# ratschlab/secedo

Measured on AMD Instinct MI355X. Metric: cell-pair x locus updates/sec (similarity matrix), higher is better.
Workload: dtype int64; 1 GPU; C3: 8000 cells x 100000 loci; entries=24345058, kept_entries=24223307, reads=23997029, block_cells=128, tiles=2016, normalization=ADD_MIN, max_fragment_length=1000, num_threads=8, parallelism=single GPU, backend=none, world_size=1, rccl_world_size=1

## Files before the change

include/secedo_simmat.h:

```cpp
#ifndef SECEDO_SIMMAT_H
#define SECEDO_SIMMAT_H

#include <stdint.h>

#ifdef __cplusplus
extern "C" {
#endif

#define SECEDO_OK 0
#define SECEDO_E_INVALID_ARG (-1)
#define SECEDO_E_INVALID_NORMALIZATION (-2)
#define SECEDO_E_NO_DEVICE (-3)
#define SECEDO_E_HIP (-4)
#define SECEDO_E_STATE (-5)
#define SECEDO_E_LIMIT (-6)

#define SECEDO_NORM_ADD_MIN 0
#define SECEDO_NORM_EXPONENTIATE 1
#define SECEDO_NORM_SCALE_MAX_1 2

int secedo_simmat_normalization_from_string(const char *name);

const char *secedo_simmat_last_error(void);
const char *secedo_simmat_version(void);
int secedo_simmat_device_count(void);

int secedo_simmat_compute(const uint32_t *chr_locus_off, uint32_t n_chr, const uint32_t *locus_pos,
                          const uint64_t *locus_entry_off, const uint32_t *read_ids,
                          const uint16_t *id_base16, const uint32_t *id_base32,
                          const uint32_t *group_id_to_pos, uint32_t n_groups, uint32_t num_cells,
                          uint32_t max_fragment_length, double mutation_rate,
                          double homozygous_rate, double seq_error_rate, uint32_t num_threads,
                          int normalization, double *out);
int secedo_simmat_set_devices(const int *device_ids, uint32_t n_devices);
int secedo_simmat_get_devices(int *device_ids, uint32_t capacity);

int secedo_simmat_staging_acquire(const uint64_t bytes[5], void *ptrs[5]);
void secedo_simmat_staging_release(void);

void secedo_simmat_release_cache(void);

typedef struct secedo_simmat secedo_simmat_t;

int secedo_simmat_create(secedo_simmat_t **handle, int device_id);
void secedo_simmat_destroy(secedo_simmat_t *handle);

int secedo_simmat_set_pileup(secedo_simmat_t *handle, const uint32_t *chr_locus_off, uint32_t n_chr,
                             const uint32_t *locus_pos, const uint64_t *locus_entry_off,
                             const uint32_t *read_ids, const uint16_t *id_base16,
                             const uint32_t *id_base32, const uint32_t *group_id_to_pos,
                             uint32_t n_groups);

int secedo_simmat_set_pileup_device(secedo_simmat_t *handle, const uint32_t *d_chr_locus_off,
                                    uint32_t n_chr, const uint32_t *d_locus_pos,
                                    const uint64_t *d_locus_entry_off, const uint32_t *d_read_ids,
                                    const uint16_t *d_id_base16, const uint32_t *d_id_base32,
                                    const uint32_t *d_group_id_to_pos, uint32_t n_groups,
                                    uint32_t n_loci, uint64_t n_entries);

int secedo_simmat_set_packing(secedo_simmat_t *handle, int mode);
int secedo_simmat_used_device_packing(const secedo_simmat_t *handle);
int secedo_simmat_used_single_entry_path(const secedo_simmat_t *handle);
#define SECEDO_ROUTE_ATTEMPTS 3
#define SECEDO_ROUTE_RADIX 4
#define SECEDO_ROUTE_RETRIED_PLAIN 8
#define SECEDO_ROUTE_ASKED_HOST 16
int secedo_simmat_packing_route(const secedo_simmat_t *handle);

int secedo_simmat_prepare(secedo_simmat_t *handle, uint32_t num_cells, uint32_t max_fragment_length,
                          uint32_t num_threads, uint32_t block_cells, void *stream);

uint32_t secedo_simmat_num_tiles(const secedo_simmat_t *handle);
uint32_t secedo_simmat_block_cells(const secedo_simmat_t *handle);
uint64_t secedo_simmat_acc_elems(const secedo_simmat_t *handle);
uint64_t secedo_simmat_num_entries(const secedo_simmat_t *handle);
uint64_t secedo_simmat_num_reads(const secedo_simmat_t *handle);
uint64_t secedo_simmat_num_loci(const secedo_simmat_t *handle);

uint64_t secedo_simmat_pair_bound(const secedo_simmat_t *handle);
uint32_t secedo_simmat_max_read_entries(const secedo_simmat_t *handle);
int secedo_simmat_cell_squares(secedo_simmat_t *handle, uint64_t *d_out , void *stream);
int secedo_simmat_set_scale_bounds(secedo_simmat_t *handle, uint64_t pair_bound, uint32_t max_read_entries);
int secedo_simmat_set_pair_bound(secedo_simmat_t *handle, uint64_t pair_bound);
int secedo_simmat_scale_bounds_state(const secedo_simmat_t *handle);
int secedo_simmat_scale_log2(const secedo_simmat_t *handle);

int secedo_simmat_zero_acc(secedo_simmat_t *handle, int64_t *d_acc, void *stream);
int secedo_simmat_accumulate(secedo_simmat_t *handle, double mutation_rate, double homozygous_rate,
                             double seq_error_rate, uint32_t tile_begin, uint32_t tile_end,
                             int64_t *d_acc, void *stream);
int secedo_simmat_assign(secedo_simmat_t *handle, double mutation_rate, double homozygous_rate,
                         double seq_error_rate, uint32_t tile_begin, uint32_t tile_end, int64_t *d_acc,
                         void *stream);
int secedo_simmat_finalize(secedo_simmat_t *handle, int normalization, const int64_t *d_acc,
                           double *d_out, void *stream);
int secedo_simmat_assign_finalize(secedo_simmat_t *handle, double mutation_rate, double homozygous_rate,
                                  double seq_error_rate, int normalization, int64_t *d_acc, double *d_out,
                                  void *stream);
int secedo_simmat_tiles_of_rows(const secedo_simmat_t *handle, uint32_t row_begin, uint32_t row_end,
                                uint32_t *tile_ids, uint32_t *n_tile_ids);
int secedo_simmat_accumulate_list(secedo_simmat_t *handle, double mutation_rate, double homozygous_rate,
                                  double seq_error_rate, const uint32_t *tile_ids, uint32_t n_tile_ids,
                                  int64_t *d_acc, void *stream);
int secedo_simmat_assign_list(secedo_simmat_t *handle, double mutation_rate, double homozygous_rate,
                              double seq_error_rate, const uint32_t *tile_ids, uint32_t n_tile_ids,
                              int64_t *d_acc, void *stream);
int secedo_simmat_max_of_tiles(secedo_simmat_t *handle, const int64_t *d_acc, const uint32_t *tile_ids,
                               uint32_t n_tile_ids, double *max_value, void *stream);
int secedo_simmat_finalize_rows_max(secedo_simmat_t *handle, int normalization, const int64_t *d_acc,
                                    uint32_t row_begin, uint32_t row_end, double max_value, double *d_out_rows,
                                    void *stream);
int secedo_simmat_finalize_rows(secedo_simmat_t *handle, int normalization, const int64_t *d_acc,
                                uint32_t row_begin, uint32_t row_end, double *d_out_rows, void *stream);
int secedo_simmat_finalize_raw(secedo_simmat_t *handle, const int64_t *d_acc, double *d_out,
                               void *stream);

int secedo_simmat_last_counts(secedo_simmat_t *handle, uint64_t *updates, uint64_t *read_pairs);
int secedo_simmat_last_accumulate_ms(secedo_simmat_t *handle, float *ms);
int secedo_simmat_last_pair_kernel_ms(secedo_simmat_t *handle, float *ms);
const char *secedo_simmat_pair_kernel(const secedo_simmat_t *handle);
int secedo_simmat_last_correction_fused(const secedo_simmat_t *handle);
int secedo_simmat_last_locus_words(const secedo_simmat_t *handle);
uint32_t secedo_simmat_last_workgroups(const secedo_simmat_t *handle);
int secedo_simmat_debug_flag_lists(secedo_simmat_t *handle, uint64_t *n_flagged, uint32_t *grp, uint32_t *rec,
                                   uint32_t *idx);

double secedo_simmat_llr(uint32_t x_s, uint32_t x_d, double mutation_rate, double homozygous_rate,
                         double seq_error_rate);
double secedo_simmat_llr_closed_form(uint32_t x_s, uint32_t x_d, double mutation_rate, double homozygous_rate,
                                     double seq_error_rate);

int secedo_is_significant(const uint16_t *base_count , double seq_error_rate,
                          uint32_t cell_proportion);

int secedo_filter(const uint32_t *chr_locus_off, uint32_t n_chr, const uint32_t *locus_pos,
                  const uint64_t *locus_entry_off, const uint32_t *read_ids, const uint16_t *id_base16,
                  const uint32_t *id_base32, const uint32_t *id_to_pos, uint32_t n_groups,
                  double seq_error_rate, uint32_t cell_proportion, uint32_t *out_chr_locus_off,
                  uint32_t *out_locus_pos, uint64_t *out_locus_entry_off, uint32_t *out_read_ids,
                  void *out_id_base, uint64_t *out_n_loci, uint64_t *out_n_entries, double *avg_coverage);

int secedo_filter_device(const uint32_t *d_chr_locus_off, uint32_t n_chr, const uint32_t *d_locus_pos,
                         const uint64_t *d_locus_entry_off, const uint32_t *d_read_ids,
                         const uint16_t *d_id_base16, const uint32_t *d_id_base32, const uint32_t *d_id_to_pos,
                         uint32_t n_groups, uint32_t n_loci, uint64_t n_entries, double seq_error_rate,
                         uint32_t cell_proportion, uint32_t *d_out_chr_locus_off, uint32_t *d_out_locus_pos,
                         uint64_t *d_out_locus_entry_off, uint32_t *d_out_read_ids, void *d_out_id_base,
                         uint64_t *out_n_loci, uint64_t *out_n_entries, double *avg_coverage, void *stream);

typedef struct secedo_pileup_info {
    uint64_t n_loci;
    uint64_t n_entries;
    uint32_t num_cells;
    uint32_t max_read_length;
} secedo_pileup_info;

int secedo_pileup_read(const char *path, const uint16_t *id_to_group, uint32_t n_ids, uint32_t max_coverage,
                       const uint32_t *positions, uint64_t n_positions, int compute_max_read_len,
                       int write_bin, secedo_pileup_info *info, uint32_t *locus_pos,
                       uint64_t *locus_entry_off, uint32_t *read_ids, uint16_t *id_base16);
const char *secedo_pileup_last_error(void);

#ifdef __cplusplus
}
#endif
#endif
```

secedo_amd/_lib.py:

```python
from __future__ import annotations

import ctypes as C
import os

import numpy as np

HERE = os.path.dirname(os.path.abspath(__file__))
LIB_PATH = os.environ.get("SECEDO_LIB_PATH") or os.path.join(HERE, "libsecedo_simmat.so")

OK = 0
E_INVALID_ARG = -1
E_INVALID_NORMALIZATION = -2
E_NO_DEVICE = -3
E_HIP = -4
E_STATE = -5
E_LIMIT = -6

_u16p = C.POINTER(C.c_uint16)
_u32p = C.POINTER(C.c_uint32)
_u64p = C.POINTER(C.c_uint64)
_f64p = C.POINTER(C.c_double)
_vp = C.c_void_p


class PileupInfo(C.Structure):
    _fields_ = [("n_loci", C.c_uint64), ("n_entries", C.c_uint64), ("num_cells", C.c_uint32),
                ("max_read_length", C.c_uint32)]


class SpectralInfo(C.Structure):
    _fields_ = [("cycles", C.c_uint32), ("block_products", C.c_uint32), ("converged", C.c_uint32),
                ("reserved", C.c_uint32), ("max_residual_vectors", C.c_double),
                ("max_residual_values", C.c_double)]


ALLREDUCE_SUM_FN = C.CFUNCTYPE(C.c_int, C.c_void_p, C.c_void_p, C.c_uint64, C.c_void_p)


class SynthSpec(C.Structure):
    _fields_ = [
        ("num_cells", C.c_uint32), ("num_loci", C.c_uint32), ("num_chromosomes", C.c_uint32),
        ("gap_max", C.c_uint32), ("new_frag_prob", C.c_double), ("frag_min", C.c_uint32),
        ("frag_max", C.c_uint32), ("base_error", C.c_double), ("mate_frac", C.c_double),
        ("seed", C.c_uint64),
    ]


SIGNATURES = {
    "secedo_simmat_normalization_from_string": (C.c_int, [C.c_char_p]),
    "secedo_simmat_last_error": (C.c_char_p, []),
    "secedo_simmat_version": (C.c_char_p, []),
    "secedo_simmat_device_count": (C.c_int, []),
    "secedo_simmat_compute": (C.c_int, [_vp, C.c_uint32, _vp, _vp, _vp, _vp, _vp, _vp, C.c_uint32,
                                        C.c_uint32, C.c_uint32, C.c_double, C.c_double, C.c_double,
                                        C.c_uint32, C.c_int, _vp]),
    "secedo_simmat_release_cache": (None, []),
    "secedo_simmat_staging_acquire": (C.c_int, [_vp, _vp]),
    "secedo_simmat_staging_release": (None, []),
    "secedo_simmat_create": (C.c_int, [C.POINTER(_vp), C.c_int]),
    "secedo_simmat_destroy": (None, [_vp]),
    "secedo_simmat_set_pileup": (C.c_int, [_vp, _vp, C.c_uint32, _vp, _vp, _vp, _vp, _vp, _vp,
                                           C.c_uint32]),
    "secedo_simmat_set_pileup_device": (C.c_int, [_vp, _vp, C.c_uint32, _vp, _vp, _vp, _vp, _vp, _vp,
                                                  C.c_uint32, C.c_uint32, C.c_uint64]),
    "secedo_simmat_set_packing": (C.c_int, [_vp, C.c_int]),
    "secedo_simmat_used_device_packing": (C.c_int, [_vp]),
    "secedo_simmat_used_single_entry_path": (C.c_int, [_vp]),
    "secedo_simmat_packing_route": (C.c_int, [_vp]),
    "secedo_simmat_prepare": (C.c_int, [_vp, C.c_uint32, C.c_uint32, C.c_uint32, C.c_uint32, _vp]),
    "secedo_simmat_num_tiles": (C.c_uint32, [_vp]),
    "secedo_simmat_block_cells": (C.c_uint32, [_vp]),
    "secedo_simmat_acc_elems": (C.c_uint64, [_vp]),
    "secedo_simmat_num_entries": (C.c_uint64, [_vp]),
    "secedo_simmat_num_reads": (C.c_uint64, [_vp]),
    "secedo_simmat_num_loci": (C.c_uint64, [_vp]),
    "secedo_simmat_zero_acc": (C.c_int, [_vp, _vp, _vp]),
    "secedo_simmat_accumulate": (C.c_int, [_vp, C.c_double, C.c_double, C.c_double, C.c_uint32,
                                           C.c_uint32, _vp, _vp]),
    "secedo_simmat_finalize": (C.c_int, [_vp, C.c_int, _vp, _vp, _vp]),
    "secedo_simmat_tiles_of_rows": (C.c_int, [_vp, C.c_uint32, C.c_uint32, _vp, C.POINTER(C.c_uint32)]),
    "secedo_simmat_assign": (C.c_int, [_vp, C.c_double, C.c_double, C.c_double, C.c_uint32, C.c_uint32, _vp, _vp]),
    "secedo_simmat_assign_list": (C.c_int, [_vp, C.c_double, C.c_double, C.c_double, _vp, C.c_uint32, _vp, _vp]),
    "secedo_simmat_assign_finalize": (C.c_int, [_vp, C.c_double, C.c_double, C.c_double, C.c_int, _vp, _vp, _vp]),
    "secedo_simmat_accumulate_list": (C.c_int, [_vp, C.c_double, C.c_double, C.c_double, _vp, C.c_uint32, _vp, _vp]),
    "secedo_simmat_max_of_tiles": (C.c_int, [_vp, _vp, _vp, C.c_uint32, C.POINTER(C.c_double), _vp]),
    "secedo_simmat_finalize_rows_max": (C.c_int, [_vp, C.c_int, _vp, C.c_uint32, C.c_uint32, C.c_double, _vp, _vp]),
    "secedo_simmat_finalize_rows": (C.c_int, [_vp, C.c_int, _vp, C.c_uint32, C.c_uint32, _vp, _vp]),
    "secedo_simmat_finalize_raw": (C.c_int, [_vp, _vp, _vp, _vp]),
    "secedo_simmat_last_counts": (C.c_int, [_vp, _u64p, _u64p]),
    "secedo_simmat_last_accumulate_ms": (C.c_int, [_vp, C.POINTER(C.c_float)]),
    "secedo_simmat_last_pair_kernel_ms": (C.c_int, [_vp, C.POINTER(C.c_float)]),
    "secedo_simmat_pair_kernel": (C.c_char_p, [_vp]),
    "secedo_simmat_last_correction_fused": (C.c_int, [_vp]),
    "secedo_simmat_last_locus_words": (C.c_int, [_vp]),
    "secedo_simmat_last_workgroups": (C.c_uint32, [_vp]),
    "secedo_simmat_debug_flag_lists": (C.c_int, [_vp, _u64p, _vp, _vp, _vp]),
    "secedo_simmat_llr": (C.c_double, [C.c_uint32, C.c_uint32, C.c_double, C.c_double, C.c_double]),
    "secedo_simmat_llr_closed_form": (C.c_double, [C.c_uint32, C.c_uint32, C.c_double, C.c_double, C.c_double]),
    "secedo_simmat_pair_bound": (C.c_uint64, [_vp]),
    "secedo_simmat_set_pair_bound": (C.c_int, [_vp, C.c_uint64]),
    "secedo_simmat_max_read_entries": (C.c_uint32, [_vp]),
    "secedo_simmat_cell_squares": (C.c_int, [_vp, _vp, _vp]),
    "secedo_simmat_set_scale_bounds": (C.c_int, [_vp, C.c_uint64, C.c_uint32]),
    "secedo_simmat_scale_log2": (C.c_int, [_vp]),
    "secedo_simmat_scale_bounds_state": (C.c_int, [_vp]),
    "secedo_simmat_set_devices": (C.c_int, [C.POINTER(C.c_int), C.c_uint32]),
    "secedo_simmat_get_devices": (C.c_int, [C.POINTER(C.c_int), C.c_uint32]),
    "secedo_is_significant": (C.c_int, [_vp, C.c_double, C.c_uint32]),
    "secedo_filter": (C.c_int, [_vp, C.c_uint32, _vp, _vp, _vp, _vp, _vp, _vp, C.c_uint32, C.c_double,
                                C.c_uint32, _vp, _vp, _vp, _vp, _vp, _u64p, _u64p, _f64p]),
    "secedo_filter_device": (C.c_int, [_vp, C.c_uint32, _vp, _vp, _vp, _vp, _vp, _vp, C.c_uint32, C.c_uint32,
                                       C.c_uint64, C.c_double, C.c_uint32, _vp, _vp, _vp, _vp, _vp, _u64p,
                                       _u64p, _f64p, _vp]),
    "secedo_pileup_read": (C.c_int, [C.c_char_p, _vp, C.c_uint32, C.c_uint32, _vp, C.c_uint64, C.c_int, C.c_int,
                                     C.POINTER(PileupInfo), _vp, _vp, _vp, _vp]),
    "secedo_pileup_last_error": (C.c_char_p, []),
    "secedo_em_refine_device": (C.c_int, [C.c_int, _vp, C.c_uint32, C.c_uint64, _vp, _vp, _vp, C.c_uint32, C.c_double,
                                          _vp, C.c_uint32, C.c_uint32, C.POINTER(C.c_uint32), _vp]),
    "secedo_em_refine": (C.c_int, [C.c_int, _vp, C.c_uint32, _vp, _vp, _vp, C.c_uint32, C.c_double, _vp, C.c_uint32,
                                   C.c_uint32, C.POINTER(C.c_uint32)]),
    "secedo_laplacian_device": (C.c_int, [_vp, C.c_uint32, _vp, _vp]),
    "secedo_spectral_eigs_device": (C.c_int, [C.c_int, _vp, C.c_uint32, C.c_uint32, C.c_uint32, C.c_double,
                                              C.c_uint32, _vp, _vp, C.POINTER(SpectralInfo), _vp]),
    "secedo_spectral_eigs_rows_device": (C.c_int, [C.c_int, _vp, C.c_uint32, C.c_uint32, C.c_uint32, C.c_uint32,
                                                   C.c_uint32, C.c_double, C.c_uint32, _vp, _vp,
                                                   C.POINTER(SpectralInfo), _vp, _vp, _vp]),
    "secedo_spectral_eigs": (C.c_int, [C.c_int, _vp, C.c_uint32, C.c_uint32, C.c_uint32, C.c_double, C.c_uint32,
                                       _vp, _vp, C.POINTER(SpectralInfo)]),
}

_lib = None


class SecedoError(RuntimeError):
    def __init__(self, code, message):
        super().__init__("secedo_simmat error %d: %s" % (code, message))
        self.code = code


class InvalidNormalization(ValueError):
    """The reference throws std::logic_error here (similarity_matrix.cpp:264)."""


def lib():
    global _lib
    if _lib is None:
        if not os.path.exists(LIB_PATH):
            raise ImportError(
                "%s is missing: build it with `python -c 'import __graft_entry__ as g; g.build()'` "
                "or `make -C secedo_amd/csrc` (there is no fallback implementation)" % LIB_PATH)
        try:
            import torch
        except ImportError:
            pass
        l = C.CDLL(LIB_PATH)
        for name, (res, args) in SIGNATURES.items():
            f = getattr(l, name)
            f.restype = res
            f.argtypes = args
        _lib = l
    return _lib


def check(rc):
    if rc == OK:
        return
    msg = lib().secedo_simmat_last_error().decode(errors="replace")
    if rc == E_INVALID_NORMALIZATION:
        raise InvalidNormalization(msg)
    raise SecedoError(rc, msg)


def ptr(a):
    return None if a is None else a.ctypes.data
```

secedo_amd/csrc/pack_device.hip:

```cpp
#include "pack_device.hpp"

#include <hip/hip_runtime.h>
#include <hipcub/hipcub.hpp>

#include <algorithm>
#include <chrono>
#include <cstdio>
#include <cstdlib>
#include <cstring>
#include <functional>

namespace secedo {

DeviceArena::~DeviceArena() {
    if (p) (void)hipFree(p);
}

DevicePacked::~DevicePacked() {
    if (side) (void)hipStreamDestroy(side);
    if (ev_fork) (void)hipEventDestroy(ev_fork);
    if (ev_join) (void)hipEventDestroy(ev_join);
    if (ev_offsets) (void)hipEventDestroy(ev_offsets);
    if (ev_flush) (void)hipEventDestroy(ev_flush);
    if (mailbox) (void)hipHostFree(mailbox);
}

int poison_level() {
    static const int level = [] {
        const char *e = std::getenv("SECEDO_POISON");
        return e ? std::atoi(e) : 0;
    }();
    return level;
}

hipError_t DeviceArena::ensure(size_t n) {
    if (n <= bytes && p) return hipSuccess;
    if (p) (void)hipFree(p);
    p = nullptr;
    bytes = 0;
    const size_t want = n ? n + n / 8 + 256 : 256;
    hipError_t e = hipMalloc(&p, want);
    if (e == hipSuccess) bytes = want;
    if (e == hipSuccess && poison_level() >= 1) e = hipMemset(p, 0xA5, want);
    return e;
}

namespace {

constexpr int TPB = 256;

inline uint32_t blocks_for(uint64_t n) {
    return static_cast<uint32_t>(std::max<uint64_t>(1, std::min<uint64_t>((n + TPB - 1) / TPB, 1u << 16)));
}

struct Scalars {
    uint32_t error;
    uint32_t need_host;
    uint32_t num_ranges;
    uint32_t max_read_id;
    uint32_t regroup;
    uint32_t long_reads;
    uint32_t split_changed;
    uint32_t id_exceeded;
    uint32_t max_read_entries;
    uint32_t caps_wrong;
    uint32_t n_multi_id;
    uint32_t reads_total;
    uint32_t n_wide;
    uint32_t max_range_span;
    unsigned long long id_space;
    unsigned long long multi_entries;
    unsigned long long pair_bound;
};

struct Mailbox {
    Scalars sc;
    unsigned long long totals;
    unsigned long long seq;
};

__global__ void k_publish(const Scalars *sc, const unsigned long long *totals, Mailbox *box, unsigned long long seq) {
    if (threadIdx.x == 0) {
        box->sc = *sc;
        box->totals = totals ? *totals : 0ull;
        __hip_atomic_store(&box->seq, seq, __ATOMIC_RELEASE, __HIP_MEMORY_SCOPE_SYSTEM);
    }
}

hipError_t read_scalars(DevicePacked &pk, hipStream_t stream, const Scalars *sc, const unsigned long long *totals,
                        Scalars *out, unsigned long long *out_totals, const std::function<void()> &behind = nullptr) {
    static const bool plain = [] {
        const char *e = std::getenv("SECEDO_PACK_READBACK");
        return e && std::strcmp(e, "memcpy") == 0;
    }();
    hipError_t e;
    if (!plain && !pk.mailbox && !pk.mailbox_failed) {
        if (hipHostMalloc(&pk.mailbox, sizeof(Mailbox), hipHostMallocCoherent) == hipSuccess) {
            std::memset(pk.mailbox, 0, sizeof(Mailbox));
        } else {
            (void)hipGetLastError();
            pk.mailbox = nullptr;
            pk.mailbox_failed = true;
        }
    }
    if (!plain && pk.mailbox) {
        Mailbox *box = static_cast<Mailbox *>(pk.mailbox);
        const unsigned long long seq = ++pk.mailbox_seq;
        hipLaunchKernelGGL(k_publish, dim3(1), dim3(64), 0, stream, sc, totals, box, seq);
        if ((e = hipGetLastError()) != hipSuccess) return e;
        if (behind) behind();
        bool arrived = false;
        for (unsigned spins = 0;; ++spins) {
            if (__atomic_load_n(&box->seq, __ATOMIC_ACQUIRE) == seq) {
                arrived = true;
                break;
            }
            if ((spins & 0xFFFu) == 0xFFFu) {
                const hipError_t q = hipStreamQuery(stream);
                if (q != hipErrorNotReady) {
                    arrived = __atomic_load_n(&box->seq, __ATOMIC_ACQUIRE) == seq;
                    if (q != hipSuccess) return q;
                    break;
                }
            }
        }
        if (arrived) {
            *out = box->sc;
            if (out_totals) *out_totals = box->totals;
            return hipSuccess;
        }
    } else if (behind) {
        behind();
    }
    if (out_totals) {
        *out_totals = 0;
        if (totals && (e = hipMemcpyAsync(out_totals, totals, 8, hipMemcpyDeviceToHost, stream)) != hipSuccess) return e;
    }
    if ((e = hipMemcpyAsync(out, sc, sizeof(*out), hipMemcpyDeviceToHost, stream)) != hipSuccess) return e;
    return hipStreamSynchronize(stream);
}

struct HostTrace {
    bool on;
    std::chrono::steady_clock::time_point t0;
    HostTrace() : on(std::getenv("SECEDO_PACK_TRACE") != nullptr), t0(std::chrono::steady_clock::now()) {}
    void mark(const char *what) const {
        if (on)
            std::fprintf(stderr, "[pack-trace] %8.1f us  %s\n",
                         std::chrono::duration<double, std::micro>(std::chrono::steady_clock::now() - t0).count(), what);
    }
};

constexpr uint32_t kRankScanLimit = 8192;
constexpr int kMaxSplitRounds = 32;
constexpr uint32_t kIdSpaceFactor = 4;

struct Raw {
    const uint32_t *chr_locus_off;
    uint32_t n_chr;
    const uint32_t *locus_pos;
    const uint64_t *locus_entry_off;
    const uint32_t *read_ids;
    const uint16_t *id_base16;
    const uint32_t *id_base32;
    const uint32_t *g2p;
    uint32_t n_groups;
    uint32_t n_loci;
    uint32_t n_entries;
    __device__ __forceinline__ uint32_t id_base(uint32_t e) const {
        return id_base16 ? (uint32_t)id_base16[e] : id_base32[e];
    }
};

template <class T>
__device__ __forceinline__ uint32_t last_le(const T *a, uint32_t n, T x) {
    uint32_t lo = 0, hi = n;
    while (hi - lo > 1) {
        const uint32_t mid = lo + (hi - lo) / 2;
        if (a[mid] <= x) lo = mid; else hi = mid;
    }
    return lo;
}

__global__ __launch_bounds__(TPB) void k_entry_locus(Raw in, uint32_t *entry_locus, Scalars *sc) {
    const uint32_t lane = threadIdx.x & 63u;
    const uint32_t wave = (blockIdx.x * TPB + threadIdx.x) >> 6, n_waves = (gridDim.x * TPB) >> 6;
    for (uint32_t l = wave; l < in.n_loci; l += n_waves) {
        const uint32_t b = (uint32_t)in.locus_entry_off[l], e = (uint32_t)in.locus_entry_off[l + 1];
        for (uint32_t i = b + lane; i < e; i += 64u) entry_locus[i] = l;
        if (lane == 0u && l + 1 < in.n_loci && in.locus_pos[l + 1] <= in.locus_pos[l]) {
            const uint32_t c = last_le<uint32_t>(in.chr_locus_off, in.n_chr + 1, l);
            if (l + 1 < in.chr_locus_off[c + 1]) sc->error = 3;
        }
    }
}

__device__ __forceinline__ uint32_t chr_first_entry(const Raw &in, uint32_t c) {
    return (uint32_t)in.locus_entry_off[in.chr_locus_off[c]];
}

__global__ __launch_bounds__(TPB) void k_id_range(Raw in, uint32_t *id_max, uint32_t *id_negmin, int vec, Scalars *sc) {
    __shared__ uint32_t s_hi[TPB / 64], s_neg[TPB / 64];
    __shared__ uint32_t s_chr;
    for (uint32_t l = blockIdx.x * TPB + threadIdx.x; l + 1 < in.n_loci; l += gridDim.x * TPB) {
        if (in.locus_pos[l + 1] <= in.locus_pos[l]) {
            const uint32_t c = last_le<uint32_t>(in.chr_locus_off, in.n_chr + 1, l);
            if (l + 1 < in.chr_locus_off[c + 1]) sc->error = 3;
        }
    }
    const uint32_t E = in.n_entries;
    const uint32_t chunk = (E + gridDim.x - 1) / gridDim.x;
    uint32_t cur = min(E, blockIdx.x * chunk);
    const uint32_t e1 = min(E, cur + chunk);
    if (cur >= e1) return;
    if (threadIdx.x == 0) s_chr = 0;
    __syncthreads();
    {
        uint32_t best = 0;
        for (uint32_t i = threadIdx.x; i < in.n_chr; i += TPB)
            if (chr_first_entry(in, i) <= cur) best = i;
        if (best) atomicMax(&s_chr, best);
    }
    __syncthreads();
    uint32_t c = s_chr;
    while (cur < e1) {
        uint32_t c_end = (uint32_t)in.locus_entry_off[in.chr_locus_off[c + 1]];
        while (c_end <= cur && c + 1 < in.n_chr) {
            ++c;
            c_end = (uint32_t)in.locus_entry_off[in.chr_locus_off[c + 1]];
        }
        const uint32_t seg_end = (c + 1 < in.n_chr) ? min(e1, c_end) : e1;
        uint32_t hi = 0, neg = 0;
        uint32_t s_cur = cur, s_end = seg_end;
        if (vec) {
            const uint32_t a = min(seg_end, (cur + 3u) & ~3u), b = max(a, seg_end & ~3u);
            if (threadIdx.x < a - cur) {
                const uint32_t id = in.read_ids[cur + threadIdx.x];
                hi = max(hi, id);
                neg = max(neg, ~id);
            }
            if (threadIdx.x < seg_end - b) {
                const uint32_t id = in.read_ids[b + threadIdx.x];
                hi = max(hi, id);
                neg = max(neg, ~id);
            }
            const uint4 *src = reinterpret_cast<const uint4 *>(in.read_ids);
            for (uint32_t q = a / 4u + threadIdx.x; q < b / 4u; q += TPB * 4) {
                uint4 v[4];
#pragma unroll
                for (int u = 0; u < 4; ++u) v[u] = q + (uint32_t)u * TPB < b / 4u ? src[q + (uint32_t)u * TPB] : src[q];
#pragma unroll
                for (int u = 0; u < 4; ++u) {
                    hi = max(max(hi, v[u].x), max(max(v[u].y, v[u].z), v[u].w));
                    neg = max(max(neg, ~v[u].x), max(max(~v[u].y, ~v[u].z), ~v[u].w));
                }
            }
            s_cur = s_end = seg_end;
        }
        for (uint32_t e = s_cur + threadIdx.x; e < s_end; e += TPB * 8) {
            uint32_t id[8];
#pragma unroll
            for (int u = 0; u < 8; ++u) {
                const uint32_t eu = e + (uint32_t)u * TPB;
                id[u] = eu < s_end ? in.read_ids[eu] : in.read_ids[e];
            }
#pragma unroll
            for (int u = 0; u < 8; ++u) {
                hi = max(hi, id[u]);
                neg = max(neg, ~id[u]);
            }
        }
        for (int off = 32; off > 0; off >>= 1) {
            hi = max(hi, (uint32_t)__shfl_down(hi, off));
            neg = max(neg, (uint32_t)__shfl_down(neg, off));
        }
        __syncthreads();
        if ((threadIdx.x & 63u) == 0) {
            s_hi[threadIdx.x >> 6] = hi;
            s_neg[threadIdx.x >> 6] = neg;
        }
        __syncthreads();
        if (threadIdx.x == 0) {
            for (int w = 1; w < TPB / 64; ++w) {
                hi = max(hi, s_hi[w]);
                neg = max(neg, s_neg[w]);
            }
            atomicMax(&id_max[c], hi);
            atomicMax(&id_negmin[c], neg);
        }
        cur = seg_end;
    }
}

__global__ void k_id_bases(Raw in, const uint32_t *id_max, const uint32_t *id_negmin, uint32_t *id_base,
                           uint32_t *chr_entry, unsigned long long assumed_space, Scalars *sc) {
    const uint32_t n_chr = in.n_chr;
    if (blockIdx.x != 0) return;
    for (uint32_t c = threadIdx.x; c <= n_chr; c += blockDim.x) chr_entry[c] = chr_first_entry(in, c);
    if (threadIdx.x != 0) return;
    unsigned long long sum = 0;
    uint32_t top = 0;
    for (uint32_t c = 0; c < n_chr; ++c) {
        id_base[c] = (uint32_t)min(sum, 0xFFFFFFFFull);
        const uint32_t lo = ~id_negmin[c];
        if ((id_max[c] | id_negmin[c]) != 0u) sum += (unsigned long long)(id_max[c] - lo) + 1ull;
        top = max(top, id_max[c]);
    }
    id_base[n_chr] = (uint32_t)min(sum, 0xFFFFFFFFull);
    sc->id_space = sum;
    sc->max_read_id = top;
    if (assumed_space && sum > assumed_space) sc->id_exceeded = 1;
}

__global__ void k_entry_keys(Raw in, const uint32_t *entry_locus, uint32_t id_bits, unsigned long long *key,
                             uint32_t *val) {
    for (uint32_t e = blockIdx.x * TPB + threadIdx.x; e < in.n_entries; e += gridDim.x * TPB) {
        const uint32_t c = last_le<uint32_t>(in.chr_locus_off, in.n_chr + 1, entry_locus[e]);
        key[e] = ((unsigned long long)c << id_bits) | in.read_ids[e];
        val[e] = e;
    }
}

constexpr uint32_t kSlocLocusMask = 0x3FFFFFFFu;
__device__ __forceinline__ uint32_t sloc_pack(uint32_t locus, uint32_t id_base) { return locus | (id_base << 30); }
__device__ __forceinline__ uint32_t sloc_locus(uint32_t v) { return v & kSlocLocusMask; }
__device__ __forceinline__ uint32_t sloc_base(uint32_t v) { return v >> 30; }

__global__ void k_sorted_locus(Raw in, const uint32_t *sval, const uint32_t *entry_locus, uint32_t n, uint32_t *sloc) {
    for (uint32_t s = blockIdx.x * TPB + threadIdx.x; s < n; s += gridDim.x * TPB)
        sloc[s] = sloc_pack(entry_locus[sval[s]], in.id_base(sval[s]));
}

constexpr uint32_t kChrLds = 1024;
struct ChrTables {
    uint32_t first[kChrLds + 1], base[kChrLds], min_id[kChrLds];
};
__device__ __forceinline__ bool chr_tables_load(const Raw &in, const uint32_t *first, const uint32_t *id_base,
                                                const uint32_t *id_negmin, ChrTables &t) {
    const bool in_lds = in.n_chr <= kChrLds;
    if (in_lds) {
        for (uint32_t i = threadIdx.x; i <= in.n_chr; i += blockDim.x) t.first[i] = first[i];
        for (uint32_t i = threadIdx.x; i < in.n_chr; i += blockDim.x) {
            t.base[i] = id_base[i];
            t.min_id[i] = ~id_negmin[i];
        }
    }
    __syncthreads();
    return in_lds;
}
__device__ __forceinline__ uint32_t chr_of(const Raw &in, const uint32_t *first, const ChrTables &t, bool in_lds,
                                           uint32_t key) {
    return last_le<uint32_t>(in_lds ? t.first : first, in.n_chr + 1, key);
}
__device__ __forceinline__ uint32_t dense_of(const uint32_t *id_base, const uint32_t *id_negmin, const ChrTables &t,
                                             bool in_lds, uint32_t c, uint32_t id) {
    return in_lds ? t.base[c] + (id - t.min_id[c]) : id_base[c] + (id - ~id_negmin[c]);
}
__device__ __forceinline__ uint32_t dense_id(const Raw &in, const uint32_t *first, const uint32_t *id_base,
                                             const uint32_t *id_negmin, const ChrTables &t, bool in_lds, uint32_t key,
                                             uint32_t id) {
    return dense_of(id_base, id_negmin, t, in_lds, chr_of(in, first, t, in_lds, key), id);
}
__device__ __forceinline__ void dense_id_quad(const Raw &in, const uint32_t *chr_entry, const uint32_t *id_base,
                                              const uint32_t *id_negmin, const ChrTables &t, bool in_lds, uint32_t e0,
                                              const uint32_t (&id)[4], uint32_t (&d)[4]) {
    const uint32_t c0 = chr_of(in, chr_entry, t, in_lds, e0);
    const uint32_t next = in_lds ? t.first[c0 + 1] : chr_entry[c0 + 1];
#pragma unroll
    for (int u = 0; u < 4; ++u) {
        const uint32_t e = min(e0 + (uint32_t)u, in.n_entries - 1u);
        const uint32_t c = e < next ? c0 : chr_of(in, chr_entry, t, in_lds, e);
        d[u] = dense_of(id_base, id_negmin, t, in_lds, c, id[u]);
    }
}

__global__ void k_id_hist(Raw in, const uint32_t *entry_locus, const uint32_t *id_base, const uint32_t *id_negmin,
                          const Scalars *sc, uint32_t *dense, uint32_t *hist) {
    if (sc->id_exceeded) return;
    __shared__ ChrTables tables;
    const bool in_lds = chr_tables_load(in, in.chr_locus_off, id_base, id_negmin, tables);
    for (uint32_t e = blockIdx.x * TPB + threadIdx.x; e < in.n_entries; e += gridDim.x * TPB) {
        const uint32_t d = dense_id(in, in.chr_locus_off, id_base, id_negmin, tables, in_lds, entry_locus[e], in.read_ids[e]);
        dense[e] = d;
        atomicAdd(&hist[d], 1u);
    }
}

__global__ void k_id_scatter(const uint32_t *dense, uint32_t n, const uint32_t *id_off, const Scalars *sc,
                             uint32_t *hist, uint32_t *grouped) {
    if (sc->id_exceeded) return;
    for (uint32_t e = blockIdx.x * TPB + threadIdx.x; e < n; e += gridDim.x * TPB) {
        const uint32_t d = dense[e];
        grouped[id_off[d] + atomicSub(&hist[d], 1u) - 1u] = e;
    }
}

__global__ void k_id_rank(Raw in, const uint32_t *dense, const uint32_t *id_off, const uint32_t *grouped,
                          const uint32_t *entry_locus, unsigned long long *skey, uint32_t *sval, uint32_t *sloc,
                          Scalars *sc) {
    const bool void_run = sc->id_exceeded != 0;
    for (uint32_t p = blockIdx.x * TPB + threadIdx.x; p < in.n_entries; p += gridDim.x * TPB) {
        if (void_run) {
            skey[p] = p;
            sval[p] = p;
            sloc[p] = 0;
            continue;
        }
        const uint32_t e = grouped[p];
        const uint32_t d = dense[e];
        const uint32_t b = id_off[d], n = id_off[d + 1] - b;
        uint32_t rank = p - b;
        if (n > kRankScanLimit) {
            sc->regroup = 1;
        } else if (n > 1) {
            rank = 0;
            for (uint32_t q = b; q < b + n; ++q) rank += grouped[q] < e ? 1u : 0u;
        }
        skey[b + rank] = d;
        sval[b + rank] = e;
        sloc[b + rank] = sloc_pack(entry_locus[e], in.id_base(e));
    }
}

__device__ __forceinline__ void load_id_quad(const Raw &in, uint32_t q, int vec, uint32_t (&id)[4]) {
    const uint32_t n = in.n_entries, e0 = q * 4u;
    if (vec && e0 + 4u <= n) {
        const uint4 iv = reinterpret_cast<const uint4 *>(in.read_ids)[q];
        id[0] = iv.x, id[1] = iv.y, id[2] = iv.z, id[3] = iv.w;
    } else {
#pragma unroll
        for (int u = 0; u < 4; ++u) id[u] = in.read_ids[min(e0 + (uint32_t)u, n - 1u)];
    }
}
__global__ void k_id_store(Raw in, const uint32_t *chr_entry, const uint32_t *id_base, const uint32_t *id_negmin,
                           const Scalars *sc, uint32_t *last, int vec) {
    if (sc->id_exceeded) return;
    __shared__ ChrTables tables;
    const bool in_lds = chr_tables_load(in, chr_entry, id_base, id_negmin, tables);
    const uint32_t n = in.n_entries, stride = gridDim.x * TPB;
    for (uint32_t q = blockIdx.x * TPB + threadIdx.x; q < (n + 3u) / 4u; q += stride) {
        const uint32_t e0 = q * 4u;
        uint32_t id[4], d[4];
        load_id_quad(in, q, vec, id);
        dense_id_quad(in, chr_entry, id_base, id_negmin, tables, in_lds, e0, id, d);
#pragma unroll
        for (int u = 0; u < 4; ++u)
            if (e0 + (uint32_t)u < n) last[d[u]] = e0 + (uint32_t)u + 1u;
    }
}
__global__ void k_id_check(Raw in, const uint32_t *chr_entry, const uint32_t *id_base, const uint32_t *id_negmin,
                           const Scalars *sc, const uint32_t *last, uint8_t *multi, int vec) {
    if (sc->id_exceeded) return;
    __shared__ ChrTables tables;
    const bool in_lds = chr_tables_load(in, chr_entry, id_base, id_negmin, tables);
    const uint32_t n = in.n_entries, stride = gridDim.x * TPB;
    for (uint32_t q = blockIdx.x * TPB + threadIdx.x; q < (n + 3u) / 4u; q += stride) {
        const uint32_t e0 = q * 4u;
        uint32_t id[4], d[4], w[4];
        load_id_quad(in, q, vec, id);
        dense_id_quad(in, chr_entry, id_base, id_negmin, tables, in_lds, e0, id, d);
#pragma unroll
        for (int u = 0; u < 4; ++u) w[u] = e0 + (uint32_t)u < n ? last[d[u]] : 0u;
#pragma unroll
        for (int u = 0; u < 4; ++u) {
            const uint32_t e = e0 + (uint32_t)u;
            if (e < n && w[u] != e + 1u) {
                multi[e] = 1;
                multi[w[u] - 1u] = 1;
            }
        }
    }
}
__global__ __launch_bounds__(TPB) void k_flag_count(const uint8_t *multi, uint32_t *block_sum) {
    __shared__ uint32_t part[TPB / 64];
    static_assert(kFlagBlock == TPB * 16, "a thread takes 16 consecutive flags");
    const uint4 w = reinterpret_cast<const uint4 *>(multi + (size_t)blockIdx.x * kFlagBlock)[threadIdx.x];
    uint32_t n = ((w.x * 0x01010101u) >> 24) + ((w.y * 0x01010101u) >> 24) + ((w.z * 0x01010101u) >> 24)
            + ((w.w * 0x01010101u) >> 24);
    for (int off = 32; off > 0; off >>= 1) n += __shfl_down(n, off);
    if ((threadIdx.x & 63u) == 0u) part[threadIdx.x >> 6] = n;
    __syncthreads();
    if (threadIdx.x == 0u) {
        for (int w2 = 1; w2 < TPB / 64; ++w2) n += part[w2];
        block_sum[blockIdx.x] = n;
    }
}
constexpr int TPB_SCAN = 1024;
__global__ __launch_bounds__(TPB_SCAN) void k_flag_scan(const uint32_t *block_sum, uint32_t n_blocks, uint32_t *block_off,
                                                       uint32_t *total_out, Scalars *sc) {
    constexpr int TPB = TPB_SCAN;
    __shared__ uint32_t part[TPB / 64];
    __shared__ uint32_t carry;
    if (threadIdx.x == 0u) carry = 0;
    __syncthreads();
    const uint32_t lane = threadIdx.x & 63u, wv = threadIdx.x >> 6;
    for (uint32_t base = 0; base < n_blocks; base += TPB) {
        const uint32_t i = base + threadIdx.x;
        const uint32_t v = i < n_blocks ? block_sum[i] : 0u;
        uint32_t incl = v;
        for (int off = 1; off < 64; off <<= 1) {
            const uint32_t up = __shfl_up(incl, off);
            if (lane >= (uint32_t)off) incl += up;
        }
        if (lane == 63u) part[wv] = incl;
        __syncthreads();
        uint32_t before = carry;
        for (uint32_t w2 = 0; w2 < wv; ++w2) before += part[w2];
        if (i < n_blocks) block_off[i] = before + incl - v;
        __syncthreads();
        if (threadIdx.x == TPB - 1) carry = before + incl;
        __syncthreads();
    }
    if (threadIdx.x == 0u) {
        *total_out = carry;
        if (sc) sc->n_multi_id = carry;
    }
}
struct MIndex {
    const uint32_t *chunk_pre;
    const unsigned long long *chunk_mask;
    __device__ __forceinline__ uint32_t operator()(uint32_t e) const {
        const uint32_t c = e >> 6, r = e & 63u;
        return chunk_pre[c] + (uint32_t)__popcll(chunk_mask[c] & ((1ull << r) - 1ull));
    }
};
__global__ __launch_bounds__(TPB) void k_compact_m(Raw in, const uint8_t *multi, const uint32_t *block_off,
                                                  uint32_t *chunk_pre, unsigned long long *chunk_mask,
                                                  uint32_t *m_entry) {
    __shared__ uint32_t part[TPB / 64];
    const uint32_t lane = threadIdx.x & 63u, wv = threadIdx.x >> 6;
    const uint32_t e0 = blockIdx.x * kFlagBlock + threadIdx.x * 16u;
    const uint4 w = reinterpret_cast<const uint4 *>(multi + (size_t)blockIdx.x * kFlagBlock)[threadIdx.x];
    const uint32_t words[4] = {w.x, w.y, w.z, w.w};
    uint32_t bits = 0;
#pragma unroll
    for (int i = 0; i < 16; ++i) bits |= ((words[i >> 2] >> ((i & 3) * 8)) & 1u) << i;
    const uint32_t mine = (uint32_t)__popc(bits);
    uint32_t incl = mine;
    for (int off = 1; off < 64; off <<= 1) {
        const uint32_t up = __shfl_up(incl, off);
        if (lane >= (uint32_t)off) incl += up;
    }
    if (lane == 63u) part[wv] = incl;
    __syncthreads();
    uint32_t j = block_off[blockIdx.x] + incl - mine;
    for (uint32_t w2 = 0; w2 < wv; ++w2) j += part[w2];
    unsigned long long m = (unsigned long long)bits << ((lane & 3u) * 16u);
    m |= __shfl_xor(m, 1);
    m |= __shfl_xor(m, 2);
    if ((lane & 3u) == 0u) {
        const uint32_t chunk = blockIdx.x * (kFlagBlock / 64u) + (threadIdx.x >> 2);
        chunk_pre[chunk] = j;
        chunk_mask[chunk] = m;
    }
    if (blockIdx.x == gridDim.x - 1u && threadIdx.x == 0u) chunk_mask[gridDim.x * (kFlagBlock / 64u)] = 0ull;
    for (uint32_t b = bits; b; b &= b - 1u) m_entry[j++] = e0 + (uint32_t)__ffs((int)b) - 1u;
}
__global__ __launch_bounds__(TPB) void k_pflag_count(const uint32_t *entry32, uint32_t n, uint32_t *block_sum) {
    __shared__ uint32_t part[TPB / 64];
    const uint32_t b0 = blockIdx.x * kFlagBlock + threadIdx.x;
    uint32_t c = 0;
#pragma unroll
    for (int k = 0; k < 16; ++k) {
        const uint32_t e = b0 + (uint32_t)k * TPB;
        c += (e < n && (entry32[e] & (kC_Tail | kC_Multi)) != 0u) ? 1u : 0u;
    }
    for (int off = 32; off > 0; off >>= 1) c += __shfl_down(c, off);
    if ((threadIdx.x & 63u) == 0u) part[threadIdx.x >> 6] = c;
    __syncthreads();
    if (threadIdx.x == 0u) {
        for (int w = 1; w < TPB / 64; ++w) c += part[w];
        block_sum[blockIdx.x] = c;
    }
}
__global__ __launch_bounds__(TPB) void k_pflag_compact(const uint32_t *entry32, const uint4 *entry, uint32_t n,
                                                      const uint32_t *block_off, uint4 *rec, uint32_t *idx,
                                                      uint32_t *chunk_pre, unsigned long long *chunk_mask) {
    constexpr int WAVES = TPB / 64;
    static_assert(16 * WAVES == 64, "one wave scans the (round, wave) counts");
    __shared__ uint32_t cnt[16 * WAVES];
    const uint32_t lane = threadIdx.x & 63u, wv = threadIdx.x >> 6;
    const uint32_t b0 = blockIdx.x * kFlagBlock + threadIdx.x;
    unsigned long long m[16];
#pragma unroll
    for (int k = 0; k < 16; ++k) {
        const uint32_t e = b0 + (uint32_t)k * TPB;
        m[k] = __ballot(e < n && (entry32[e] & (kC_Tail | kC_Multi)) != 0u);
        if (lane == 0u) cnt[k * WAVES + wv] = (uint32_t)__popcll(m[k]);
    }
    __syncthreads();
    if (threadIdx.x < 64u) {
        const uint32_t v = cnt[threadIdx.x];
        uint32_t incl = v;
        for (int off = 1; off < 64; off <<= 1) {
            const uint32_t up = __shfl_up(incl, off);
            if (lane >= (uint32_t)off) incl += up;
        }
        cnt[threadIdx.x] = incl - v;
    }
    __syncthreads();
    const uint32_t base = block_off[blockIdx.x];
#pragma unroll
    for (int k = 0; k < 16; ++k) {
        const uint32_t e = b0 + (uint32_t)k * TPB;
        const uint32_t before = base + cnt[k * WAVES + wv];
        if (lane == 0u) {
            const uint32_t chunk = (blockIdx.x * kFlagBlock + (uint32_t)k * TPB) / 64u + wv;
            chunk_pre[chunk] = before;
            chunk_mask[chunk] = m[k];
        }
        if ((m[k] >> lane) & 1ull) {
            const uint32_t j = before + (uint32_t)__popcll(m[k] & ((1ull << lane) - 1ull));
            rec[j] = entry[e];
            idx[j] = e;
        }
    }
}
__global__ __launch_bounds__(TPB) void k_pflag_compact_masks(const unsigned long long *chunk_mask, const uint4 *entry,
                                                            const uint32_t *block_off, uint4 *rec, uint32_t *idx,
                                                            uint32_t *chunk_pre) {
    constexpr int WAVES = TPB / 64;
    constexpr uint32_t CHUNKS = kFlagBlock / 64u;
    static_assert(CHUNKS == 64, "one wave scans the chunks' counts");
    __shared__ unsigned long long mask[CHUNKS];
    __shared__ uint32_t pre[CHUNKS];
    const uint32_t lane = threadIdx.x & 63u, wv = threadIdx.x >> 6;
    const uint32_t chunk0 = blockIdx.x * CHUNKS;
    if (threadIdx.x < 64u) {
        const unsigned long long m = chunk_mask[chunk0 + threadIdx.x];
        const uint32_t v = (uint32_t)__popcll(m);
        uint32_t incl = v;
        for (int off = 1; off < 64; off <<= 1) {
            const uint32_t up = __shfl_up(incl, off);
            if (lane >= (uint32_t)off) incl += up;
        }
        mask[threadIdx.x] = m;
        pre[threadIdx.x] = incl - v;
        chunk_pre[chunk0 + threadIdx.x] = block_off[blockIdx.x] + incl - v;
    }
    __syncthreads();
    const uint32_t base = block_off[blockIdx.x];
#pragma unroll 4
    for (uint32_t c = wv; c < CHUNKS; c += WAVES) {
        const unsigned long long m = mask[c];
        if ((m >> lane) & 1ull) {
            const uint32_t e = (chunk0 + c) * 64u + lane;
            const uint32_t j = base + pre[c] + (uint32_t)__popcll(m & ((1ull << lane) - 1ull));
            rec[j] = entry[e];
            idx[j] = e;
        }
    }
}
__global__ __launch_bounds__(TPB) void k_pflag_groups(const uint32_t *blk_off, size_t n_off, const uint32_t *chunk_pre,
                                                     const unsigned long long *chunk_mask, uint32_t *grp) {
    for (size_t i = (size_t)blockIdx.x * TPB + threadIdx.x; i < n_off; i += (size_t)gridDim.x * TPB) {
        const uint32_t d = blk_off[i], c = d >> 6, r = d & 63u;
        grp[i] = chunk_pre[c] + (r ? (uint32_t)__popcll(chunk_mask[c] & ((1ull << r) - 1ull)) : 0u);
    }
}
void flag_groups(const FlagScratch &fs, const uint32_t *blk_off, size_t n_off, uint32_t *grp, hipStream_t stream) {
    if (!n_off) return;
    const uint32_t blocks = (uint32_t)std::min<size_t>((n_off + TPB - 1) / TPB, 256 * 32);
    hipLaunchKernelGGL(k_pflag_groups, dim3(blocks), dim3(TPB), 0, stream, blk_off, n_off, fs.chunk_pre, fs.chunk_mask, grp);
}
void flag_lists_from_masks(const FlagScratch &fs, const uint4 *entry, const uint32_t *blk_off, size_t n_off,
                           uint32_t *grp, uint4 *rec, uint32_t *idx, hipStream_t stream) {
    hipLaunchKernelGGL(k_flag_scan, dim3(1), dim3(TPB_SCAN), 0, stream, fs.block_sum, fs.nb, fs.block_off,
                       fs.chunk_pre + 64 * (size_t)fs.nb, static_cast<Scalars *>(nullptr));
    hipLaunchKernelGGL(k_pflag_compact_masks, dim3(fs.nb), dim3(TPB), 0, stream, fs.chunk_mask, entry, fs.block_off, rec,
                       idx, fs.chunk_pre);
    flag_groups(fs, blk_off, n_off, grp, stream);
}

__global__ void k_m_fields(Raw in, const uint32_t *chr_entry, const uint32_t *id_base, const uint32_t *id_negmin,
                           const uint32_t *last, MIndex m_index, const uint32_t *m_entry, uint32_t n_m, uint32_t *rid_m,
                           uint32_t *idb_m, uint32_t *eloc_m, uint32_t *winner_m, uint32_t *count_m) {
    __shared__ ChrTables tables;
    const bool in_lds = chr_tables_load(in, chr_entry, id_base, id_negmin, tables);
    for (uint32_t j = blockIdx.x * TPB + threadIdx.x; j < n_m; j += gridDim.x * TPB) {
        const uint32_t e = m_entry[j];
        const uint32_t id = in.read_ids[e];
        rid_m[j] = id;
        idb_m[j] = in.id_base(e);
        eloc_m[j] = last_le<uint64_t>(in.locus_entry_off, in.n_loci + 1, (uint64_t)e);
        const uint32_t d = dense_id(in, chr_entry, id_base, id_negmin, tables, in_lds, e, id);
        const uint32_t w = m_index(last[d] - 1u);
        winner_m[j] = w;
        atomicAdd(&count_m[w], 1u);
    }
}
__global__ void k_group_scatter(const uint32_t *winner_m, uint32_t n_m, const uint32_t *goff, uint32_t *count_m,
                                uint32_t *members, uint32_t *g_begin, uint32_t *g_len) {
    for (uint32_t j = blockIdx.x * TPB + threadIdx.x; j < n_m; j += gridDim.x * TPB) {
        const uint32_t w = winner_m[j];
        const uint32_t b = goff[w], n = goff[w + 1] - b;
        members[b + atomicSub(&count_m[w], 1u) - 1u] = j;
        g_begin[j] = b;
        g_len[j] = n;
    }
}
__global__ void k_group_rank(Raw sub, const uint32_t *members, const uint32_t *g_begin, const uint32_t *g_len,
                             const uint32_t *eloc_m, uint32_t n_m, unsigned long long *skey, uint32_t *sval,
                             uint32_t *sloc, Scalars *sc) {
    for (uint32_t p = blockIdx.x * TPB + threadIdx.x; p < n_m; p += gridDim.x * TPB) {
        const uint32_t m = members[p];
        const uint32_t b = g_begin[m], n = g_len[m];
        uint32_t rank = p - b;
        if (n > kRankScanLimit) {
            sc->regroup = 1;
        } else {
            rank = 0;
            for (uint32_t q = b; q < b + n; ++q) rank += members[q] < m ? 1u : 0u;
        }
        skey[b + rank] = b;
        sval[b + rank] = m;
        sloc[b + rank] = sloc_pack(eloc_m[m], sub.id_base(m));
    }
}

constexpr uint32_t kCibBits = 7;
constexpr uint32_t kNoEntry = 0xFFFFFFFFu;
constexpr uint32_t kSingle = 0x80000000u;
constexpr uint32_t kSingleBaseShift = 29;
constexpr uint32_t kSingleTail = 4u;

struct Ranks {
    MIndex m_index;
    const uint32_t *unm;
    const uint32_t *arank;
    __device__ __forceinline__ uint32_t operator()(uint32_t e) const { return unm ? e - unm[m_index(e)] : arank[e]; }
};
struct UnmarkedM {
    const uint32_t *mark_m;
    uint32_t n_m;
    __device__ __forceinline__ uint32_t operator()(uint32_t j) const { return j < n_m ? 1u - mark_m[j] : 0u; }
};
__global__ void k_arank_m(const uint32_t *unm, const uint32_t *m_entry, uint32_t n_m, uint32_t n, uint32_t *arank_m,
                          Scalars *sc) {
    for (uint32_t j = blockIdx.x * TPB + threadIdx.x; j < n_m; j += gridDim.x * TPB) arank_m[j] = m_entry[j] - unm[j];
    if (blockIdx.x == 0 && threadIdx.x == 0) sc->reads_total = n - unm[n_m];
}
__global__ void k_rbeg(Raw in, Ranks rank, uint32_t *rbeg) {
    for (uint32_t c = blockIdx.x * TPB + threadIdx.x; c <= in.n_chr; c += gridDim.x * TPB)
        rbeg[c] = rank((uint32_t)in.locus_entry_off[in.chr_locus_off[c]]);
}
struct HeadKeepOp {
    const unsigned long long *skey;
    const uint32_t *keep;
    const uint32_t *split;
    __device__ __forceinline__ unsigned long long operator()(uint32_t s) const {
        const unsigned long long head = (s == 0 || skey[s] != skey[s - 1] || (split && split[s])) ? 1ull : 0ull;
        return head | ((unsigned long long)keep[s] << 32);
    }
};
__device__ __forceinline__ uint32_t incl_reads(unsigned long long v) { return (uint32_t)v; }
__device__ __forceinline__ uint32_t incl_kept(unsigned long long v) { return (uint32_t)(v >> 32); }

__global__ void k_dup_mark(Raw in, const unsigned long long *skey, const uint32_t *sval,
                           const uint32_t *sloc, const uint32_t *split, uint32_t n, uint32_t *keep,
                           uint32_t *mark) {
    for (uint32_t s = blockIdx.x * TPB + threadIdx.x; s < n; s += gridDim.x * TPB) {
        const uint32_t e = sval[s];
        const uint32_t l = sloc_locus(sloc[s]);
        const bool same_read = s > 0 && skey[s] == skey[s - 1];
        mark[e] = (same_read && !(split && split[s])) ? 0u : 1u;
        if (s == 0) mark[n] = 0u;
        if (same_read && sloc_locus(sloc[s - 1]) == l) continue;
        uint32_t stored = s;
        bool have = true;
        keep[s] = 0u;
        for (uint32_t t = s + 1; t < n && skey[t] == skey[s] && sloc_locus(sloc[t]) == l; ++t) {
            keep[t] = 0u;
            if (have) {
                if (sloc_base(sloc[t]) != sloc_base(sloc[stored])) have = false;
            } else {
                stored = t;
                have = true;
            }
        }
        if (have) keep[stored] = 1u;
    }
}

__global__ void k_runs_csr(Raw in, const unsigned long long *incl, const uint32_t *sval,
                           const uint32_t *sloc, uint32_t n, uint32_t *run_start, uint32_t *read_locus,
                           uint8_t *read_base) {
    for (uint32_t s = blockIdx.x * TPB + threadIdx.x; s < n; s += gridDim.x * TPB) {
        const unsigned long long cur = incl[s], prev = s ? incl[s - 1] : 0ull;
        if (incl_reads(cur) != incl_reads(prev)) run_start[incl_reads(cur) - 1] = s;
        if (s == n - 1) run_start[incl_reads(cur)] = n;
        if (incl_kept(cur) != incl_kept(prev)) {
            const uint32_t k = incl_kept(prev), v = sloc[s];
            read_locus[k] = sloc_locus(v);
            read_base[k] = (uint8_t)sloc_base(v);
        }
    }
}

__global__ __launch_bounds__(TPB) void k_read_info(Raw in, const unsigned long long *incl, const uint32_t *run_start,
                                                  const uint32_t *sval, const uint32_t *sloc,
                                                  const uint32_t *arank, uint32_t mfl, uint32_t *run_rank,
                                                  uint32_t *rbeg, uint32_t *read_off, Scalars *sc) {
    __shared__ unsigned long long part[TPB / 64];
    __shared__ uint32_t part_len[TPB / 64];
    const uint32_t n = in.n_entries;
    const uint32_t n_runs = n ? incl_reads(incl[n - 1]) : 0u;
    unsigned long long multi = 0;
    uint32_t longest = 0;
    for (uint32_t r = blockIdx.x * TPB + threadIdx.x; r < n_runs; r += gridDim.x * TPB) {
        const uint32_t s0 = run_start[r], s1 = run_start[r + 1];
        const uint32_t e0 = sval[s0];
        const uint32_t p0 = in.locus_pos[sloc_locus(sloc[s0])], p1 = in.locus_pos[sloc_locus(sloc[s1 - 1])];
        if (p1 - p0 >= mfl) sc->long_reads = 1;
        if ((unsigned long long)p1 + mfl > 0xFFFFFFFFull) sc->need_host = 1;
        const uint32_t rk = arank[e0];
        run_rank[r] = rk;
        const uint32_t k0 = s0 ? incl_kept(incl[s0 - 1]) : 0u, k1 = incl_kept(incl[s1 - 1]);
        read_off[r] = k0;
        if (r == n_runs - 1) read_off[n_runs] = k1;
        if (k1 - k0 > 1) multi += k1 - k0;
        longest = max(longest, k1 - k0);
    }
    if (rbeg) {
        for (uint32_t c = blockIdx.x * TPB + threadIdx.x; c <= in.n_chr; c += gridDim.x * TPB)
            rbeg[c] = arank[(uint32_t)in.locus_entry_off[in.chr_locus_off[c]]];
    }
    for (int off = 32; off > 0; off >>= 1) {
        multi += __shfl_down(multi, off);
        longest = max(longest, (uint32_t)__shfl_down(longest, off));
    }
    if ((threadIdx.x & 63) == 0) {
        part[threadIdx.x >> 6] = multi;
        part_len[threadIdx.x >> 6] = longest;
    }
    __syncthreads();
    if (threadIdx.x == 0) {
        unsigned long long sum = 0;
        uint32_t len = 0;
        for (int w = 0; w < TPB / 64; ++w) {
            sum += part[w];
            len = max(len, part_len[w]);
        }
        if (sum) atomicAdd(&sc->multi_entries, sum);
        if (len > 1) atomicMax(&sc->max_read_entries, len);
    }
}

__global__ void k_completed(Raw in, Ranks rank, const uint32_t *rbeg, uint32_t mfl, uint32_t *cnt, Scalars *sc) {
    for (uint32_t l = blockIdx.x * TPB + threadIdx.x; l < in.n_loci; l += gridDim.x * TPB) {
        const uint32_t c = last_le<uint32_t>(in.chr_locus_off, in.n_chr + 1, l);
        const uint32_t pos = in.locus_pos[l], l0 = in.chr_locus_off[c];
        if ((unsigned long long)pos + mfl > 0xFFFFFFFFull && in.locus_entry_off[l + 1] > in.locus_entry_off[l])
            sc->need_host = 1;
        uint32_t done = 0;
        if (pos >= mfl && in.locus_pos[l0] <= pos - mfl) {
            const uint32_t lp = l0 + last_le<uint32_t>(in.locus_pos + l0, l - l0 + 1, pos - mfl);
            done = rank((uint32_t)in.locus_entry_off[lp + 1]) - rbeg[c];
        }
        cnt[l] = done;
    }
}

__global__ __launch_bounds__(TPB) void k_flush_chain(Raw in, const uint32_t *cnt, uint32_t threshold,
                                                    const Scalars *sc, uint32_t *flushed_out,
                                                    uint32_t *flush_loci, uint32_t *flush_count, Ranks rank,
                                                    const uint32_t *rbeg, uint32_t *tail_begin) {
    __shared__ uint32_t buf[2048];
    __shared__ uint32_t hits[2048];
    __shared__ uint32_t s_flushed, s_listed, s_hits;
    const uint32_t c = blockIdx.x;
    const uint32_t l0 = in.chr_locus_off[c], l1 = in.chr_locus_off[c + 1];
    if (threadIdx.x == 0) {
        s_flushed = 0;
        s_listed = 0;
    }
    for (uint32_t base = l0; base < l1; base += 2048) {
        const uint32_t n = min(2048u, l1 - base);
        __syncthreads();
        for (uint32_t i = threadIdx.x; i < n; i += TPB) buf[i] = cnt[base + i];
        __syncthreads();
        if (threadIdx.x == 0) {
            uint32_t f = s_flushed, h = 0;
            if (sc->long_reads) {
                for (uint32_t i = 0; i < n; ++i) {
                    const uint32_t v = buf[i];
                    if (v - f >= threshold) {
                        f = v;
                        hits[h++] = base + i;
                    }
                }
            } else {
                for (uint32_t i = 0; i < n; ++i) {
                    const uint32_t v = buf[i];
                    if (v - f >= threshold) f = v;
                }
            }
            s_flushed = f;
            s_hits = h;
        }
        __syncthreads();
        const uint32_t h = s_hits, listed = s_listed;
        for (uint32_t i = threadIdx.x; i < h; i += TPB) flush_loci[l0 + listed + i] = hits[i];
        __syncthreads();
        if (threadIdx.x == 0) s_listed = listed + h;
    }
    __syncthreads();
    if (threadIdx.x == 0) {
        flushed_out[c] = s_flushed;
        flush_count[c] = s_listed;
    }
    if (tail_begin) {
        __shared__ uint32_t s_first;
        const unsigned long long want = (unsigned long long)rbeg[c] + s_flushed;
        uint32_t lo = (uint32_t)in.locus_entry_off[l0], hi = (uint32_t)in.locus_entry_off[l1];
        while (lo < hi) {
            const uint32_t step = (hi - lo + TPB - 1) / TPB;
            const unsigned long long probe = (unsigned long long)lo + (unsigned long long)threadIdx.x * step;
            const bool reached = probe < hi && (unsigned long long)rank((uint32_t)probe) >= want;
            __syncthreads();
            if (threadIdx.x == 0) s_first = TPB;
            __syncthreads();
            if (reached) atomicMin(&s_first, threadIdx.x);
            __syncthreads();
            const uint32_t first = s_first;
            if (first == TPB) {
                lo = lo + ((hi - lo - 1) / step) * step + 1;
            } else {
                hi = lo + first * step;
                if (first) lo = lo + (first - 1) * step + 1;
            }
        }
        if (threadIdx.x == 0) tail_begin[c] = lo;
    }
}

__global__ void k_split_update(Raw in, const unsigned long long *skey, const uint32_t *sloc, uint32_t mfl, const uint32_t *flush_loci,
                               const uint32_t *flush_count, uint32_t *split, Scalars *sc) {
    const uint32_t n = in.n_entries;
    for (uint32_t s = blockIdx.x * TPB + threadIdx.x; s < n; s += gridDim.x * TPB) {
        if (s > 0 && skey[s] == skey[s - 1]) continue;
        uint32_t end = s + 1;
        while (end < n && skey[end] == skey[s]) ++end;
        if (end == s + 1) continue;
        const uint32_t l_first = sloc_locus(sloc[s]);
        const uint32_t p_first = in.locus_pos[l_first], p_last = in.locus_pos[sloc_locus(sloc[end - 1])];
        if (p_last - p_first < mfl) continue;
        const uint32_t c = last_le<uint32_t>(in.chr_locus_off, in.n_chr + 1, l_first);
        const uint32_t *fl = flush_loci + in.chr_locus_off[c];
        const uint32_t n_fl = flush_count[c];
        uint32_t seg_start = p_first, l_prev = l_first;
        for (uint32_t t = s + 1; t < end; ++t) {
            const uint32_t l_t = sloc_locus(sloc[t]);
            uint32_t cut = 0;
            if (l_t != l_prev) {
                uint32_t lo = 0, hi = n_fl;
                const unsigned long long reach = (unsigned long long)seg_start + mfl;
                while (lo < hi) {
                    const uint32_t mid = lo + (hi - lo) / 2;
                    if (fl[mid] <= l_prev || in.locus_pos[fl[mid]] < reach) lo = mid + 1; else hi = mid;
                }
                if (lo < n_fl && fl[lo] <= l_t) {
                    cut = 1;
                    seg_start = in.locus_pos[l_t];
                }
            }
            if (split[t] != cut) {
                split[t] = cut;
                sc->split_changed = 1;
            }
            l_prev = l_t;
        }
    }
}

__device__ __forceinline__ unsigned long long bin_key(uint32_t blk, uint32_t l, uint32_t cib, uint32_t lbits) {
    return ((((unsigned long long)blk << lbits) | l) << kCibBits) | cib;
}

__global__ void k_keys2(Raw in, const uint32_t *sval, const unsigned long long *incl,
                        const uint32_t *read_locus, const uint32_t *run_rank, const uint32_t *read_off,
                        uint32_t num_cells, uint32_t B,
                        uint32_t lbits, unsigned long long *key2, uint32_t *val2, uint32_t *t_read,
                        uint32_t *krank, uint8_t *kflags, unsigned long long *entry_kc, const uint32_t *entry_map,
                        uint32_t *blk_cnt_add, uint32_t L, Scalars *sc) {
    const uint32_t n = in.n_entries;
    for (uint32_t s = blockIdx.x * TPB + threadIdx.x; s < n; s += gridDim.x * TPB) {
        const unsigned long long cur = incl[s], prev = s ? incl[s - 1] : 0ull;
        const uint32_t e_out = entry_map ? entry_map[sval[s]] : sval[s];
        if (incl_kept(cur) == incl_kept(prev)) {
            if (entry_kc) entry_kc[e_out] = kNoEntry;
            continue;
        }
        const uint32_t k = incl_kept(prev);
        const uint32_t group = in.id_base(sval[s]) >> 2;
        uint32_t cell = 0;
        if (group >= in.n_groups) {
            sc->error = 1;
        } else {
            cell = in.g2p[group];
            if (cell >= num_cells) {
                sc->error = 2;
                cell = 0;
            }
        }
        const uint32_t blk = cell / B, cib = cell - blk * B;
        if (key2) {
            key2[k] = bin_key(blk, read_locus[k], cib, lbits);
            val2[k] = k;
        }
        const uint32_t r = incl_reads(cur) - 1;
        t_read[k] = r;
        krank[k] = run_rank[r];
        kflags[k] = (uint8_t)((in.id_base(sval[s]) & 3u) | (read_off[r + 1] - read_off[r] > 1u ? 4u : 0u));
        if (entry_kc) entry_kc[e_out] = ((unsigned long long)((blk << kCibBits) | cib) << 32) | k;
        if (blk_cnt_add) atomicAdd(&blk_cnt_add[(size_t)blk * (L + 1) + read_locus[k]], 1u);
    }
}

__device__ __forceinline__ uint32_t tile_locus(const uint32_t *s_off, uint32_t lo, uint32_t hi, uint32_t e) {
    while (hi - lo > 1u) {
        const uint32_t mid = (lo + hi) >> 1;
        if (s_off[mid] <= e) lo = mid; else hi = mid;
    }
    return lo;
}

__global__ __launch_bounds__(TPB) void k_bin_hist(Raw in, uint32_t nb, uint32_t TL, unsigned long long *__restrict__ entry_kc,
                                                 const unsigned long long *__restrict__ m_mask, uint32_t num_cells,
                                                 uint32_t B_log2, uint32_t *__restrict__ blk_cnt, Scalars *sc,
                                                 uint32_t g2p_lds) {
    extern __shared__ uint32_t lds_hist[];
    __shared__ uint32_t s_off[65];
    static_assert(TPB >= 65, "one thread per offset");
    const uint32_t L = in.n_loci, TLP = TL + 1u, TL_log2 = 31u - (uint32_t)__clz((int)TL);
    const uint32_t n_tiles = (L + TL - 1u) / TL;
    constexpr int U = 4;
    uint16_t *s_g2p = reinterpret_cast<uint16_t *>(lds_hist + nb * TLP);
    if (g2p_lds) {
        for (uint32_t i = threadIdx.x; i < in.n_groups; i += TPB) s_g2p[i] = (uint16_t)min(in.g2p[i], 0xFFFFu);
    }
    for (uint32_t tile = blockIdx.x; tile < n_tiles; tile += gridDim.x) {
        const uint32_t l0 = tile * TL, n_l = min(TL, L - l0);
        for (uint32_t i = threadIdx.x; i < nb * TLP; i += TPB) lds_hist[i] = 0;
        if (threadIdx.x <= n_l) s_off[threadIdx.x] = (uint32_t)in.locus_entry_off[l0 + threadIdx.x];
        __syncthreads();
        const uint32_t eb = s_off[0], ee = s_off[n_l];
        for (uint32_t base = eb + threadIdx.x; base < ee; base += TPB * U) {
            uint32_t slot[U];
            constexpr uint32_t kNone = 0xFFFFFFFFu;
            if (m_mask) {
                unsigned long long mw[U];
                uint32_t ib[U], cell[U];
                bool is_m[U];
#pragma unroll
                for (int u = 0; u < U; ++u) {
                    const uint32_t e = base + (uint32_t)u * TPB;
                    const bool in_tile = e < ee;
                    mw[u] = in_tile ? m_mask[e >> 6] : ~0ull;
                    ib[u] = in_tile ? in.id_base(e) : 0u;
                }
#pragma unroll
                for (int u = 0; u < U; ++u) {
                    const uint32_t group = ib[u] >> 2;
                    cell[u] = 0;
                    is_m[u] = (mw[u] >> ((base + (uint32_t)u * TPB) & 63u)) & 1ull;
                    if (!is_m[u]) {
                        if (group >= in.n_groups) sc->error = 1;
                        else cell[u] = g2p_lds ? (uint32_t)s_g2p[group] : in.g2p[group];
                    }
                }
#pragma unroll
                for (int u = 0; u < U; ++u) {
                    slot[u] = kNone;
                    if (is_m[u]) continue;
                    const uint32_t e = base + (uint32_t)u * TPB;
                    uint32_t c = cell[u];
                    if (c >= num_cells) {
                        sc->error = 2;
                        c = 0;
                    }
                    const uint32_t blk = c >> B_log2, cib = c - (blk << B_log2);
                    entry_kc[e] = ((unsigned long long)(((ib[u] & 3u) << kSingleBaseShift) | (blk << kCibBits) | cib) << 32)
                            | kSingle;
                    slot[u] = blk;
                }
            } else {
#pragma unroll
                for (int u = 0; u < U; ++u) {
                    const uint32_t e = base + (uint32_t)u * TPB;
                    const unsigned long long kc = e < ee ? entry_kc[e] : (unsigned long long)kNoEntry;
                    slot[u] = (uint32_t)kc != kNoEntry ? (uint32_t)(kc >> 32) >> kCibBits : kNone;
                }
            }
#pragma unroll
            for (int u = 0; u < U; ++u) {
                if (slot[u] == kNone) continue;
                const uint32_t j = tile_locus(s_off, 0u, n_l, base + (uint32_t)u * TPB);
                atomicAdd(&lds_hist[slot[u] * TLP + j], 1u);
            }
        }
        __syncthreads();
        for (uint32_t i = threadIdx.x; i < nb * TL; i += TPB) {
            const uint32_t b = i >> TL_log2, j = i & (TL - 1u);
            if (j < n_l) {
                blk_cnt[(size_t)b * (L + 1) + l0 + j] = lds_hist[b * TLP + j];
                if (l0 + j == L - 1) blk_cnt[(size_t)b * (L + 1) + L] = 0;
            }
        }
        __syncthreads();
    }
}

__global__ __launch_bounds__(TPB) void k_bin_place(Raw in, uint32_t nb, uint32_t TL,
                                                  const unsigned long long *__restrict__ entry_kc,
                                                  const uint32_t *__restrict__ blk_off, uint32_t B_log2, uint32_t bm_words,
                                                  const uint32_t *tail_begin,
                                                  unsigned long long *__restrict__ grouped, uint8_t *dupflag) {
    extern __shared__ uint32_t lds_hist[];
    __shared__ uint32_t s_off[65];
    __shared__ uint32_t s_tail[64];
    constexpr uint32_t NW = TPB / 64;
    constexpr int D = 4;
    const uint32_t lane = threadIdx.x & 63u, wv = threadIdx.x >> 6, L = in.n_loci, TLP = TL + 1u;
    const uint32_t TL_log2 = 31u - (uint32_t)__clz((int)TL);
    uint32_t *bm = lds_hist + nb * TLP + wv * bm_words;
    for (uint32_t i = lane; i < bm_words; i += 64u) bm[i] = 0;
    const uint32_t n_tiles = (L + TL - 1u) / TL;
    for (uint32_t tile = blockIdx.x; tile < n_tiles; tile += gridDim.x) {
        const uint32_t l0 = tile * TL, n_l = min(TL, L - l0);
        for (uint32_t i = threadIdx.x; i < nb * TL; i += TPB) {
            const uint32_t b = i >> TL_log2, j = i & (TL - 1u);
            if (j < n_l) lds_hist[b * TLP + j] = blk_off[(size_t)b * (L + 1) + l0 + j];
        }
        if (threadIdx.x <= n_l) s_off[threadIdx.x] = (uint32_t)in.locus_entry_off[l0 + threadIdx.x];
        if (threadIdx.x < n_l)
            s_tail[threadIdx.x] = tail_begin
                    ? tail_begin[last_le<uint32_t>(in.chr_locus_off, in.n_chr + 1, l0 + threadIdx.x)] : 0u;
        __syncthreads();
        const uint32_t per_wave = (n_l + NW - 1u) / NW;
        const uint32_t ja = min(n_l, wv * per_wave), jb = min(n_l, ja + per_wave);
        const uint32_t E0 = s_off[ja], E1 = s_off[jb];
        uint32_t cur = ja;
        bool twice = bm_words == 0u;
        auto close_locus = [&]() {
            const bool any_twice = __ballot(twice) != 0ull;
            if (lane == 0u) dupflag[l0 + cur] = any_twice ? 1 : 0;
            if (bm_words) {
                __builtin_amdgcn_fence(__ATOMIC_RELEASE, "wavefront");
                __builtin_amdgcn_wave_barrier();
                for (uint32_t i = lane; i < bm_words; i += 64u) bm[i] = 0;
                __builtin_amdgcn_fence(__ATOMIC_RELEASE, "wavefront");
                __builtin_amdgcn_wave_barrier();
            }
            twice = bm_words == 0u;
            ++cur;
        };
        auto chunk = [&](unsigned long long kc, uint32_t base) {
            const uint32_t e = base + lane;
            const bool valid = e < E1;
            const uint32_t j = valid ? tile_locus(s_off, cur, jb, e) : 0xFFFFFFFFu;
            const uint32_t chunk_end = min(E1, base + 64u);
            while (true) {
                if (valid && j == cur) {
                    uint32_t k = (uint32_t)kc;
                    if (k != kNoEntry) {
                        uint32_t cc = (uint32_t)(kc >> 32);
                        if (k & kSingle) {
                            k = kSingle | (e >= s_tail[cur] ? kSingleTail : 0u) | (cc >> kSingleBaseShift);
                            cc &= (1u << kSingleBaseShift) - 1u;
                        }
                        if (bm_words) {
                            const uint32_t cell = ((cc >> kCibBits) << B_log2) + (cc & ((1u << kCibBits) - 1u));
                            const uint32_t bit = 1u << (cell & 31u);
                            twice |= (atomicOr(&bm[cell >> 5], bit) & bit) != 0u;
                        }
                        const uint32_t pos = atomicAdd(&lds_hist[(cc >> kCibBits) * TLP + cur], 1u);
                        grouped[pos] = ((unsigned long long)((cc & ((1u << kCibBits) - 1u)) | ((l0 + cur) << kCibBits)) << 32) | k;
                    }
                }
                if (s_off[cur + 1] > chunk_end) break;
                close_locus();
                if (cur >= jb) break;
            }
        };
        unsigned long long ring[D];
#pragma unroll
        for (int d = 0; d < D; ++d) {
            const uint32_t e = E0 + (uint32_t)d * 64u + lane;
            ring[d] = e < E1 ? entry_kc[e] : (unsigned long long)kNoEntry;
        }
        for (uint32_t base = E0; base < E1; base += 64u * D) {
#pragma unroll
            for (int d = 0; d < D; ++d) {
                const uint32_t b = base + (uint32_t)d * 64u;
                if (b >= E1) break;
                const unsigned long long kc = ring[d];
                const uint32_t nxt = b + 64u * D + lane;
                ring[d] = nxt < E1 ? entry_kc[nxt] : (unsigned long long)kNoEntry;
                chunk(kc, b);
            }
        }
        while (cur < jb) close_locus();
        __syncthreads();
    }
}

__global__ __launch_bounds__(TPB) void k_group_counts(const unsigned long long *skey2, uint32_t n, uint32_t B,
                                                     uint32_t L, uint32_t lbits, uint32_t *blk_cnt,
                                                     unsigned long long *per_cell_sq) {
    constexpr uint32_t SLOTS = 512;
    __shared__ unsigned long long sq[SLOTS];
    __shared__ uint32_t first_cell;
    const uint32_t per_block = (n + gridDim.x - 1) / gridDim.x;
    const uint32_t d0 = blockIdx.x * per_block, d1 = min(n, d0 + per_block);
    for (uint32_t i = threadIdx.x; i < SLOTS; i += TPB) sq[i] = 0;
    if (threadIdx.x == 0 && d0 < n) {
        const unsigned long long key = skey2[d0];
        first_cell = (uint32_t)(key >> (kCibBits + lbits)) * B;
    }
    __syncthreads();
    for (uint32_t d = d0 + threadIdx.x; d < d1; d += TPB) {
        const unsigned long long key = skey2[d];
        const unsigned long long grp = key >> kCibBits;
        const uint32_t blk = (uint32_t)(grp >> lbits), l = (uint32_t)grp & ((1u << lbits) - 1u);
        if (d == 0 || skey2[d - 1] >> kCibBits != grp) {
            uint32_t len = 1;
            for (uint32_t t = d + 1; t < n && skey2[t] >> kCibBits == grp; ++t) ++len;
            blk_cnt[(size_t)blk * (L + 1) + l] = len;
        }
        if (d == 0 || skey2[d - 1] != key) {
            unsigned long long cnt = 1;
            for (uint32_t t = d + 1; t < n && skey2[t] == key; ++t) ++cnt;
            const uint32_t cell = blk * B + ((uint32_t)key & ((1u << kCibBits) - 1u));
            const uint32_t rel = cell - first_cell;
            if (rel < SLOTS) atomicAdd(&sq[rel], cnt * cnt);
            else atomicAdd(&per_cell_sq[cell], cnt * cnt);
        }
    }
    __syncthreads();
    if (d0 < n) {
        for (uint32_t i = threadIdx.x; i < SLOTS; i += TPB) {
            if (sq[i]) atomicAdd(&per_cell_sq[first_cell + i], sq[i]);
        }
    }
}

struct CapChoice {
    uint32_t entries_plain, loci_plain;
    uint32_t entries_counts, loci_counts;
    unsigned long long count_limit;
    uint32_t allow_counts;
    __device__ __forceinline__ bool counts(const Scalars *sc) const {
        return allow_counts && sc->pair_bound < count_limit;
    }
};

__global__ __launch_bounds__(TPB) void k_ranges_segment(const uint32_t *blk_off, uint32_t nb, uint32_t L,
                                                       CapChoice caps, uint32_t *seg_ends_both,
                                                       uint32_t *seg_count_both, size_t variant_stride) {
    const bool use_counts = blockIdx.y == 1u;
    const uint32_t cap_entries = use_counts ? caps.entries_counts : caps.entries_plain;
    const uint32_t cap_loci = use_counts ? caps.loci_counts : caps.loci_plain;
    uint32_t *seg_ends = seg_ends_both + blockIdx.y * variant_stride;
    uint32_t *seg_count = seg_count_both + blockIdx.y * variant_stride;
    const size_t stride = (size_t)L + 1;
    const uint32_t seg = blockIdx.x;
    if ((unsigned long long)seg * cap_loci >= L) {
        if (threadIdx.x == 0) seg_count[seg] = 0;
        return;
    }
    const uint32_t seg_begin = seg * cap_loci, seg_end = min(L, seg_begin + cap_loci);
    uint32_t *ends = seg_ends + (size_t)seg * cap_loci;
    uint32_t s = seg_begin, nr = 0, guess = 0;
    auto feasible = [&](uint32_t e) {
        int ok = 1;
        for (uint32_t b = threadIdx.x; b < nb; b += TPB)
            if (blk_off[b * stride + e] - blk_off[b * stride + s] > cap_entries) ok = 0;
        return __syncthreads_and(ok) != 0;
    };
    while (s < seg_end) {
        uint32_t e = s + 1;
        if (feasible(e)) {
            const uint32_t top = seg_end;
            uint32_t lo = e, hi = top;
            if (feasible(top)) {
                lo = top;
            } else if (guess > 1 && s + guess < top) {
                hi = top - 1;
                const uint32_t g = s + guess;
                if (feasible(g)) {
                    lo = g;
                    uint32_t step = max(guess / 8, 1u);
                    while (lo < hi) {
                        const uint32_t nx = min(hi, lo + step);
                        if (feasible(nx)) lo = nx; else { hi = nx - 1; break; }
                        step *= 2;
                    }
                } else {
                    hi = g - 1;
                    uint32_t step = max(guess / 8, 1u);
                    while (hi > lo) {
                        const uint32_t nx = (hi - lo > step) ? hi - step : lo;
                        if (feasible(nx)) { lo = nx; break; }
                        hi = nx - 1;
                        step *= 2;
                    }
                }
            } else {
                hi = top - 1;
            }
            while (lo < hi) {
                const uint32_t mid = lo + (hi - lo + 1) / 2;
                if (feasible(mid)) lo = mid; else hi = mid - 1;
            }
            e = lo;
        }
        guess = e - s;
        if (threadIdx.x == 0) ends[nr] = e;
        ++nr;
        s = e;
    }
    if (threadIdx.x == 0) seg_count[seg] = nr;
}

__global__ __launch_bounds__(TPB) void k_ranges_compact(const uint32_t *seg_ends_both, const uint32_t *seg_count_both,
                                                       size_t variant_stride, uint32_t n_seg, CapChoice caps,
                                                       uint32_t *range_off, const unsigned long long *per_cell_sq,
                                                       uint32_t n_cells_padded, int force_variant, Scalars *sc) {
    __shared__ unsigned long long s_best[TPB / 64];
    if (force_variant < 0) {
        unsigned long long best = 0;
        for (uint32_t i = threadIdx.x; i < n_cells_padded; i += TPB) best = max(best, per_cell_sq[i]);
        for (int off = 32; off > 0; off >>= 1) best = max(best, (unsigned long long)__shfl_down(best, off));
        if ((threadIdx.x & 63) == 0) s_best[threadIdx.x >> 6] = best;
        __syncthreads();
        if (threadIdx.x == 0) {
            for (int w = 1; w < TPB / 64; ++w) best = max(best, s_best[w]);
            sc->pair_bound = max(sc->pair_bound, best);
        }
        __syncthreads();
    }
    const bool use_counts = force_variant < 0 ? caps.counts(sc) : force_variant == 1;
    const uint32_t cap_loci = use_counts ? caps.loci_counts : caps.loci_plain;
    const uint32_t *seg_ends = seg_ends_both + (use_counts ? variant_stride : 0);
    const uint32_t *seg_count = seg_count_both + (use_counts ? variant_stride : 0);
    __shared__ uint32_t s_base, s_span;
    if (threadIdx.x == 0) {
        s_base = 0;
        s_span = 0;
        range_off[0] = 0;
    }
    __syncthreads();
    uint32_t span = 0;
    for (uint32_t seg = 0; seg < n_seg; ++seg) {
        const uint32_t base = s_base, cnt = seg_count[seg];
        const uint32_t *ends = seg_ends + (size_t)seg * cap_loci;
        for (uint32_t i = threadIdx.x; i < cnt; i += TPB) {
            const uint32_t e = ends[i];
            uint32_t begin = __shfl_up(e, 1);
            if ((threadIdx.x & 63u) == 0) begin = i ? ends[i - 1] : seg * cap_loci;
            range_off[1 + base + i] = e;
            span = max(span, e - begin);
        }
        __syncthreads();
        if (threadIdx.x == 0) s_base = base + cnt;
        __syncthreads();
    }
    atomicMax(&s_span, span);
    __syncthreads();
    if (threadIdx.x == 0) {
        sc->num_ranges = s_base;
        sc->max_range_span = s_span;
    }
}

constexpr uint32_t kLocusDup = 0x80000000u;
__global__ void k_locus_info(Raw in, const uint32_t *range_off, const Scalars *sc, const uint8_t *dupflag,
                             uint32_t *locus_chr, uint32_t *locus_rel) {
    const uint32_t n_ranges = sc->num_ranges;
    for (uint32_t l = blockIdx.x * TPB + threadIdx.x; l < in.n_loci; l += gridDim.x * TPB) {
        locus_chr[l] = last_le<uint32_t>(in.chr_locus_off, in.n_chr + 1, l);
        locus_rel[l] = (l - range_off[last_le<uint32_t>(range_off, n_ranges + 1, l)])
                | ((dupflag && dupflag[l]) ? kLocusDup : 0u);
    }
}

__global__ void k_records(Raw in, const unsigned long long *skey2, const uint32_t *sval2, uint32_t n,
                          const uint32_t *t_read, const uint32_t *read_off, const uint32_t *read_locus,
                          const uint8_t *read_base, const uint32_t *krank, const uint8_t *kflags, const uint32_t *rbeg,
                          const uint32_t *flushed, const uint32_t *locus_chr, const uint32_t *locus_rel, uint32_t B,
                          uint32_t lbits, uint4 *entry, uint32_t *entry32, uint32_t *mask32,
                          uint32_t *entry_read, Scalars *sc) {
    uint32_t n_wide = 0;
    for (uint32_t d = blockIdx.x * TPB + threadIdx.x; d < n; d += gridDim.x * TPB) {
        const unsigned long long key = skey2[d];
        const uint32_t k = sval2[d];
        const uint32_t cib = (uint32_t)key & ((1u << kCibBits) - 1u);
        const unsigned long long grp = key >> kCibBits;
        const uint32_t blk = (uint32_t)(grp >> lbits), l = (uint32_t)grp & ((1u << lbits) - 1u);
        const uint32_t cell = blk * B + cib;
        const uint32_t fl = kflags[k];
        const uint32_t base = fl & 3u;
        const bool multi = (fl & 4u) != 0u;
        const uint32_t chr = locus_chr[l];
        const bool tail = krank[k] - rbeg[chr] >= flushed[chr];
        uint32_t r = 0, lo = k, hi = k + 1;
        if (multi) {
            r = t_read[k];
            lo = read_off[r];
            hi = read_off[r + 1];
        }
        uint32_t meta = cell | (base << kMetaBaseShift) | (tail ? kMetaTail : 0u);
        uint32_t masks = 0, bases = 0;
        bool wide = false;
        for (uint32_t j = k; j-- > lo;) {
            const uint32_t dist = l - read_locus[j];
            if (dist > kNarrowWindow) wide = true;
            if (dist > kWindow) {
                meta |= kMetaPrevOvf;
                break;
            }
            masks |= 1u << (dist - 1);
        }
        for (uint32_t j = k + 1; j < hi; ++j) {
            const uint32_t dist = read_locus[j] - l;
            if (dist > kNarrowWindow) wide = true;
            if (dist > kWindow) {
                meta |= kMetaNextOvf;
                break;
            }
            masks |= 1u << (16 + dist - 1);
            bases |= (uint32_t)(read_base[j] & 1u) << (dist - 1);
            bases |= (uint32_t)((read_base[j] >> 1) & 1u) << (16 + dist - 1);
        }
        if (multi || tail) {
            entry[d] = make_uint4(meta, masks, bases, l);
            entry_read[d] = r;
        }
        entry32[d] = cib | (base << kC_BaseShift) | (tail ? kC_Tail : 0u) | (multi ? kC_Multi : 0u)
                | (wide ? kC_Wide : 0u) | ((locus_rel[l] & 0xFFFFu) << 16);
        if (mask32)
            mask32[d] = (masks & 0xFFu) | (((masks >> 16) & 0xFFu) << 8) | ((bases & 0xFFu) << 16)
                    | (((bases >> 16) & 0xFFu) << 24);
        n_wide += wide ? 1u : 0u;
    }
    if (n_wide) atomicAdd(&sc->n_wide, n_wide);
}

constexpr uint32_t kRecMulti = 1u << 30, kRecWide = 1u << 31;
__global__ void k_m_records(Raw in, uint32_t n_kept_m, const uint32_t *t_read, const uint32_t *read_off,
                            const uint32_t *read_locus, const uint8_t *read_base, const uint32_t *krank,
                            const uint8_t *kflags, const uint32_t *rbeg, const uint32_t *flushed, uint4 *m_rec,
                            Scalars *sc) {
    __shared__ uint32_t s_chr[1025];
    const bool chr_lds = in.n_chr <= 1024u;
    if (chr_lds)
        for (uint32_t i = threadIdx.x; i <= in.n_chr; i += TPB) s_chr[i] = in.chr_locus_off[i];
    __syncthreads();
    uint32_t n_wide = 0;
    for (uint32_t k = blockIdx.x * TPB + threadIdx.x; k < n_kept_m; k += gridDim.x * TPB) {
        const uint32_t fl = kflags[k], l = read_locus[k];
        const bool multi = (fl & 4u) != 0u;
        const uint32_t chr = chr_lds ? last_le<uint32_t>(s_chr, in.n_chr + 1, l)
                                     : last_le<uint32_t>(in.chr_locus_off, in.n_chr + 1, l);
        const bool tail = krank[k] - rbeg[chr] >= flushed[chr];
        uint32_t r = 0, lo = k, hi = k + 1;
        if (multi) {
            r = t_read[k];
            lo = read_off[r];
            hi = read_off[r + 1];
        }
        uint32_t meta = ((fl & 3u) << kMetaBaseShift) | (tail ? kMetaTail : 0u) | (multi ? kRecMulti : 0u);
        uint32_t masks = 0, bases = 0;
        for (uint32_t j = k; j-- > lo;) {
            const uint32_t dist = l - read_locus[j];
            if (dist > kNarrowWindow) meta |= kRecWide;
            if (dist > kWindow) {
                meta |= kMetaPrevOvf;
                break;
            }
            masks |= 1u << (dist - 1);
        }
        for (uint32_t j = k + 1; j < hi; ++j) {
            const uint32_t dist = read_locus[j] - l;
            if (dist > kNarrowWindow) meta |= kRecWide;
            if (dist > kWindow) {
                meta |= kMetaNextOvf;
                break;
            }
            masks |= 1u << (16 + dist - 1);
            bases |= (uint32_t)(read_base[j] & 1u) << (dist - 1);
            bases |= (uint32_t)((read_base[j] >> 1) & 1u) << (16 + dist - 1);
        }
        m_rec[k] = make_uint4(meta, masks, bases, r);
        n_wide += (meta & kRecWide) ? 1u : 0u;
    }
    if (n_wide) atomicAdd(&sc->n_wide, n_wide);
}

struct RecordTables {
    const uint4 *m_rec;
    const uint32_t *locus_rel;
    uint4 *entry;
    uint32_t *entry32, *mask32, *entry_read;
};

__device__ __forceinline__ bool emit_record(const RecordTables &t, uint32_t d, uint32_t k, uint4 rec, uint32_t cib,
                                            uint32_t cell, uint32_t l, uint32_t lrel) {
    uint32_t base, meta, masks = 0, bases = 0, r = 0;
    bool multi = false, wide = false, tail;
    if (k & kSingle) {
        base = k & 3u;
        tail = (k & kSingleTail) != 0u;
        meta = cell | (base << kMetaBaseShift) | (tail ? kMetaTail : 0u);
    } else {
        base = (rec.x >> kMetaBaseShift) & 3u;
        tail = (rec.x & kMetaTail) != 0u;
        multi = (rec.x & kRecMulti) != 0u;
        wide = (rec.x & kRecWide) != 0u;
        meta = cell | (rec.x & ~(kRecMulti | kRecWide));
        masks = rec.y;
        bases = rec.z;
        r = rec.w;
    }
    if (multi || tail) {
        t.entry[d] = make_uint4(meta, masks, bases, l);
        t.entry_read[d] = r;
    }
    t.entry32[d] = cib | (base << kC_BaseShift) | (tail ? kC_Tail : 0u) | (multi ? kC_Multi : 0u)
            | (wide ? kC_Wide : 0u) | (lrel << 16);
    if (t.mask32)
        t.mask32[d] = (masks & 0xFFu) | (((masks >> 16) & 0xFFu) << 8) | ((bases & 0xFFu) << 16)
                | (((bases >> 16) & 0xFFu) << 24);
    return multi || tail;
}

constexpr int TPB_REC = 512;
__global__ __launch_bounds__(TPB_REC) void k_entry_records(const unsigned long long *grouped, const uint32_t *blk_off,
                                                          uint32_t n, uint32_t nb, uint32_t L, uint32_t B,
                                                          uint32_t lbits, RecordTables t,
                                                          unsigned long long *per_cell_sq, Scalars *sc,
                                                          unsigned long long *chunk_mask, uint32_t *block_sum) {
    constexpr uint32_t SLOTS = 512;
    __shared__ unsigned long long sq[SLOTS];
    __shared__ uint32_t blk_start[1025];
    __shared__ uint32_t first_cell;
    __shared__ uint32_t n_flagged;
    constexpr int U = 4;
    static_assert(kFlagBlock % (TPB_REC * U) == 0, "whole rounds per block of the lists");
    const uint32_t d0 = blockIdx.x * kFlagBlock, d1 = min(n, d0 + kFlagBlock);
    if (threadIdx.x == 0) n_flagged = 0;
    for (uint32_t i = threadIdx.x; i < SLOTS; i += TPB_REC) sq[i] = 0;
    for (uint32_t i = threadIdx.x; i <= nb; i += TPB_REC) blk_start[i] = i < nb ? blk_off[(size_t)i * (L + 1)] : n;
    __syncthreads();
    auto block_of = [&](uint32_t p) {
        uint32_t lo = 0, hi = nb;
        while (hi - lo > 1) {
            const uint32_t mid = (lo + hi) >> 1;
            if (blk_start[mid] <= p) lo = mid; else hi = mid;
        }
        return lo;
    };
    if (threadIdx.x == 0 && d0 < n) first_cell = block_of(d0) * B;
    __syncthreads();
    const uint32_t lmask = (1u << lbits) - 1u;
    uint32_t wave_flagged = 0;
    for (uint32_t base = d0; base < d0 + kFlagBlock; base += TPB_REC * U) {
        if (base >= d1 && !chunk_mask) break;
        unsigned long long mine[U];
        uint32_t blk[U], linfo[U], same[U];
        uint4 rec[U];
#pragma unroll
        for (int u = 0; u < U; ++u) {
            const uint32_t p = base + (uint32_t)u * TPB_REC + threadIdx.x;
            mine[u] = p < d1 ? grouped[p] : (unsigned long long)kSingle;
        }
#pragma unroll
        for (int u = 0; u < U; ++u) {
            const uint32_t p = base + (uint32_t)u * TPB_REC + threadIdx.x;
            const uint32_t l = (uint32_t)(mine[u] >> (32 + kCibBits)) & lmask;
            blk[u] = p < d1 ? block_of(p) : 0u;
            linfo[u] = t.locus_rel[l];
            rec[u] = make_uint4(0u, 0u, 0u, 0u);
            if (((uint32_t)mine[u] & kSingle) == 0u) rec[u] = t.m_rec[(uint32_t)mine[u]];
        }
#pragma unroll
        for (int u = 0; u < U; ++u) {
            const uint32_t p = base + (uint32_t)u * TPB_REC + threadIdx.x;
            same[u] = 1;
            if (p < d1 && (linfo[u] & kLocusDup)) {
                const uint32_t l = (uint32_t)(mine[u] >> (32 + kCibBits)) & lmask;
                const uint32_t cib = (uint32_t)(mine[u] >> 32) & ((1u << kCibBits) - 1u);
                const size_t g = (size_t)blk[u] * (L + 1) + l;
                const uint32_t gb = blk_off[g], ge = blk_off[g + 1];
                if (ge - gb > kRankScanLimit) {
                    sc->regroup = 1;
                } else if (ge - gb > 1) {
                    same[u] = 0;
                    for (uint32_t q = gb; q < ge; ++q)
                        same[u] += ((uint32_t)(grouped[q] >> 32) & ((1u << kCibBits) - 1u)) == cib ? 1u : 0u;
                }
            }
        }
#pragma unroll
        for (int u = 0; u < U; ++u) {
            const uint32_t p = base + (uint32_t)u * TPB_REC + threadIdx.x;
            bool flagged = false;
            if (p < d1) {
                const uint32_t k = (uint32_t)mine[u], cib = (uint32_t)(mine[u] >> 32) & ((1u << kCibBits) - 1u);
                const uint32_t l = (uint32_t)(mine[u] >> (32 + kCibBits)) & lmask;
                const uint32_t cell = blk[u] * B + cib;
                flagged = emit_record(t, p, k, rec[u], cib, cell, l, linfo[u] & 0xFFFFu);
                const uint32_t rel = cell - first_cell;
                if (rel < SLOTS) atomicAdd(&sq[rel], (unsigned long long)same[u]);
                else atomicAdd(&per_cell_sq[cell], (unsigned long long)same[u]);
            }
            if (chunk_mask) {
                const unsigned long long m = __ballot(flagged);
                wave_flagged += (uint32_t)__popcll(m);
                if ((threadIdx.x & 63u) == 0u) chunk_mask[p >> 6] = m;
            }
        }
    }
    if (chunk_mask && (threadIdx.x & 63u) == 0u && wave_flagged) atomicAdd(&n_flagged, wave_flagged);
    __syncthreads();
    if (block_sum && threadIdx.x == 0) block_sum[blockIdx.x] = n_flagged;
    if (d0 < n)
        for (uint32_t i = threadIdx.x; i < SLOTS; i += TPB_REC)
            if (sq[i]) atomicAdd(&per_cell_sq[first_cell + i], sq[i]);
}

__global__ __launch_bounds__(TPB) void k_pair_bound(const unsigned long long *per_cell_sq, uint32_t n_cells_padded,
                                                   CapChoice caps, uint32_t assumed_counts, Scalars *sc) {
    __shared__ unsigned long long s_best[TPB / 64];
    unsigned long long best = 0;
    for (uint32_t i = threadIdx.x; i < n_cells_padded; i += TPB) best = max(best, per_cell_sq[i]);
    for (int off = 32; off > 0; off >>= 1) best = max(best, (unsigned long long)__shfl_down(best, off));
    if ((threadIdx.x & 63) == 0) s_best[threadIdx.x >> 6] = best;
    __syncthreads();
    if (threadIdx.x == 0) {
        for (int w = 1; w < TPB / 64; ++w) best = max(best, s_best[w]);
        sc->pair_bound = max(sc->pair_bound, best);
        sc->caps_wrong = (assumed_counts && !caps.counts(sc)) ? 1u : 0u;
    }
}

__global__ __launch_bounds__(TPB) void k_fix_locus_rel(const uint32_t *blk_off, uint32_t nb, uint32_t L,
                                                      const uint32_t *locus_rel, uint32_t *entry32) {
    const uint32_t n_groups = nb * (L + 1);
    for (uint32_t g = blockIdx.x * TPB + threadIdx.x; g < n_groups; g += gridDim.x * TPB) {
        const uint32_t l = g % (L + 1);
        if (l == L) continue;
        const uint32_t b = blk_off[g], e = blk_off[g + 1];
        if (b == e) continue;
        const uint32_t lrel = (locus_rel[l] & 0xFFFFu) << 16;
        for (uint32_t d = b; d < e; ++d) entry32[d] = (entry32[d] & 0xFFFFu) | lrel;
    }
}

int bits_for(unsigned long long max_value) {
    int b = 1;
    while (b < 64 && (max_value >> b) != 0) ++b;
    return b;
}


struct Attempt {
    enum Kind { Go, Done, NeedHost, RetryRadix, RetryPlain, Error } kind = Go;
    std::string text;
    bool go() const { return kind == Go; }
    static Attempt stop(Kind k) {
        Attempt a;
        a.kind = k;
        return a;
    }
    static Attempt error(std::string t) {
        Attempt a;
        a.kind = Error;
        a.text = std::move(t);
        return a;
    }
};

#define HIP_OK(expr)                                                                                      \
    do {                                                                                                  \
        hipError_t e__ = (expr);                                                                          \
        if (e__ != hipSuccess) return Attempt::error(std::string(#expr) + ": " + hipGetErrorString(e__)); \
    } while (0)
#define STEP(expr)                  \
    do {                            \
        Attempt a__ = (expr);       \
        if (!a__.go()) return a__;  \
    } while (0)

Attempt scalar_verdict(const Scalars &h, bool records_written) {
    if (records_written) {
        if (h.error == 1) return Attempt::error("group id outside group_id_to_pos");
        if (h.error == 2) return Attempt::error("group_id_to_pos maps outside the matrix");
        if (h.regroup) return Attempt::stop(Attempt::RetryRadix);
        return h.need_host ? Attempt::stop(Attempt::NeedHost) : Attempt();
    }
    if (h.error == 3) return Attempt::error("positions must be strictly increasing within a chromosome");
    if (h.id_exceeded) return Attempt::stop(Attempt::RetryPlain);
    if (h.regroup) return Attempt::stop(Attempt::RetryRadix);
    return h.need_host ? Attempt::stop(Attempt::NeedHost) : Attempt();
}

struct Grouped : Attempt {
    Grouped() = default;
    Grouped(Attempt a) : Attempt(std::move(a)) {}
    unsigned long long *skey = nullptr;
    uint32_t *sval = nullptr, *sloc = nullptr;
    Raw sub{};
    uint32_t n_m = 0;
    MIndex m_index{nullptr, nullptr};
    const uint32_t *m_entry = nullptr;
    bool counting = false;
    bool single_entry = false;
    bool abandoned = false;
};

struct ReadViews {
    uint32_t *keep;
    unsigned long long *incl;
    MarksRanksCounts marks;
    Runs runs;
    uint32_t *mark_sub, *arank_m;
    Ranks ranks;
    uint32_t *read_off, *read_locus;
    uint8_t *read_base;
};

struct TilePlan {
    uint32_t B, nb, B_log2, lbits;
    bool stage_masks;
    CapChoice caps;
    uint32_t n_seg;
    size_t variant_stride;
    uint32_t TL, locus_grid;
    size_t lds;
};
TilePlan plan_tiles(uint32_t num_cells, uint32_t L, uint32_t block_cells, StageGeometry (*geometry)(uint32_t),
                    bool allow_count_tile, uint32_t n_kept, uint64_t multi_entries) {
    TilePlan p;
    if (block_cells == 0) {
        const StageGeometry g64 = geometry(64);
        const bool clustered = n_kept && (double)multi_entries > g64.masks_threshold * (double)n_kept;
        block_cells = (clustered || num_cells <= 64) ? 64 : 128;
    }
    const StageGeometry geo = geometry(block_cells);
    p.B = block_cells;
    p.nb = (num_cells + p.B - 1) / p.B;
    p.B_log2 = p.B == 64 ? 6u : 7u;
    p.lbits = (uint32_t)bits_for(L - 1);
    p.stage_masks = n_kept && (double)multi_entries > geo.masks_threshold * (double)n_kept;
    CapChoice &caps = p.caps;
    caps.entries_plain = p.stage_masks ? geo.cap_entries_masks : geo.cap_entries_plain;
    caps.loci_plain = p.stage_masks ? geo.cap_loci_masks : geo.cap_loci_plain;
    caps.entries_counts = geo.cap_entries_counts;
    caps.loci_counts = geo.cap_loci_counts;
    caps.count_limit = kCountTileLimit;
    caps.allow_counts = (allow_count_tile && !p.stage_masks) ? 1u : 0u;
    if (caps.allow_counts && n_kept && L) {
        const double density = (double)n_kept / ((double)num_cells / p.B) / (double)L;
        const double per_segment = density * caps.loci_counts / caps.entries_counts;
        if (per_segment > 1.0) {
            const double greedy = std::ceil((double)L / caps.loci_counts) * std::ceil(per_segment);
            const uint32_t one = std::max(64u, (uint32_t)(0.93 * caps.entries_counts / density));
            if (one < caps.loci_counts && std::ceil((double)L / one) * 1.05 < greedy) caps.loci_counts = one;
        }
    }
    const uint32_t lo_loci = caps.allow_counts ? std::min(caps.loci_plain, caps.loci_counts) : caps.loci_plain;
    const uint32_t hi_loci = caps.allow_counts ? std::max(caps.loci_plain, caps.loci_counts) : caps.loci_plain;
    p.n_seg = (L + lo_loci - 1) / lo_loci;
    p.variant_stride = (size_t)p.n_seg * hi_loci + p.n_seg + 2;
    p.TL = 64;
    while (p.TL > 1 && (size_t)p.nb * (p.TL + 1) * 4 > 32768) p.TL >>= 1;
    p.locus_grid = std::min<uint32_t>((L + p.TL - 1) / p.TL, 8192);
    p.lds = (size_t)p.nb * (p.TL + 1) * 4;
    return p;
}

struct Stage5 {
    TilePlan p;
    uint32_t n_kept, kept_m;
    size_t n_off;
    uint32_t *t_read, *krank, *blk_off, *blk_cnt;
    uint8_t *kflags, *dupflag;
    unsigned long long *entry_kc;
    BinRadix bin;
    uint4 *m_rec;
    unsigned long long *per_cell_sq;
    Segs segs;
};

struct PackAttempt {
    const DeviceFlatPileup &in;
    const uint32_t num_cells, mfl, num_threads, block_cells;
    StageGeometry (*const geometry)(uint32_t);
    const bool allow_count_tile, force_radix, no_assumptions, overlap;
    const hipStream_t stream;
    DevicePacked &pk;
    DeviceArena *const S;
    const uint32_t E, L, C;
    const PackShape shape;
    const Raw raw;
    const int ids_aligned;
    HostTrace trace;
    MiscViews<Scalars> m{nullptr, PackShape{0, 0, 0, 0}};
    Scalars *sc = nullptr;
    void *cub_tmp = nullptr;

    PackAttempt(const DeviceFlatPileup &in_, uint32_t num_cells_, uint32_t mfl_, uint32_t num_threads_,
                uint32_t block_cells_, StageGeometry (*geometry_)(uint32_t), bool allow_count_tile_, bool force_radix_,
                bool no_assumptions_, bool overlap_, hipStream_t stream_, DevicePacked &pk_)
        : in(in_), num_cells(num_cells_), mfl(mfl_), num_threads(num_threads_), block_cells(block_cells_),
          geometry(geometry_), allow_count_tile(allow_count_tile_), force_radix(force_radix_),
          no_assumptions(no_assumptions_), overlap(overlap_), stream(stream_), pk(pk_), S(pk_.scratch),
          E(static_cast<uint32_t>(in_.n_entries)), L(in_.n_loci), C(in_.n_chr), shape{E, L, C, num_cells_},
          raw{in_.chr_locus_off, C, in_.locus_pos, in_.locus_entry_off, in_.read_ids, in_.id_base16, in_.id_base32,
              in_.group_id_to_pos, in_.n_groups, L, E},
          ids_aligned((reinterpret_cast<uintptr_t>(in_.read_ids) & 15u) == 0 ? 1 : 0) {}

    hipError_t ensure(Arena::Id a, size_t id_slots = 0) { return S[a].ensure(arena_bytes<Scalars>(a, shape, id_slots)); }
    template <class T>
    hipError_t exclusive_sum(const T &in_it, uint32_t *out, size_t n) {
        size_t cub_cap = S[Arena::CUB].bytes;
        return hipcub::DeviceScan::ExclusiveSum(cub_tmp, cub_cap, in_it, out, (int)n, stream);
    }

    Attempt prepare_workspace() {
        for (Arena::Id a : {Arena::MISC, Arena::KEY_A, Arena::KEY_B, Arena::VAL_A, Arena::VAL_B, Arena::WORK_A,
                            Arena::WORK_B, Arena::RUNS, Arena::ENTRY_KC, Arena::TMP, Arena::BIN})
            HIP_OK(ensure(a));
        m = MiscViews<Scalars>(S[Arena::MISC].p, shape);
        sc = m.sc;
        {
            unsigned long long *key_a = UnsortedKeys(S[Arena::KEY_A].p, E), *key_b = SortedKeys(S[Arena::KEY_B].p, E);
            uint32_t *val_a = GroupedIds(S[Arena::VAL_A].p, E), *val_b = SortedValues(S[Arena::VAL_B].p, E);
            size_t need = 0, most = 0;
            HIP_OK(hipcub::DeviceRadixSort::SortPairs(nullptr, need, key_a, key_b, val_a, val_b, (int)E, 0, 64, stream));
            most = std::max(most, need);
            {
                hipcub::CountingInputIterator<uint32_t> positions(0u);
                hipcub::TransformInputIterator<unsigned long long, HeadKeepOp, hipcub::CountingInputIterator<uint32_t>>
                        flags(positions, HeadKeepOp{key_b, val_a, val_a});
                HIP_OK(hipcub::DeviceScan::InclusiveSum(nullptr, need, flags, key_a, (int)E, stream));
                most = std::max(most, need);
            }
            HIP_OK(hipcub::DeviceScan::ExclusiveSum(nullptr, need, val_a, val_b, (int)E + 1, stream));
            most = std::max(most, need);
            HIP_OK(hipcub::DeviceScan::ExclusiveSum(nullptr, need, val_a, val_b,
                                                    (int)std::max<size_t>(shape.n_off_max(), id_space_cap() + 2), stream));
            most = std::max(most, need);
            HIP_OK(S[Arena::CUB].ensure(most + 1024));
        }
        cub_tmp = S[Arena::CUB].p;
        HIP_OK(hipMemsetAsync(sc, 0, m.zeroed, stream));
        if (!pk.side) {
            HIP_OK(hipStreamCreateWithFlags(&pk.side, hipStreamNonBlocking));
            HIP_OK(hipEventCreateWithFlags(&pk.ev_fork, hipEventDisableTiming));
            HIP_OK(hipEventCreateWithFlags(&pk.ev_join, hipEventDisableTiming));
            HIP_OK(hipEventCreateWithFlags(&pk.ev_offsets, hipEventDisableTiming));
            HIP_OK(hipEventCreateWithFlags(&pk.ev_flush, hipEventDisableTiming));
        }
        return Attempt();
    }
    size_t id_space_cap() const { return std::min<size_t>((size_t)kIdSpaceFactor * E + 1024, (size_t)1 << 30); }

    Attempt make_entry_locus() {
        HIP_OK(ensure(Arena::ELOC));
        hipLaunchKernelGGL(k_entry_locus, dim3(blocks_for((uint64_t)L * 64)), dim3(TPB), 0, stream, raw,
                           EntryLocus(S[Arena::ELOC].p, E).p, sc);
        return Attempt();
    }
    Grouped whole_pileup(bool counting) const {
        Grouped g;
        g.skey = SortedKeys(S[Arena::KEY_B].p, E), g.sval = SortedValues(S[Arena::VAL_B].p, E);
        g.sloc = SortedLoci(S[Arena::ENTRY_KC].p, E);
        g.sub = raw;
        g.n_m = E;
        g.counting = counting;
        return g;
    }

    Grouped group_by_read() {
        hipLaunchKernelGGL(k_id_range, dim3(std::min<uint32_t>(256, (E + 4095) / 4096)), dim3(TPB), 0, stream, raw,
                           m.id_max, m.id_negmin, ids_aligned, sc);
        const bool assume = !force_radix && !no_assumptions && pk.id_space_hint && pk.id_space_hint <= id_space_cap();
        hipLaunchKernelGGL(k_id_bases, dim3(1), dim3(64), 0, stream, raw, m.id_max, m.id_negmin, m.id_base, m.chr_entry,
                           (unsigned long long)(assume ? pk.id_space_hint : 0), sc);
        Scalars hsc;
        std::memset(&hsc, 0, sizeof(hsc));
        if (!assume) {
            HIP_OK(read_scalars(pk, stream, sc, nullptr, &hsc, nullptr));
            STEP(scalar_verdict(hsc, false));
        }
        const size_t id_space = assume ? (size_t)pk.id_space_hint
                                       : (size_t)std::min<unsigned long long>(hsc.id_space, 1ull << 40);
        const bool counting = !force_radix && id_space <= id_space_cap();
        HIP_OK(ensure(Arena::WORK_A, counting ? id_space + 1 : 0));
        HIP_OK(ensure(Arena::WORK_B, counting ? id_space + 1 : 0));
        if (!pk.split_pays && ++pk.calls_without_split >= 16) {
            pk.split_pays = true;
            pk.calls_without_split = 0;
        }
        if (!(counting && pk.split_pays)) {
            STEP(make_entry_locus());
            return counting ? group_by_read_counting(id_space, false) : group_by_read_radix(hsc.max_read_id);
        }
        Grouped g = group_by_read_single_entry(id_space);
        if (!g.abandoned) return g;
        pk.split_pays = false;
        pk.calls_without_split = 0;
        return group_by_read_counting(id_space, true);
    }

    Grouped group_by_read_single_entry(size_t id_space) {
        const uint32_t n_flag_blocks = (uint32_t)shape.flag_blocks();
        const size_t n_chunks = shape.chunks();
        uint32_t *last = IdSlots(S[Arena::WORK_A].p, id_space + 1);
        HIP_OK(ensure(Arena::M_CHUNKS));
        const MChunks chunks(S[Arena::M_CHUNKS].p, shape);
        HIP_OK(ensure(Arena::MARK_M));
        uint8_t *multi = MultiFlags(S[Arena::MARK_M].p, shape.flag_bytes());
        HIP_OK(hipMemsetAsync(multi, 0, shape.flag_bytes(), stream));
        hipLaunchKernelGGL(k_id_store, dim3(blocks_for((E + 3) / 4)), dim3(TPB), 0, stream, raw, m.chr_entry, m.id_base,
                           m.id_negmin, sc, last, ids_aligned);
        hipLaunchKernelGGL(k_id_check, dim3(blocks_for((E + 3) / 4)), dim3(TPB), 0, stream, raw, m.chr_entry, m.id_base,
                           m.id_negmin, sc, last, multi, ids_aligned);
        for (Arena::Id a : {Arena::M_ENTRY, Arena::RID_M, Arena::IDB_M, Arena::ELOC_M, Arena::ARANK_M, Arena::DENSE_M})
            HIP_OK(ensure(a));
        uint32_t *m_entry = PerM(S[Arena::M_ENTRY].p, E), *rid_m = PerM(S[Arena::RID_M].p, E);
        uint32_t *idb_m = PerM(S[Arena::IDB_M].p, E), *eloc_m = PerM(S[Arena::ELOC_M].p, E);
        const FlagBlockSums sums(S[Arena::VAL_A].p, shape);
        hipLaunchKernelGGL(k_flag_count, dim3(n_flag_blocks), dim3(TPB), 0, stream, multi, sums.block_sum);
        hipLaunchKernelGGL(k_flag_scan, dim3(1), dim3(TPB_SCAN), 0, stream, sums.block_sum, n_flag_blocks, sums.block_off,
                           chunks.chunk_pre + (n_chunks - 1), sc);
        hipLaunchKernelGGL(k_compact_m, dim3(n_flag_blocks), dim3(TPB), 0, stream, raw, multi, sums.block_off,
                           chunks.chunk_pre, chunks.chunk_mask, m_entry);
        Scalars hsc;
        HIP_OK(read_scalars(pk, stream, sc, nullptr, &hsc, nullptr));
        STEP(scalar_verdict(hsc, false));
        Grouped g = whole_pileup(true);
        g.n_m = hsc.n_multi_id;
        if ((uint64_t)g.n_m * 2 > E) {
            g.abandoned = true;
            return g;
        }
        g.single_entry = true;
        g.m_index = MIndex{chunks.chunk_pre, chunks.chunk_mask};
        g.m_entry = m_entry;
        g.sub.read_ids = rid_m;
        g.sub.id_base16 = nullptr;
        g.sub.id_base32 = idb_m;
        g.sub.n_entries = g.n_m;
        if (g.n_m) {
            const uint32_t n_m = g.n_m;
            const MReads r(S[Arena::DENSE_M].p, n_m);
            HIP_OK(hipMemsetAsync(r.count_m, 0, ((size_t)n_m + 1) * 4, stream));
            hipLaunchKernelGGL(k_m_fields, dim3(blocks_for(n_m)), dim3(TPB), 0, stream, raw, m.chr_entry, m.id_base,
                               m.id_negmin, last, g.m_index, m_entry, n_m, rid_m, idb_m, eloc_m, r.winner_m, r.count_m);
            HIP_OK(exclusive_sum(r.count_m, r.goff, (size_t)n_m + 1));
            hipLaunchKernelGGL(k_group_scatter, dim3(blocks_for(n_m)), dim3(TPB), 0, stream, r.winner_m, n_m, r.goff,
                               r.count_m, r.members, r.g_begin, r.g_len);
            hipLaunchKernelGGL(k_group_rank, dim3(blocks_for(n_m)), dim3(TPB), 0, stream, g.sub, r.members, r.g_begin,
                               r.g_len, eloc_m, n_m, g.skey,
                               g.sval, g.sloc, sc);
        }
        return g;
    }

    Grouped group_by_read_counting(size_t id_space, bool single_entry_abandoned) {
        Grouped g = whole_pileup(true);
        uint32_t *hist = IdSlots(S[Arena::WORK_A].p, id_space + 1), *id_off = IdOffsets(S[Arena::WORK_B].p, id_space + 1);
        uint32_t *grouped = GroupedIds(S[Arena::VAL_A].p, E), *dense = DenseIds(S[Arena::KEY_A].p, E);
        HIP_OK(hipMemsetAsync(hist, 0, (id_space + 1) * 4, stream));
        if (single_entry_abandoned) STEP(make_entry_locus());
        const uint32_t *eloc = EntryLocus(S[Arena::ELOC].p, E);
        hipLaunchKernelGGL(k_id_hist, dim3(blocks_for(E)), dim3(TPB), 0, stream, raw, eloc, m.id_base, m.id_negmin, sc,
                           dense, hist);
        HIP_OK(exclusive_sum(hist, id_off, id_space + 1));
        hipLaunchKernelGGL(k_id_scatter, dim3(blocks_for(E)), dim3(TPB), 0, stream, dense, E, id_off, sc, hist, grouped);
        hipLaunchKernelGGL(k_id_rank, dim3(blocks_for(E)), dim3(TPB), 0, stream, raw, dense, id_off, grouped, eloc,
                           g.skey, g.sval, g.sloc, sc);
        return g;
    }

    Grouped group_by_read_radix(uint32_t max_read_id) {
        Grouped g = whole_pileup(false);
        unsigned long long *key_a = UnsortedKeys(S[Arena::KEY_A].p, E);
        uint32_t *val_a = GroupedIds(S[Arena::VAL_A].p, E);
        const uint32_t *eloc = EntryLocus(S[Arena::ELOC].p, E);
        const uint32_t id_bits = (uint32_t)bits_for(max_read_id);
        hipLaunchKernelGGL(k_entry_keys, dim3(blocks_for(E)), dim3(TPB), 0, stream, raw, eloc, id_bits, key_a, val_a);
        size_t cub_cap = S[Arena::CUB].bytes;
        HIP_OK(hipcub::DeviceRadixSort::SortPairs(cub_tmp, cub_cap, key_a, g.skey, val_a,
                                                   g.sval, (int)E, 0, (int)id_bits + bits_for(C),
                                                   stream));
        hipLaunchKernelGGL(k_sorted_locus, dim3(blocks_for(E)), dim3(TPB), 0, stream, raw, g.sval, eloc, E, g.sloc);
        return g;
    }

    Attempt ensure_outputs() {
        const size_t n_off_max = shape.n_off_max();
        HIP_OK(pk.read_off.ensure(((size_t)E + 1) * 4));
        HIP_OK(pk.read_locus.ensure((size_t)E * 4));
        HIP_OK(pk.read_base.ensure(E));
        HIP_OK(pk.range_off.ensure(((size_t)L + 2) * 4));
        HIP_OK(pk.entry.ensure((size_t)E * 16));
        HIP_OK(pk.entry32.ensure((size_t)E * 4));
        HIP_OK(pk.mask32.ensure((size_t)E * 4));
        HIP_OK(pk.entry_read.ensure((size_t)E * 4));
        HIP_OK(pk.blk_off.ensure((n_off_max + 1) * 4));
        return Attempt();
    }
    ReadViews read_views(const Grouped &g) const {
        const MarksRanksCounts marks(S[Arena::KEY_A].p, shape);
        return ReadViews{KeepFlags(S[Arena::WORK_A].p, (size_t)E + 1),
                         InclSums(S[Arena::WORK_B].p, (size_t)E + 1),
                         marks,
                         Runs(S[Arena::RUNS].p, shape),
                         g.single_entry ? MarksOfM(S[Arena::MARK_M].p, (size_t)E + 2).p : nullptr,
                         g.single_entry ? PerM(S[Arena::ARANK_M].p, E).p : nullptr,
                         Ranks{g.m_index, g.single_entry ? marks.arank : nullptr, marks.arank},
                         pk.read_off.as<uint32_t>(),
                         pk.read_locus.as<uint32_t>(),
                         pk.read_base.as<uint8_t>()};
    }
    Attempt build_reads(const Grouped &g, const ReadViews &v, const uint32_t *split) {
        const uint32_t n_m = g.n_m;
        uint32_t *mark_sub = g.single_entry ? v.mark_sub : v.marks.mark, *arank = v.marks.arank;
        if (n_m) {
            hipLaunchKernelGGL(k_dup_mark, dim3(blocks_for(n_m)), dim3(TPB), 0, stream, g.sub, g.skey, g.sval, g.sloc, split,
                               n_m, v.keep, mark_sub);
            hipcub::CountingInputIterator<uint32_t> positions(0u);
            hipcub::TransformInputIterator<unsigned long long, HeadKeepOp, hipcub::CountingInputIterator<uint32_t>>
                    flags(positions, HeadKeepOp{g.skey, v.keep, split});
            size_t cub_cap = S[Arena::CUB].bytes;
            HIP_OK(hipcub::DeviceScan::InclusiveSum(cub_tmp, cub_cap, flags, v.incl, (int)n_m, stream));
        }
        const uint32_t *arank_sub = arank;
        if (g.single_entry) {
            hipcub::CountingInputIterator<uint32_t> entries(0u);
            hipcub::TransformInputIterator<uint32_t, UnmarkedM, hipcub::CountingInputIterator<uint32_t>> unmarked(
                    entries, UnmarkedM{mark_sub, n_m});
            HIP_OK(exclusive_sum(unmarked, arank, (size_t)n_m + 1));
            hipLaunchKernelGGL(k_arank_m, dim3(blocks_for(std::max(n_m, 1u))), dim3(TPB), 0, stream, arank, g.m_entry, n_m,
                               E, v.arank_m, sc);
            arank_sub = v.arank_m;
            hipLaunchKernelGGL(k_rbeg, dim3(1), dim3(TPB), 0, stream, raw, v.ranks, m.rbeg);
        } else {
            HIP_OK(exclusive_sum(v.marks.mark, arank, (size_t)E + 1));
        }
        if (n_m) {
            hipLaunchKernelGGL(k_runs_csr, dim3(blocks_for(n_m)), dim3(TPB), 0, stream, g.sub, v.incl, g.sval, g.sloc, n_m,
                               v.runs.run_start, v.read_locus, v.read_base);
            hipLaunchKernelGGL(k_read_info, dim3(std::min<uint32_t>(blocks_for(n_m), 2048)), dim3(TPB), 0, stream, g.sub,
                               v.incl, v.runs.run_start, g.sval, g.sloc, arank_sub, mfl, v.runs.run_rank,
                               g.single_entry ? nullptr : m.rbeg, v.read_off, sc);
        }
        HIP_OK(hipEventRecord(pk.ev_fork, stream));
        HIP_OK(hipStreamWaitEvent(pk.side, pk.ev_fork, 0));
        hipLaunchKernelGGL(k_completed, dim3(blocks_for(L)), dim3(TPB), 0, pk.side, raw, v.ranks, m.rbeg, mfl, m.cnt, sc);
        hipLaunchKernelGGL(k_flush_chain, dim3(C), dim3(TPB), 0, pk.side, raw, m.cnt, 4u * num_threads, sc, m.flushed,
                           m.flush_loci, m.flush_count, v.ranks, m.rbeg, g.single_entry ? m.tail_begin : nullptr);
        HIP_OK(hipEventRecord(pk.ev_flush, pk.side));
        HIP_OK(hipEventRecord(pk.ev_join, pk.side));
        return Attempt();
    }
    Attempt settle_flush_cuts(const Grouped &g, const ReadViews &v, Scalars *hsc, unsigned long long *totals) {
        const uint32_t n_m = g.n_m;
        uint32_t *split = SplitFlags(S[Arena::TMP].p, E);
        HIP_OK(hipMemsetAsync(split, 0, (size_t)std::max(n_m, 1u) * 4, stream));
        for (int round = 0; round < kMaxSplitRounds; ++round) {
            HIP_OK(hipStreamWaitEvent(stream, pk.ev_join, 0));
            HIP_OK(hipMemsetAsync(&sc->split_changed, 0, 4, stream));
            hipLaunchKernelGGL(k_split_update, dim3(blocks_for(n_m)), dim3(TPB), 0, stream, g.sub, g.skey, g.sloc, mfl,
                               m.flush_loci, m.flush_count, split, sc);
            HIP_OK(read_scalars(pk, stream, sc, nullptr, hsc, nullptr));
            if (!hsc->split_changed) return Attempt();
            HIP_OK(hipMemsetAsync(&sc->multi_entries, 0, 8, stream));
            STEP(build_reads(g, v, split));
            HIP_OK(read_scalars(pk, stream, sc, n_m ? v.incl + (n_m - 1) : nullptr, hsc, totals));
        }
        return Attempt::stop(Attempt::NeedHost);
    }

    void launch_ranges_segment(const Stage5 &s, hipStream_t on) {
        hipLaunchKernelGGL(k_ranges_segment, dim3(s.p.n_seg, s.p.caps.allow_counts ? 2u : 1u), dim3(TPB), 0, on, s.blk_off,
                           s.p.nb, L, s.p.caps, s.segs.seg_ends, s.segs.seg_count, s.p.variant_stride);
    }
    Attempt cut_ranges_on_side(const Stage5 &s) {
        HIP_OK(hipEventRecord(pk.ev_offsets, stream));
        HIP_OK(hipStreamWaitEvent(pk.side, pk.ev_offsets, 0));
        launch_ranges_segment(s, pk.side);
        HIP_OK(hipEventRecord(pk.ev_join, pk.side));
        return Attempt();
    }
    Attempt m_records_on_side(const Stage5 &s, const ReadViews &v) {
        hipLaunchKernelGGL(k_m_records, dim3(blocks_for(s.kept_m)), dim3(TPB), 0, pk.side, raw, s.kept_m, s.t_read,
                           v.read_off, v.read_locus, v.read_base, s.krank, s.kflags, m.rbeg, m.flushed,
                           s.m_rec, sc);
        HIP_OK(hipEventRecord(pk.ev_join, pk.side));
        return Attempt();
    }
    void pick_ranges(const Stage5 &s, uint32_t sq_rows, int assumed, const uint8_t *dupflag) {
        hipLaunchKernelGGL(k_ranges_compact, dim3(1), dim3(TPB), 0, stream, s.segs.seg_ends, s.segs.seg_count,
                           s.p.variant_stride, s.p.n_seg, s.p.caps, pk.range_off.as<uint32_t>(), s.per_cell_sq, sq_rows,
                           assumed, sc);
        if (s.n_kept)
            hipLaunchKernelGGL(k_locus_info, dim3(blocks_for(L)), dim3(TPB), 0, stream, raw, pk.range_off.as<uint32_t>(),
                               sc, dupflag, m.locus_chr, m.locus_rel);
    }

    Attempt bin_radix(const Stage5 &s) {
        const BinRadix &b = s.bin;
        if (s.n_kept) {
            size_t cub_cap = S[Arena::CUB].bytes;
            HIP_OK(hipcub::DeviceRadixSort::SortPairs(cub_tmp, cub_cap, b.key2_a, b.key2_b, b.val2_a, b.val2_b,
                                                       (int)s.n_kept, 0, (int)(kCibBits + s.p.lbits) + bits_for(s.p.nb - 1),
                                                       stream));
            hipLaunchKernelGGL(k_group_counts, dim3(std::min<uint32_t>(2048, (s.n_kept + 4095) / 4096)), dim3(TPB), 0,
                               stream, b.key2_b, s.n_kept, s.p.B, L, s.p.lbits, s.blk_cnt, s.per_cell_sq);
        }
        HIP_OK(exclusive_sum(s.blk_cnt, s.blk_off, s.n_off));
        return cut_ranges_on_side(s);
    }
    Attempt bin_counting(const Grouped &g, const ReadViews &v, const Stage5 &s, bool hist_first) {
        const TilePlan &p = s.p;
        if (!hist_first)
            hipLaunchKernelGGL(k_bin_hist, dim3(p.locus_grid), dim3(TPB), p.lds, stream, raw, p.nb, p.TL, s.entry_kc, nullptr,
                               num_cells, p.B_log2, s.blk_cnt, sc, 0u);
        trace.mark("k_bin_hist launched");
        const bool records_first = s.kept_m && (uint64_t)s.kept_m * 4u > (uint64_t)s.n_kept;
        if (records_first) {
            HIP_OK(hipEventRecord(pk.ev_offsets, stream));
            HIP_OK(hipStreamWaitEvent(pk.side, pk.ev_offsets, 0));
            STEP(m_records_on_side(s, v));
        }
        HIP_OK(exclusive_sum(s.blk_cnt, s.blk_off, s.n_off));
        trace.mark("offset scan launched");
        if (records_first) {
            launch_ranges_segment(s, stream);
        } else {
            STEP(cut_ranges_on_side(s));
            if (s.kept_m) STEP(m_records_on_side(s, v));
        }
        if (s.n_kept) {
            HIP_OK(hipStreamWaitEvent(stream, pk.ev_flush, 0));
            uint32_t bm_words = (p.nb * p.B + 31) / 32;
            if (p.lds + (size_t)(TPB / 64) * bm_words * 4 > 49152) bm_words = 0;
            hipLaunchKernelGGL(k_bin_place, dim3(p.locus_grid), dim3(TPB), p.lds + (size_t)(TPB / 64) * bm_words * 4, stream,
                               raw, p.nb, p.TL, s.entry_kc, s.blk_off, p.B_log2, bm_words,
                               g.single_entry ? m.tail_begin : nullptr, GroupedKept(S[Arena::KEY_B].p, E).p, s.dupflag);
        }
        return Attempt();
    }
    void records_radix(const ReadViews &v, const Stage5 &s) {
        const BinRadix &b = s.bin;
        pick_ranges(s, s.n_kept ? s.p.nb * s.p.B : 0u, -1, nullptr);
        if (s.n_kept)
            hipLaunchKernelGGL(k_records, dim3(blocks_for(s.n_kept)), dim3(TPB), 0, stream, raw, b.key2_b, b.val2_b, s.n_kept,
                               s.t_read, v.read_off, v.read_locus, v.read_base, s.krank, s.kflags, m.rbeg, m.flushed,
                               m.locus_chr, m.locus_rel, s.p.B, s.p.lbits, pk.entry.as<uint4>(), pk.entry32.as<uint32_t>(),
                               pk.stage_masks ? pk.mask32.as<uint32_t>() : nullptr, pk.entry_read.as<uint32_t>(), sc);
    }
    bool records_counting(const Stage5 &s) {
        const TilePlan &p = s.p;
        const int assumed = p.caps.allow_counts ? 1 : 0;
        bool lists_here = false;
        pick_ranges(s, 0u, assumed, s.dupflag);
        if (s.n_kept) {
            const RecordTables tables{s.m_rec, m.locus_rel, pk.entry.as<uint4>(), pk.entry32.as<uint32_t>(),
                                      pk.stage_masks ? pk.mask32.as<uint32_t>() : nullptr, pk.entry_read.as<uint32_t>()};
            lists_here = overlap && p.caps.allow_counts && !pk.stage_masks && pk.flag_lists.scratch;
            const FlagScratch fs(pk.flag_lists.scratch, s.n_kept);
            hipLaunchKernelGGL(k_entry_records, dim3((s.n_kept + kFlagBlock - 1) / kFlagBlock), dim3(TPB_REC), 0, stream,
                               GroupedKept(S[Arena::KEY_B].p, E).p, s.blk_off, s.n_kept, p.nb, L, p.B, p.lbits, tables,
                               s.per_cell_sq, sc, lists_here ? fs.chunk_mask : nullptr, lists_here ? fs.block_sum : nullptr);
        }
        hipLaunchKernelGGL(k_pair_bound, dim3(1), dim3(TPB), 0, stream, s.per_cell_sq, s.n_kept ? p.nb * p.B : 0u, p.caps,
                           (uint32_t)assumed, sc);
        return lists_here;
    }
    Attempt close_attempt(const Stage5 &s, bool lists_launched) {
        const TilePlan &p = s.p;
        Scalars hsc;
        trace.mark("records launched");
        HIP_OK(read_scalars(pk, stream, sc, nullptr, &hsc, nullptr, [&] {
            if (lists_launched)
                flag_lists_from_masks(FlagScratch(pk.flag_lists.scratch, s.n_kept), pk.entry.as<uint4>(), s.blk_off, s.n_off,
                                      pk.flag_lists.grp, pk.flag_lists.rec, pk.flag_lists.idx, stream);
        }));
        trace.mark("read-back 3 arrived");
        if (!force_radix && hsc.caps_wrong && !hsc.regroup && hsc.error == 0) {
            pick_ranges(s, 0u, 0, nullptr);
            if (s.n_kept)
                hipLaunchKernelGGL(k_fix_locus_rel, dim3(blocks_for(s.n_off)), dim3(TPB), 0, stream, s.blk_off, p.nb, L,
                                   m.locus_rel, pk.entry32.as<uint32_t>());
            HIP_OK(read_scalars(pk, stream, sc, nullptr, &hsc, nullptr));
        }
        const Attempt verdict = scalar_verdict(hsc, true);
        if (verdict.kind == Attempt::NeedHost) HIP_OK(hipStreamSynchronize(stream));
        STEP(verdict);
        pk.pair_bound = hsc.pair_bound;
        pk.cell_sq = s.per_cell_sq;
        pk.cell_sq_n = s.n_kept ? p.nb * p.B : 0u;
        pk.cell_sq_host.clear();
        pk.count_tile = p.caps.allow_counts && pk.pair_bound < kCountTileLimit;
        pk.cap_entries = pk.count_tile ? p.caps.entries_counts : p.caps.entries_plain;
        pk.cap_loci = pk.count_tile ? p.caps.loci_counts : p.caps.loci_plain;
        pk.num_ranges = hsc.num_ranges;
        pk.max_range_span = hsc.max_range_span;
        pk.n_wide = hsc.n_wide;
        pk.flag_lists_built = lists_launched;
        HIP_OK(hipGetLastError());
        return Attempt::stop(Attempt::Done);
    }

    Attempt run() {
        STEP(prepare_workspace());
        trace.t0 = std::chrono::steady_clock::now();
        trace.mark("begin");
        const Grouped g = group_by_read();
        if (!g.go()) return g;
        pk.used_single_entry = g.single_entry;

        STEP(ensure_outputs());
        const ReadViews v = read_views(g);
        STEP(build_reads(g, v, nullptr));
        struct SideJoin {
            hipStream_t side;
            bool joined = false;
            ~SideJoin() { if (!joined) (void)hipStreamSynchronize(side); }
        } side_join{pk.side};

        Scalars hsc;
        unsigned long long totals = 0;
        trace.mark("reads built (launched)");
        HIP_OK(read_scalars(pk, stream, sc, g.n_m ? v.incl + (g.n_m - 1) : nullptr, &hsc, &totals));
        trace.mark("read-back 2 arrived");
        const Attempt verdict = scalar_verdict(hsc, false);
        if (verdict.go() || verdict.kind == Attempt::RetryRadix || verdict.kind == Attempt::NeedHost)
            pk.id_space_hint = g.counting ? std::max<uint64_t>(hsc.id_space, 1) : 0;
        STEP(verdict);
        if (hsc.long_reads) STEP(settle_flush_cuts(g, v, &hsc, &totals));

        const uint32_t kept_m = (uint32_t)(totals >> 32);
        const uint32_t R = g.single_entry ? hsc.reads_total : (uint32_t)totals;
        const uint32_t n_kept = g.single_entry ? kept_m + (E - g.n_m) : kept_m;
        pk.multi_entries = hsc.multi_entries;
        pk.max_read_entries = std::max(hsc.max_read_entries, n_kept ? 1u : 0u);
        const TilePlan p = plan_tiles(num_cells, L, block_cells, geometry, allow_count_tile, n_kept, pk.multi_entries);
        if (p.B != 64 && p.B != 128) return Attempt::error("block_cells must be 64 or 128");
        if (!force_radix && (p.lbits + kCibBits > 32u || E >= kSingle)) return Attempt::stop(Attempt::RetryRadix);
        pk.num_cells = num_cells;
        pk.block_cells = p.B;
        pk.num_blocks = p.nb;
        pk.num_loci = L;
        pk.num_entries = n_kept;
        pk.num_reads = R;
        pk.stage_masks = p.stage_masks;

        HIP_OK(ensure(Arena::DUPF));
        HIP_OK(S[Arena::SEGS].ensure(carved<Segs>((size_t)p.n_seg, p.variant_stride)));
        const size_t nk = std::max<uint32_t>(n_kept, 1), rows = (size_t)p.nb * p.B;
        const BinRadix bin(S[Arena::BIN].p, nk, rows);
        const Stage5 s{p,
                       n_kept,
                       kept_m,
                       (size_t)p.nb * ((size_t)L + 1),
                       KeptRead(S[Arena::TMP].p, E),
                       KeptRank(S[Arena::WORK_A].p, E),
                       pk.blk_off.as<uint32_t>(),
                       v.marks.blk_cnt,
                       KeptFlags(S[Arena::VAL_A].p, E),
                       DupFlags(S[Arena::DUPF].p, L),
                       force_radix ? nullptr : EntryKC(S[Arena::ENTRY_KC].p, E).p,
                       bin,
                       reinterpret_cast<uint4 *>(BinCounting(S[Arena::BIN].p, nk, rows).m_rec),
                       bin.per_cell_sq,
                       Segs(S[Arena::SEGS].p, p.n_seg, p.variant_stride)};
        if (force_radix) HIP_OK(hipMemsetAsync(s.blk_cnt, 0, (s.n_off + 1) * 4, stream));
        HIP_OK(hipMemsetAsync(s.per_cell_sq, 0, (rows + 1) * 8, stream));
        const bool hist_first = g.single_entry && !force_radix;
        if (hist_first) {
            const size_t g2p_bytes = ((size_t)in.n_groups * 2 + 15) / 16 * 16;
            const bool g2p_lds = num_cells <= 0xFFFFu && p.lds + g2p_bytes <= 49152;
            hipLaunchKernelGGL(k_bin_hist, dim3(g2p_lds ? std::min<uint32_t>(p.locus_grid, 1024) : p.locus_grid), dim3(TPB),
                               p.lds + (g2p_lds ? g2p_bytes : 0), stream, raw, p.nb, p.TL, s.entry_kc, g.m_index.chunk_mask,
                               num_cells, p.B_log2, s.blk_cnt, sc, g2p_lds ? 1u : 0u);
        }
        if (g.n_m) {
            hipLaunchKernelGGL(k_keys2, dim3(blocks_for(g.n_m)), dim3(TPB), 0, stream, g.sub, g.sval, v.incl, v.read_locus,
                               v.runs.run_rank, v.read_off, num_cells, p.B, p.lbits, force_radix ? bin.key2_a : nullptr,
                               force_radix ? bin.val2_a : nullptr, s.t_read, s.krank, s.kflags, s.entry_kc,
                               g.single_entry ? g.m_entry : nullptr, hist_first ? s.blk_cnt : nullptr, L, sc);
        }
        trace.mark("k_keys2 launched");
        STEP(force_radix ? bin_radix(s) : bin_counting(g, v, s, hist_first));
        HIP_OK(hipStreamWaitEvent(stream, pk.ev_join, 0));
        side_join.joined = true;
        bool lists_launched = false;
        if (force_radix)
            records_radix(v, s);
        else
            lists_launched = records_counting(s);
        return close_attempt(s, lists_launched);
    }
};

}

std::string pack_pileup_device(const DeviceFlatPileup &in, uint32_t num_cells, uint32_t mfl,
                               uint32_t num_threads, uint32_t block_cells,
                               StageGeometry (*geometry)(uint32_t), bool allow_count_tile,
                               hipStream_t stream, DevicePacked *out, bool *need_host) {
    *need_host = false;
    out->flag_lists_built = false;
    out->used_single_entry = false;
    out->route = DevicePacked::Route();
    if ((in.id_base16 != nullptr) == (in.id_base32 != nullptr))
        return "exactly one of id_base16 / id_base32 must be given";
    if (num_threads == 0) return "num_threads must be positive";
    if (num_cells == 0 || num_cells > 65535) return "num_cells must be in [1, 65535]";
    if (block_cells != 0 && block_cells != 64 && block_cells != 128) return "block_cells must be 0, 64 or 128";
    const uint64_t E64 = in.n_entries;
    const uint32_t L = in.n_loci;
    const size_t n_off_max = (size_t)((num_cells + 63) / 64) * ((size_t)L + 1);
    if (E64 >= (1ull << 31) || L == 0 || L >= (1u << 30) || E64 == 0 || (uint64_t)4 * num_threads > 0xFFFFFFFFull
        || n_off_max >= (1ull << 31)) {
        *need_host = out->route.asked_host = true;
        return std::string();
    }
    bool force_radix = false;
    if (const char *env = std::getenv("SECEDO_PACK_GROUPING")) force_radix = std::string(env) == "radix";
    bool overlap = true;
    if (const char *env = std::getenv("SECEDO_PACK_OVERLAP")) overlap = std::atoi(env) != 0;
    bool no_assumptions = false;
    for (int attempt = 0; attempt < 3; ++attempt) {
        if (poison_level() >= 2) {
            if (hipStreamSynchronize(stream) != hipSuccess || (out->side && hipStreamSynchronize(out->side) != hipSuccess))
                return "poison: synchronise failed";
            DeviceArena *outputs[] = {&out->blk_off, &out->entry32, &out->mask32, &out->entry,
                                      &out->entry_read, &out->range_off, &out->read_off, &out->read_locus, &out->read_base};
            for (DeviceArena *a : outputs)
                if (a->p && hipMemset(a->p, 0xA5, a->bytes) != hipSuccess) return "poison: memset failed";
            for (DeviceArena &a : out->scratch)
                if (a.p && hipMemset(a.p, 0xA5, a.bytes) != hipSuccess) return "poison: memset failed";
        }
        ++out->route.attempts;
        out->route.radix = force_radix;
        Attempt result = PackAttempt(in, num_cells, mfl, num_threads, block_cells, geometry, allow_count_tile, force_radix,
                                     no_assumptions, overlap, stream, *out).run();
        switch (result.kind) {
            case Attempt::Error: return std::move(result.text);
            case Attempt::NeedHost: *need_host = out->route.asked_host = true; return std::string();
            case Attempt::RetryRadix: force_radix = true; break;
            case Attempt::RetryPlain:
                no_assumptions = out->route.retried_plain = true;
                out->id_space_hint = 0;
                break;
            default: return std::string();
        }
    }
    *need_host = out->route.asked_host = true;
    return std::string();
}


size_t flag_list_scratch_bytes(uint32_t n_entries) { return FlagScratch::bytes(n_entries); }

hipError_t pack_flag_lists(const uint32_t *entry32, const uint4 *entry, uint32_t n_entries, const uint32_t *blk_off,
                           size_t n_off, void *scratch, uint32_t *grp, uint4 *rec, uint32_t *idx, hipStream_t stream) {
    const FlagScratch fs(scratch, n_entries);
    hipLaunchKernelGGL(k_pflag_count, dim3(fs.nb), dim3(TPB), 0, stream, entry32, n_entries, fs.block_sum);
    hipLaunchKernelGGL(k_flag_scan, dim3(1), dim3(TPB_SCAN), 0, stream, fs.block_sum, fs.nb, fs.block_off,
                       fs.chunk_pre + 64 * (size_t)fs.nb, static_cast<Scalars *>(nullptr));
    hipLaunchKernelGGL(k_pflag_compact, dim3(fs.nb), dim3(TPB), 0, stream, entry32, entry, n_entries, fs.block_off, rec, idx,
                       fs.chunk_pre, fs.chunk_mask);
    flag_groups(fs, blk_off, n_off, grp, stream);
    return hipGetLastError();
}

}
```

secedo_amd/csrc/simmat_api.cpp:

```cpp
#include "simmat_handle.hpp"

#include <algorithm>
#include <cstdio>
#include <new>
#include <utility>

using namespace secedo::host;

namespace {

void note_pileup(secedo_simmat *h, uint32_t n_chr, uint64_t n_loci, uint64_t n_entries, const void *read_ids) {
    Fnv1a id;
    for (uint64_t v : {(uint64_t)n_chr, n_loci, n_entries, (uint64_t)reinterpret_cast<uintptr_t>(read_ids)}) id.add(v);
    h->pileup_identity = id.id();
    if (h->override_identity != h->pileup_identity) {
        if (h->pair_bound_override || h->max_shared_override) h->override_dropped = true;
        h->pair_bound_override = 0;
        h->max_shared_override = 0;
        h->override_identity = 0;
    }
}

int check_pileup_args(const secedo_simmat *h, const void *chr_locus_off, const void *locus_entry_off,
                      const void *id_base16, const void *id_base32, const void *group_id_to_pos, uint32_t n_groups) {
    if (!h) return fail(SECEDO_E_INVALID_ARG, "handle is null");
    if (!chr_locus_off || !locus_entry_off) return fail(SECEDO_E_INVALID_ARG, "null offset arrays");
    if ((id_base16 != nullptr) == (id_base32 != nullptr))
        return fail(SECEDO_E_INVALID_ARG, "exactly one of id_base16 / id_base32 must be given");
    if (!group_id_to_pos && n_groups) return fail(SECEDO_E_INVALID_ARG, "group_id_to_pos is null");
    return SECEDO_OK;
}


struct HostPileupStore {
    std::vector<uint32_t> chr, pos, rid, g2p, idb32;
    std::vector<uint64_t> off;
    std::vector<uint16_t> idb16;
};
int fetch_pileup_to_host(const secedo::DeviceFlatPileup &d, hipStream_t s, HostPileupStore *store,
                         secedo::FlatPileupView *v) {
    SECEDO_TRY(hipStreamSynchronize(s));
    auto fetch = [](auto &to, const void *d_src, size_t n) {
        to.resize(n);
        return n ? hipMemcpy(to.data(), d_src, n * sizeof(to[0]), hipMemcpyDeviceToHost) : hipSuccess;
    };
    SECEDO_TRY(fetch(store->chr, d.chr_locus_off, (size_t)d.n_chr + 1));
    SECEDO_TRY(fetch(store->pos, d.locus_pos, d.n_loci));
    SECEDO_TRY(fetch(store->off, d.locus_entry_off, (size_t)d.n_loci + 1));
    SECEDO_TRY(fetch(store->rid, d.read_ids, d.n_entries));
    SECEDO_TRY(fetch(store->g2p, d.group_id_to_pos, d.n_groups));
    if (d.id_base16) SECEDO_TRY(fetch(store->idb16, d.id_base16, d.n_entries));
    else SECEDO_TRY(fetch(store->idb32, d.id_base32, d.n_entries));
    static const uint16_t none16 = 0;
    static const uint32_t none32 = 0;
    *v = secedo::FlatPileupView{store->chr.data(), d.n_chr, store->pos.data(), store->off.data(), store->rid.data(),
                                d.id_base16 ? (store->idb16.empty() ? &none16 : store->idb16.data()) : nullptr,
                                d.id_base16 ? nullptr : (store->idb32.empty() ? &none32 : store->idb32.data()),
                                store->g2p.data(), d.n_groups};
    return SECEDO_OK;
}

int adopt_host_packing(secedo::PackedPileup &from, secedo::DevicePacked *pk) {
    SECEDO_TRY(pk->blk_off.upload(from.blk_off));
    SECEDO_TRY(pk->entry32.upload(from.entry32));
    SECEDO_TRY(pk->mask32.upload(from.mask32));
    SECEDO_TRY(pk->entry.upload(from.entry));
    SECEDO_TRY(pk->entry_read.upload(from.entry_read));
    SECEDO_TRY(pk->range_off.upload(from.range_off));
    SECEDO_TRY(pk->read_off.upload(from.read_off));
    SECEDO_TRY(pk->read_locus.upload(from.read_locus));
    SECEDO_TRY(pk->read_base.upload(from.read_base));
    pk->num_cells = from.num_cells;
    pk->block_cells = from.block_cells;
    pk->num_blocks = from.num_blocks;
    pk->num_loci = from.num_loci;
    pk->num_entries = from.num_entries;
    pk->num_reads = from.num_reads;
    pk->pair_bound = from.pair_bound;
    pk->cell_sq = nullptr;
    pk->cell_sq_n = 0;
    pk->cell_sq_host = std::move(from.cell_sq);
    pk->multi_entries = from.multi_entries;
    pk->max_read_entries = from.max_read_entries;
    pk->n_wide = from.n_wide;
    pk->flag_lists_built = false;
    pk->stage_masks = from.stage_masks;
    pk->count_tile = from.count_tile;
    pk->cap_entries = from.cap_entries;
    pk->cap_loci = from.cap_loci;
    pk->num_ranges = static_cast<uint32_t>(from.range_off.size()) - 1;
    pk->max_range_span = 0;
    for (size_t r = 0; r + 1 < from.range_off.size(); ++r)
        pk->max_range_span = std::max(pk->max_range_span, from.range_off[r + 1] - from.range_off[r]);
    return SECEDO_OK;
}

struct PrepareArgs {
    uint32_t num_cells, max_fragment_length, num_threads, block_cells;
    bool allow_count_tile;
    int mode;
};

int pack_on_device(secedo_simmat *h, const PrepareArgs &p, hipStream_t s, bool *need_host) {
    if (h->have_host) SECEDO_TRY(upload_flat_pileup(h->view, h->raw, &h->dview));
    h->pk.flag_lists = secedo::DevicePacked::FlagListBuffers();
    const bool was_clustered = h->pk.stage_masks && h->pk.num_entries;
    if (p.allow_count_tile && !was_clustered && h->dview.n_entries && h->dview.n_entries < (1ull << 31)) {
        const uint32_t ne = (uint32_t)h->dview.n_entries;
        const size_t n_off_max = (size_t)((p.num_cells + 63) / 64) * ((size_t)h->dview.n_loci + 1);
        SECEDO_TRY(h->flag_tmp.ensure(secedo::flag_list_scratch_bytes(ne)));
        SECEDO_TRY(h->flag_rec.ensure((size_t)ne * 16));
        SECEDO_TRY(h->flag_idx.ensure((size_t)ne * 4));
        SECEDO_TRY(h->flag_grp.ensure(std::max<size_t>(n_off_max, 1) * 4));
        h->pk.flag_lists.scratch = h->flag_tmp.p;
        h->pk.flag_lists.grp = h->flag_grp.as<uint32_t>();
        h->pk.flag_lists.rec = h->flag_rec.as<uint4>();
        h->pk.flag_lists.idx = h->flag_idx.as<uint32_t>();
    }
    const std::string err = secedo::pack_pileup_device(h->dview, p.num_cells, p.max_fragment_length, p.num_threads,
                                                       p.block_cells, &secedo::stage_geometry, p.allow_count_tile, s,
                                                       &h->pk, need_host);
    if (!err.empty()) {
        h->have_host = h->have_device = false;
        return fail(err.find("hip") == 0 ? SECEDO_E_HIP : SECEDO_E_INVALID_ARG, err);
    }
    if (*need_host && p.mode == 2) {
        h->have_host = h->have_device = false;
        return fail(SECEDO_E_LIMIT, "this pileup needs the host packing path (a read is longer than "
                                    "max_fragment_length, or a size limit of the device path)");
    }
    if (!*need_host) h->used_device_packing = 1;
    return SECEDO_OK;
}

int pack_on_host(secedo_simmat *h, const PrepareArgs &p, hipStream_t s) {
    HostPileupStore store;
    secedo::FlatPileupView v = h->view;
    if (!h->have_host) SECEDO_CALL(fetch_pileup_to_host(h->dview, s, &store, &v));
    secedo::PackedPileup packed;
    const std::string err = secedo::pack_pileup(v, p.num_cells, p.max_fragment_length, p.num_threads, p.block_cells,
                                                &secedo::stage_geometry, p.allow_count_tile, &packed);
    if (!err.empty()) {
        h->have_host = h->have_device = false;
        return fail(SECEDO_E_INVALID_ARG, err);
    }
    return adopt_host_packing(packed, &h->pk);
}

int build_tile_table(secedo_simmat *h) {
    const uint32_t nb = h->pk.num_blocks;
    if (h->num_tiles == nb * (nb + 1) / 2 && h->tile_row.p) return SECEDO_OK;
    h->num_tiles = nb * (nb + 1) / 2;
    std::vector<uint16_t> trow, tcol;
    trow.reserve(h->num_tiles);
    tcol.reserve(h->num_tiles);
    for (uint32_t i = 0; i < nb; ++i) {
        for (uint32_t j = i; j < nb; ++j) {
            trow.push_back(static_cast<uint16_t>(i));
            tcol.push_back(static_cast<uint16_t>(j));
        }
    }
    SECEDO_TRY(h->tile_row.upload(trow));
    SECEDO_TRY(h->tile_col.upload(tcol));
    h->host_tile_row = trow;
    h->host_tile_col = tcol;
    return SECEDO_OK;
}

int build_flag_lists(secedo_simmat *h, hipStream_t s) {
    const secedo::DevicePacked &pk = h->pk;
    if (!(pk.count_tile && !pk.stage_masks && pk.num_entries)) {
        if (pk.stage_masks) {
            for (secedo_simmat::DevBuf *b : {&h->flag_tmp, &h->flag_rec, &h->flag_idx, &h->flag_grp}) b->release();
            h->pk.flag_lists = secedo::DevicePacked::FlagListBuffers();
        }
        return SECEDO_OK;
    }
    if (h->used_device_packing && pk.flag_lists_built) {
        h->flags_ready = true;
        return SECEDO_OK;
    }
    const uint32_t ne = (uint32_t)pk.num_entries;
    const size_t n_off = (size_t)pk.num_blocks * (pk.num_loci + 1);
    SECEDO_TRY(h->flag_tmp.ensure(secedo::flag_list_scratch_bytes(ne)));
    SECEDO_TRY(h->flag_rec.ensure((size_t)ne * 16));
    SECEDO_TRY(h->flag_idx.ensure((size_t)ne * 4));
    SECEDO_TRY(h->flag_grp.ensure(std::max<size_t>(n_off, 1) * 4));
    SECEDO_TRY(secedo::pack_flag_lists(pk.entry32.as<uint32_t>(), pk.entry.as<uint4>(), ne, pk.blk_off.as<uint32_t>(),
                                       n_off, h->flag_tmp.p, h->flag_grp.as<uint32_t>(), h->flag_rec.as<uint4>(),
                                       h->flag_idx.as<uint32_t>(), s));
    h->flags_ready = true;
    return SECEDO_OK;
}

int print_stamps(secedo_simmat *h) {
    const unsigned long long *counters = h->counters.as<unsigned long long>();
    const bool counts = env_set("SECEDO_STAMPS_COUNTS");
    unsigned long long st[16] = {0};
    SECEDO_TRY(hipMemcpy(st, counters, sizeof(st), hipMemcpyDeviceToHost));
    if (counts) {
        unsigned long long cf[11] = {0};
        SECEDO_TRY(hipMemcpy(cf, counters + 82, sizeof(cf), hipMemcpyDeviceToHost));
        if (cf[0])
            std::fprintf(stderr, "[stamps-correct] pair tests %llu, tail terms %llu, joint terms %llu, later-locus pairs %llu | "
                                 "per wave: pairs phase %.0f cycles (%.0f until the first q records are there), flush phase %.0f cycles, "
                                 "flagged row entries %.0f; busiest lane: %.1f q iterations, %.0f cycles until their records are there\n",
                         cf[0], cf[1], cf[2], cf[3], (double)cf[4] / (double)cf[6], (double)cf[8] / (double)cf[6],
                         (double)cf[5] / (double)cf[6], (double)cf[7] / (double)cf[6], (double)cf[10] / (double)cf[6],
                         (double)cf[9] / (double)cf[6]);
    }
    if (st[8] && counts) {
        const double w = (double)st[8];
        std::fprintf(stderr, "[stamps-counts] sampled waves %llu | per wave cycles: total %.0f barrier-A %.0f stage+barrier-B %.0f "
                             "items(+col prefetch issue) %.0f primary groups %.0f drain %.0f | per primary batch %.0f, per drain batch %.0f "
                             "(%.2f drain batches per primary batch)\n",
                     st[8], st[7] / w, st[2] / w, st[3] / w, st[4] / w, st[5] / w, st[6] / w,
                     (double)st[5] / std::max<double>(1, (double)st[9]), (double)st[6] / std::max<double>(1, (double)st[10]),
                     (double)st[10] / std::max<double>(1, (double)st[9]));
        unsigned long long pw[64] = {0};
        SECEDO_TRY(hipMemcpy(pw, counters + 16, sizeof(pw), hipMemcpyDeviceToHost));
        const double wgs = w / 16.0;
        for (int k = 0; k < 16; ++k)
            std::fprintf(stderr, "[stamps-counts] wave %2d: barrier-A %8.0f  pairs %8.0f  items %8.0f  stage+B %8.0f\n", k,
                         pw[k * 4] / wgs, pw[k * 4 + 1] / wgs, pw[k * 4 + 2] / wgs, pw[k * 4 + 3] / wgs);
    } else if (st[8]) {
        std::fprintf(stderr, "[stamps] waves %llu batches %llu trips %llu | per wave: lifetime %.0f cyc, setup %.0f, "
                             "fill %.0f, trips %.0f | per batch: setup %.0f fill %.0f trips %.0f (%.2f trips)\n",
                     st[8], st[5], st[6], (double)st[7] / st[8], (double)st[2] / st[8], (double)st[3] / st[8],
                     (double)st[4] / st[8], (double)st[2] / st[5], (double)st[3] / st[5], (double)st[4] / st[5],
                     (double)st[6] / st[5]);
        std::fprintf(stderr, "[stamps] per wave: barrier-1 wait %.0f, staging+barrier-2 %.0f, prefetch issue %.0f\n",
                     (double)st[9] / st[8], (double)st[10] / st[8], (double)st[11] / st[8]);
        std::fprintf(stderr, "[stamps] per wave: post-trip %.0f, batch loop total %.0f\n",
                     (double)st[12] / st[8], (double)st[13] / st[8]);
        std::fprintf(stderr, "[stamps] longest wave lifetime %llu cyc; ranges %u workgroups %u\n", st[14],
                     h->pk.num_ranges, h->plan_workgroups);
        std::vector<unsigned long long> wg(std::min<uint32_t>(h->plan_workgroups, 2048u));
        SECEDO_TRY(hipMemcpy(wg.data(), counters + 16, wg.size() * 8, hipMemcpyDeviceToHost));
        std::vector<unsigned long long> det(wg.size() * 8);
        SECEDO_TRY(hipMemcpy(det.data(), counters + 16 + 2048, det.size() * 8, hipMemcpyDeviceToHost));
        for (size_t k = 0; k < wg.size(); ++k)
            std::fprintf(stderr, "[stamps-wg] %zu %llu %llu %llu | hwid %llx ranges %llu listflush %llu endbarrier %llu slab %llu | realbegin %llu realend %llu batchloop %llu\n", k,
                         wg[k] & 0xFFFFFFFFull, (wg[k] >> 32) & 0xFFF, (wg[k] >> 44) & 0xFFF, det[k * 8], det[k * 8 + 1] / 1000,
                         det[k * 8 + 2] / 1000, det[k * 8 + 3] / 1000, det[k * 8 + 4] / 1000, det[k * 8 + 5], det[k * 8 + 6], det[k * 8 + 7] / 1000);
    }
    return SECEDO_OK;
}

}

int secedo::host::set_pileup_view(secedo_simmat *h, const secedo::FlatPileupView &v) {
    SECEDO_CALL(check_pileup_args(h, v.chr_locus_off, v.locus_entry_off, v.id_base16, v.id_base32, v.group_id_to_pos,
                                  v.n_groups));
    h->view = v;
    h->have_host = true;
    h->have_device = false;
    h->prepared = false;
    note_pileup(h, v.n_chr, v.n_loci(), v.n_entries(), v.read_ids);
    return SECEDO_OK;
}

int secedo::host::finalize_mode(secedo_simmat *h, int mode, const int64_t *d_acc, uint32_t row_begin, uint32_t row_end,
                                double *d_out, void *stream, bool keep_max) {
    SECEDO_CALL(check_ready(h, true, d_acc && d_out));
    SECEDO_CALL(check_row_range(h, row_begin, row_end));
    SECEDO_TRY(hipSetDevice(h->device));
    SECEDO_TRY(secedo::launch_finalize(d_acc, h->tile_row.as<uint16_t>(), h->tile_col.as<uint16_t>(), h->num_tiles,
                                       h->pk.num_cells, h->pk.block_cells, h->scale_log2, mode,
                                       h->max_bits.as<unsigned long long>(), row_begin, row_end, d_out,
                                       static_cast<hipStream_t>(stream), keep_max));
    return SECEDO_OK;
}

extern "C" {

const char *secedo_simmat_last_error(void) { return g_error.c_str(); }

const char *secedo_simmat_version(void) { return "secedo-simmat-mi355x 0.1 (gfx950)"; }

int secedo_simmat_device_count(void) {
    int n = 0;
    if (hipGetDeviceCount(&n) != hipSuccess) return 0;
    return n;
}

int secedo_simmat_normalization_from_string(const char *name) {
    if (name) {
        if (!std::strcmp(name, "ADD_MIN")) return SECEDO_NORM_ADD_MIN;
        if (!std::strcmp(name, "EXPONENTIATE")) return SECEDO_NORM_EXPONENTIATE;
        if (!std::strcmp(name, "SCALE_MAX_1")) return SECEDO_NORM_SCALE_MAX_1;
    }
    return fail(SECEDO_E_INVALID_NORMALIZATION,
                std::string("Invalid normalization: ") + (name ? name : "(null)"));
}

double secedo_simmat_llr(uint32_t x_s, uint32_t x_d, double eps, double h, double theta) {
    if (x_s + x_d >= 1 && !secedo::llr_exact_mode()) return secedo::reference_llr_any(eps, h, theta, x_s, x_d, 8);
    return secedo::llr(secedo::make_llr_model(eps, h, theta), x_s, x_d);
}

double secedo_simmat_llr_closed_form(uint32_t x_s, uint32_t x_d, double eps, double h, double theta) {
    return secedo::llr(secedo::make_llr_model(eps, h, theta), x_s, x_d);
}

int secedo_simmat_create(secedo_simmat_t **handle, int device_id) {
    if (!handle) return fail(SECEDO_E_INVALID_ARG, "handle is null");
    *handle = nullptr;
    const int n = secedo_simmat_device_count();
    if (n <= 0) return no_device("the similarity-matrix path");
    if (device_id < 0 || device_id >= n) return fail(SECEDO_E_NO_DEVICE, "device id out of range");
    SECEDO_TRY(hipSetDevice(device_id));
    secedo_simmat *h = new (std::nothrow) secedo_simmat();
    if (!h) return fail(SECEDO_E_LIMIT, "out of host memory");
    h->device = device_id;
    hipError_t e = hipEventCreate(&h->ev_begin);
    if (e == hipSuccess) e = hipEventCreate(&h->ev_end);
    if (e == hipSuccess) e = hipEventCreate(&h->ev_mid);
    if (e != hipSuccess) {
        delete h;
        return fail(SECEDO_E_HIP, std::string("hipEventCreate: ") + hipGetErrorString(e));
    }
    *handle = h;
    return SECEDO_OK;
}

void secedo_simmat_destroy(secedo_simmat_t *h) {
    if (!h) return;
    (void)hipSetDevice(h->device);
    if (h->ev_begin) (void)hipEventDestroy(h->ev_begin);
    if (h->ev_end) (void)hipEventDestroy(h->ev_end);
    if (h->ev_mid) (void)hipEventDestroy(h->ev_mid);
    h->uploads.destroy();
    delete h;
}

int secedo_simmat_set_pileup(secedo_simmat_t *h, const uint32_t *chr_locus_off, uint32_t n_chr,
                             const uint32_t *locus_pos, const uint64_t *locus_entry_off,
                             const uint32_t *read_ids, const uint16_t *id_base16,
                             const uint32_t *id_base32, const uint32_t *group_id_to_pos,
                             uint32_t n_groups) {
    return set_pileup_view(h, secedo::FlatPileupView{chr_locus_off, n_chr, locus_pos, locus_entry_off, read_ids,
                                                     id_base16, id_base32, group_id_to_pos, n_groups});
}

int secedo_simmat_set_pileup_device(secedo_simmat_t *h, const uint32_t *d_chr_locus_off, uint32_t n_chr,
                                    const uint32_t *d_locus_pos, const uint64_t *d_locus_entry_off,
                                    const uint32_t *d_read_ids, const uint16_t *d_id_base16,
                                    const uint32_t *d_id_base32, const uint32_t *d_group_id_to_pos,
                                    uint32_t n_groups, uint32_t n_loci, uint64_t n_entries) {
    SECEDO_CALL(check_pileup_args(h, d_chr_locus_off, d_locus_entry_off, d_id_base16, d_id_base32, d_group_id_to_pos,
                                  n_groups));
    h->dview = make_device_view(d_chr_locus_off, n_chr, d_locus_pos, d_locus_entry_off, d_read_ids, d_id_base16,
                                d_id_base32, d_group_id_to_pos, n_groups, n_loci, n_entries);
    h->have_device = true;
    h->have_host = false;
    h->prepared = false;
    note_pileup(h, n_chr, n_loci, n_entries, d_read_ids);
    return SECEDO_OK;
}

int secedo_simmat_set_packing(secedo_simmat_t *h, int mode) {
    if (!h) return fail(SECEDO_E_INVALID_ARG, "handle is null");
    if (mode < 0 || mode > 2) return fail(SECEDO_E_INVALID_ARG, "packing mode must be 0 (auto), 1 (host) or 2 (device)");
    h->packing_mode = mode;
    return SECEDO_OK;
}

int secedo_simmat_used_device_packing(const secedo_simmat_t *h) { return h ? h->used_device_packing : 0; }
int secedo_simmat_used_single_entry_path(const secedo_simmat_t *h) {
    return h && h->used_device_packing && h->pk.used_single_entry ? 1 : 0;
}
int secedo_simmat_packing_route(const secedo_simmat_t *h) {
    if (!h) return 0;
    const secedo::DevicePacked::Route &r = h->pk.route;
    return (int)(r.attempts & SECEDO_ROUTE_ATTEMPTS) | (r.radix ? SECEDO_ROUTE_RADIX : 0) |
           (r.retried_plain ? SECEDO_ROUTE_RETRIED_PLAIN : 0) | (r.asked_host ? SECEDO_ROUTE_ASKED_HOST : 0);
}

int secedo_simmat_prepare(secedo_simmat_t *h, uint32_t num_cells, uint32_t max_fragment_length,
                          uint32_t num_threads, uint32_t block_cells, void *stream) {
    if (!h) return fail(SECEDO_E_INVALID_ARG, "handle is null");
    if (!h->have_host && !h->have_device) return fail(SECEDO_E_STATE, "set_pileup was not called");
    if (block_cells == 0) {
        const int v = env_int("SECEDO_BLOCK_CELLS", 0);
        if (v == 64 || v == 128) block_cells = static_cast<uint32_t>(v);
    }
    PrepareArgs p{num_cells, max_fragment_length, num_threads, block_cells, env_enabled("SECEDO_COUNT_TILE"),
                  h->packing_mode};
    if (env_is("SECEDO_PACKING", "host")) p.mode = 1;
    if (env_is("SECEDO_PACKING", "device")) p.mode = 2;
    SECEDO_TRY(hipSetDevice(h->device));
    hipStream_t s = static_cast<hipStream_t>(stream);
    h->prepared = false;
    h->used_device_packing = 0;
    h->pk.route = secedo::DevicePacked::Route();
    h->num_threads = num_threads;

    bool need_host = (p.mode == 1);
    if (!need_host) SECEDO_CALL(pack_on_device(h, p, s, &need_host));
    if (need_host) SECEDO_CALL(pack_on_host(h, p, s));
    h->have_host = h->have_device = false;

    SECEDO_CALL(build_tile_table(h));
    SECEDO_TRY(h->counters.ensure((16 + 2048 * 9) * sizeof(unsigned long long)));
    SECEDO_TRY(h->max_bits.ensure(sizeof(unsigned long long)));
    SECEDO_TRY(hipMemsetAsync(h->counters.p, 0, 16 * sizeof(unsigned long long), s));
    h->prepared = true;
    h->timed = false;
    h->flags_ready = false;
    h->wide_known = false;
    return build_flag_lists(h, s);
}

uint32_t secedo_simmat_num_tiles(const secedo_simmat_t *h) { return h ? h->num_tiles : 0; }
uint32_t secedo_simmat_block_cells(const secedo_simmat_t *h) { return h ? h->pk.block_cells : 0; }
uint64_t secedo_simmat_acc_elems(const secedo_simmat_t *h) {
    return h ? static_cast<uint64_t>(h->num_tiles) * h->pk.block_cells * h->pk.block_cells : 0;
}
uint64_t secedo_simmat_num_entries(const secedo_simmat_t *h) { return h ? h->pk.num_entries : 0; }
uint64_t secedo_simmat_num_reads(const secedo_simmat_t *h) { return h ? h->pk.num_reads : 0; }
uint64_t secedo_simmat_num_loci(const secedo_simmat_t *h) { return h ? h->pk.num_loci : 0; }

uint64_t secedo_simmat_pair_bound(const secedo_simmat_t *h) { return h ? h->pk.pair_bound : 0; }
int secedo_simmat_scale_log2(const secedo_simmat_t *h) { return h ? h->scale_log2 : 0; }
uint32_t secedo_simmat_max_read_entries(const secedo_simmat_t *h) { return h ? h->pk.max_read_entries : 0; }
int secedo_simmat_set_scale_bounds(secedo_simmat_t *h, uint64_t pair_bound, uint32_t max_read_entries) {
    if (!h) return fail(SECEDO_E_INVALID_ARG, "handle is null");
    h->pair_bound_override = pair_bound;
    h->max_shared_override = max_read_entries;
    h->override_identity = (pair_bound || max_read_entries) ? h->pileup_identity : 0;
    h->override_dropped = false;
    return SECEDO_OK;
}
int secedo_simmat_scale_bounds_state(const secedo_simmat_t *h) {
    if (!h) return 0;
    if ((h->pair_bound_override || h->max_shared_override) && h->override_identity == h->pileup_identity) return 1;
    return h->override_dropped ? 2 : 0;
}
int secedo_simmat_set_pair_bound(secedo_simmat_t *h, uint64_t pair_bound) {
    return secedo_simmat_set_scale_bounds(h, pair_bound, h ? h->max_shared_override : 0);
}
int secedo_simmat_cell_squares(secedo_simmat_t *h, uint64_t *d_out, void *stream) {
    SECEDO_CALL(check_ready(h, false, d_out));
    SECEDO_TRY(hipSetDevice(h->device));
    hipStream_t s = static_cast<hipStream_t>(stream);
    const size_t n = h->pk.num_cells;
    SECEDO_TRY(hipMemsetAsync(d_out, 0, n * 8, s));
    if (h->pk.cell_sq && h->pk.cell_sq_n) {
        SECEDO_TRY(hipMemcpyAsync(d_out, h->pk.cell_sq, std::min<size_t>(n, h->pk.cell_sq_n) * 8, hipMemcpyDeviceToDevice, s));
    } else if (!h->pk.cell_sq_host.empty()) {
        SECEDO_TRY(hipMemcpyAsync(d_out, h->pk.cell_sq_host.data(), std::min(n, h->pk.cell_sq_host.size()) * 8,
                                  hipMemcpyHostToDevice, s));
        SECEDO_TRY(hipStreamSynchronize(s));
    }
    return SECEDO_OK;
}

int secedo_simmat_zero_acc(secedo_simmat_t *h, int64_t *d_acc, void *stream) {
    SECEDO_CALL(check_ready(h, false, d_acc));
    SECEDO_TRY(hipSetDevice(h->device));
    SECEDO_TRY(hipMemsetAsync(d_acc, 0, secedo_simmat_acc_elems(h) * sizeof(int64_t),
                              static_cast<hipStream_t>(stream)));
    return SECEDO_OK;
}

int secedo_simmat_tiles_of_rows(const secedo_simmat_t *h, uint32_t row_begin, uint32_t row_end, uint32_t *tile_ids,
                                uint32_t *n_tile_ids) {
    SECEDO_CALL(check_ready(h, false, n_tile_ids));
    SECEDO_CALL(check_row_range(h, row_begin, row_end));
    uint32_t n = 0;
    if (row_begin < row_end) {
        const uint32_t B = h->pk.block_cells, b0 = row_begin / B, b1 = (row_end - 1) / B;
        for (uint32_t t = 0; t < h->num_tiles; ++t) {
            const uint32_t I = h->host_tile_row[t], J = h->host_tile_col[t];
            if ((I >= b0 && I <= b1) || (J >= b0 && J <= b1)) {
                if (tile_ids) tile_ids[n] = t;
                ++n;
            }
        }
    }
    *n_tile_ids = n;
    return SECEDO_OK;
}

int secedo_simmat_max_of_tiles(secedo_simmat_t *h, const int64_t *d_acc, const uint32_t *tile_ids, uint32_t n_tile_ids,
                               double *max_value, void *stream) {
    SECEDO_CALL(check_ready(h, true, d_acc && max_value && (tile_ids || !n_tile_ids)));
    for (uint32_t k = 0; k < n_tile_ids; ++k)
        if (tile_ids[k] >= h->num_tiles) return fail(SECEDO_E_INVALID_ARG, "tile id outside [0, num_tiles)");
    SECEDO_TRY(hipSetDevice(h->device));
    hipStream_t s = static_cast<hipStream_t>(stream);
    DevBuf ids;
    SECEDO_TRY(ids.ensure((size_t)std::max(n_tile_ids, 1u) * 4));
    if (n_tile_ids) SECEDO_TRY(hipMemcpyAsync(ids.p, tile_ids, (size_t)n_tile_ids * 4, hipMemcpyHostToDevice, s));
    SECEDO_TRY(secedo::launch_tile_max(d_acc, h->tile_row.as<uint16_t>(), h->tile_col.as<uint16_t>(), ids.as<uint32_t>(),
                                       n_tile_ids, h->pk.block_cells, h->scale_log2, h->max_bits.as<unsigned long long>(),
                                       s));
    unsigned long long bits = 0;
    SECEDO_TRY(hipMemcpyAsync(&bits, h->max_bits.p, 8, hipMemcpyDeviceToHost, s));
    SECEDO_TRY(hipStreamSynchronize(s));
    std::memcpy(max_value, &bits, 8);
    return SECEDO_OK;
}

int secedo_simmat_finalize_rows_max(secedo_simmat_t *h, int normalization, const int64_t *d_acc, uint32_t row_begin,
                                    uint32_t row_end, double max_value, double *d_out_rows, void *stream) {
    SECEDO_CALL(check_normalization(normalization));
    SECEDO_CALL(check_ready(h, true, d_acc && d_out_rows));
    SECEDO_CALL(check_row_range(h, row_begin, row_end));
    if (!(max_value >= 0.0)) return fail(SECEDO_E_INVALID_ARG, "max_value must be the (non-negative) maximum of D");
    SECEDO_TRY(hipSetDevice(h->device));
    hipStream_t s = static_cast<hipStream_t>(stream);
    unsigned long long bits;
    std::memcpy(&bits, &max_value, 8);
    SECEDO_TRY(hipMemcpyAsync(h->max_bits.p, &bits, 8, hipMemcpyHostToDevice, s));
    SECEDO_TRY(hipStreamSynchronize(s));
    SECEDO_TRY(secedo::launch_finalize(d_acc, h->tile_row.as<uint16_t>(), h->tile_col.as<uint16_t>(), h->num_tiles,
                                       h->pk.num_cells, h->pk.block_cells, h->scale_log2, normalization,
                                       h->max_bits.as<unsigned long long>(), row_begin, row_end, d_out_rows, s, true));
    return SECEDO_OK;
}

int secedo_simmat_finalize(secedo_simmat_t *h, int normalization, const int64_t *d_acc, double *d_out,
                           void *stream) {
    SECEDO_CALL(check_normalization(normalization));
    return finalize_mode(h, normalization, d_acc, 0, h ? h->pk.num_cells : 0, d_out, stream);
}

int secedo_simmat_finalize_rows(secedo_simmat_t *h, int normalization, const int64_t *d_acc, uint32_t row_begin,
                                uint32_t row_end, double *d_out_rows, void *stream) {
    SECEDO_CALL(check_normalization(normalization));
    return finalize_mode(h, normalization, d_acc, row_begin, row_end, d_out_rows, stream);
}

int secedo_simmat_finalize_raw(secedo_simmat_t *h, const int64_t *d_acc, double *d_out, void *stream) {
    return finalize_mode(h, 3, d_acc, 0, h ? h->pk.num_cells : 0, d_out, stream);
}

int secedo_simmat_last_counts(secedo_simmat_t *h, uint64_t *updates, uint64_t *read_pairs) {
    if (!h) return fail(SECEDO_E_INVALID_ARG, "handle is null");
    SECEDO_CALL(check_ready(h, false));
    SECEDO_TRY(hipSetDevice(h->device));
    SECEDO_TRY(hipDeviceSynchronize());
    unsigned long long c[2] = {0, 0};
    SECEDO_TRY(hipMemcpy(c, h->counters.p, sizeof(c), hipMemcpyDeviceToHost));
    if (updates) *updates = c[0];
    if (read_pairs) *read_pairs = c[1];
    if (env_set("SECEDO_STAMPS_PRINT")) return print_stamps(h);
    return SECEDO_OK;
}

int secedo_simmat_last_accumulate_ms(secedo_simmat_t *h, float *ms) {
    if (!h || !ms) return fail(SECEDO_E_INVALID_ARG, "null argument");
    if (!h->timed) return fail(SECEDO_E_STATE, "accumulate was not called");
    SECEDO_TRY(hipSetDevice(h->device));
    SECEDO_TRY(hipEventSynchronize(h->ev_end));
    SECEDO_TRY(hipEventElapsedTime(ms, h->ev_begin, h->ev_end));
    return SECEDO_OK;
}

const char *secedo_simmat_pair_kernel(const secedo_simmat_t *h) {
    if (!h || !h->prepared) return "";
    if (h->pk.count_tile && !h->pk.stage_masks) return "accumulate_counts";
    return h->pk.stage_masks && h->pk.block_cells == 64 ? "accumulate_masks" : "accumulate_tiles";
}

int secedo_simmat_last_correction_fused(const secedo_simmat_t *h) { return h && h->last_fused ? 1 : 0; }

int secedo_simmat_last_locus_words(const secedo_simmat_t *h) { return h && h->last_locus_words ? 1 : 0; }

uint32_t secedo_simmat_last_workgroups(const secedo_simmat_t *h) { return h ? h->plan_workgroups : 0; }

int secedo_simmat_debug_flag_lists(secedo_simmat_t *h, uint64_t *n_flagged, uint32_t *grp, uint32_t *rec,
                                   uint32_t *idx) {
    if (!h || !n_flagged) return fail(SECEDO_E_INVALID_ARG, "null argument");
    if (!h->prepared || !h->flags_ready) return fail(SECEDO_E_STATE, "the flagged entries' lists have not been built");
    SECEDO_TRY(hipSetDevice(h->device));
    SECEDO_TRY(hipDeviceSynchronize());
    const size_t n_off = (size_t)h->pk.num_blocks * (h->pk.num_loci + 1);
    uint32_t n = 0;
    if (n_off) SECEDO_TRY(hipMemcpy(&n, h->flag_grp.as<uint32_t>() + n_off - 1, 4, hipMemcpyDeviceToHost));
    *n_flagged = n;
    if (grp && n_off) SECEDO_TRY(hipMemcpy(grp, h->flag_grp.p, n_off * 4, hipMemcpyDeviceToHost));
    if (rec && n) SECEDO_TRY(hipMemcpy(rec, h->flag_rec.p, (size_t)n * 16, hipMemcpyDeviceToHost));
    if (idx && n) SECEDO_TRY(hipMemcpy(idx, h->flag_idx.p, (size_t)n * 4, hipMemcpyDeviceToHost));
    return SECEDO_OK;
}

int secedo_simmat_last_pair_kernel_ms(secedo_simmat_t *h, float *ms) {
    if (!h || !ms) return fail(SECEDO_E_INVALID_ARG, "null argument");
    if (!h->timed || !h->timed_mid) return fail(SECEDO_E_STATE, "the last accumulate did not run the sparse-loci kernels");
    SECEDO_TRY(hipSetDevice(h->device));
    SECEDO_TRY(hipEventSynchronize(h->ev_mid));
    SECEDO_TRY(hipEventElapsedTime(ms, h->ev_begin, h->ev_mid));
    return SECEDO_OK;
}

}
```

Before: 815.8 billion updates/s.

## Fuse pileup packing kernels and fold scalar publishing into producer kernels

Merges several small device-packing kernels: id range and id bases are joined through a last-workgroup ticket, the flag scan moves into a records tail kernel, and rank/run kernels are combined. Mailbox scalar publishing is folded into the last kernel of each stage so no separate publish launch is needed, and range compaction is moved onto the side stream. The aim is fewer launches and host round-trip latency in the packing (prepare) phase. It adds atomic ticket synchronisation and a debug ranges API, with risk of ordering bugs. The packing phase may lie outside the timed similarity accumulate.

```diff
diff --git a/include/secedo_simmat.h b/include/secedo_simmat.h
--- a/include/secedo_simmat.h
+++ b/include/secedo_simmat.h
@@ -124,6 +124,8 @@
 uint32_t secedo_simmat_last_workgroups(const secedo_simmat_t *handle);
 int secedo_simmat_debug_flag_lists(secedo_simmat_t *handle, uint64_t *n_flagged, uint32_t *grp, uint32_t *rec,
                                    uint32_t *idx);
+int secedo_simmat_debug_ranges(secedo_simmat_t *handle, uint32_t *num_ranges, uint32_t *max_range_span,
+                               uint32_t *cap_loci, uint32_t *range_off);
 
 double secedo_simmat_llr(uint32_t x_s, uint32_t x_d, double mutation_rate, double homozygous_rate,
                          double seq_error_rate);
diff --git a/secedo_amd/_lib.py b/secedo_amd/_lib.py
--- a/secedo_amd/_lib.py
+++ b/secedo_amd/_lib.py
@@ -95,6 +95,7 @@
     "secedo_simmat_last_locus_words": (C.c_int, [_vp]),
     "secedo_simmat_last_workgroups": (C.c_uint32, [_vp]),
     "secedo_simmat_debug_flag_lists": (C.c_int, [_vp, _u64p, _vp, _vp, _vp]),
+    "secedo_simmat_debug_ranges": (C.c_int, [_vp, _vp, _vp, _vp, _vp]),
     "secedo_simmat_llr": (C.c_double, [C.c_uint32, C.c_uint32, C.c_double, C.c_double, C.c_double]),
     "secedo_simmat_llr_closed_form": (C.c_double, [C.c_uint32, C.c_uint32, C.c_double, C.c_double, C.c_double]),
     "secedo_simmat_pair_bound": (C.c_uint64, [_vp]),
diff --git a/secedo_amd/csrc/pack_device.hip b/secedo_amd/csrc/pack_device.hip
--- a/secedo_amd/csrc/pack_device.hip
+++ b/secedo_amd/csrc/pack_device.hip
@@ -68,6 +68,7 @@
     uint32_t reads_total;
     uint32_t n_wide;
     uint32_t max_range_span;
+    uint32_t ticket_ids, ticket_reads;
     unsigned long long id_space;
     unsigned long long multi_entries;
     unsigned long long pair_bound;
@@ -87,14 +88,51 @@
     }
 }
 
-hipError_t read_scalars(DevicePacked &pk, hipStream_t stream, const Scalars *sc, const unsigned long long *totals,
-                        Scalars *out, unsigned long long *out_totals, const std::function<void()> &behind = nullptr) {
-    static const bool plain = [] {
-        const char *e = std::getenv("SECEDO_PACK_READBACK");
-        return e && std::strcmp(e, "memcpy") == 0;
-    }();
-    hipError_t e;
-    if (!plain && !pk.mailbox && !pk.mailbox_failed) {
+template <class T>
+__device__ __forceinline__ T load_dev(const T *p) {
+    return __hip_atomic_load(p, __ATOMIC_RELAXED, __HIP_MEMORY_SCOPE_AGENT);
+}
+template <class T>
+__device__ __forceinline__ void store_dev(T *p, T v) {
+    __hip_atomic_store(p, v, __ATOMIC_RELAXED, __HIP_MEMORY_SCOPE_AGENT);
+}
+__device__ __forceinline__ bool last_workgroup(uint32_t *ticket) {
+    __shared__ uint32_t s_last;
+    asm volatile("s_waitcnt vmcnt(0)" ::: "memory");
+    __syncthreads();
+    if (threadIdx.x == 0) {
+        const uint32_t drawn = __hip_atomic_fetch_add(ticket, 1u, __ATOMIC_RELAXED, __HIP_MEMORY_SCOPE_AGENT);
+        const bool last = drawn + 1u == gridDim.x;
+        if (last) {
+            __builtin_amdgcn_fence(__ATOMIC_ACQUIRE, "agent");
+            store_dev(ticket, 0u);
+        }
+        s_last = last ? 1u : 0u;
+    }
+    __syncthreads();
+    return s_last != 0u;
+}
+struct Publish {
+    Mailbox *box;
+    unsigned long long seq;
+    const unsigned long long *totals;
+};
+__device__ __forceinline__ void publish_scalars(const Scalars *sc, const Publish &pub) {
+    static_assert(sizeof(Scalars) % 4 == 0, "copied word by word");
+    const uint32_t *src = reinterpret_cast<const uint32_t *>(sc);
+    uint32_t *dst = reinterpret_cast<uint32_t *>(&pub.box->sc);
+#pragma unroll
+    for (uint32_t i = 0; i < sizeof(Scalars) / 4; ++i) dst[i] = load_dev(src + i);
+    pub.box->totals = pub.totals ? load_dev(pub.totals) : 0ull;
+    __hip_atomic_store(&pub.box->seq, pub.seq, __ATOMIC_RELEASE, __HIP_MEMORY_SCOPE_SYSTEM);
+}
+bool plain_readback() {
+    const char *e = std::getenv("SECEDO_PACK_READBACK");
+    return e && std::strcmp(e, "memcpy") == 0;
+}
+Mailbox *mailbox_of(DevicePacked &pk) {
+    if (plain_readback()) return nullptr;
+    if (!pk.mailbox && !pk.mailbox_failed) {
         if (hipHostMalloc(&pk.mailbox, sizeof(Mailbox), hipHostMallocCoherent) == hipSuccess) {
             std::memset(pk.mailbox, 0, sizeof(Mailbox));
         } else {
@@ -103,10 +141,27 @@
             pk.mailbox_failed = true;
         }
     }
-    if (!plain && pk.mailbox) {
-        Mailbox *box = static_cast<Mailbox *>(pk.mailbox);
-        const unsigned long long seq = ++pk.mailbox_seq;
-        hipLaunchKernelGGL(k_publish, dim3(1), dim3(64), 0, stream, sc, totals, box, seq);
+    return static_cast<Mailbox *>(pk.mailbox);
+}
+Publish fold_publish(DevicePacked &pk, const unsigned long long *totals) {
+    Mailbox *box = mailbox_of(pk);
+    return Publish{box, box ? ++pk.mailbox_seq : 0ull, totals};
+}
+
+hipError_t read_scalars(DevicePacked &pk, hipStream_t stream, const Scalars *sc, const unsigned long long *totals,
+                        Scalars *out, unsigned long long *out_totals, const std::function<void()> &behind = nullptr,
+                        const Publish *folded = nullptr) {
+    hipError_t e;
+    Mailbox *const mailbox = folded ? folded->box : mailbox_of(pk);
+    if (mailbox) {
+        Mailbox *box = mailbox;
+        unsigned long long seq;
+        if (folded) {
+            seq = folded->seq;
+        } else {
+            seq = ++pk.mailbox_seq;
+            hipLaunchKernelGGL(k_publish, dim3(1), dim3(64), 0, stream, sc, totals, box, seq);
+        }
         if ((e = hipGetLastError()) != hipSuccess) return e;
         if (behind) behind();
         bool arrived = false;
@@ -199,7 +254,7 @@
     return (uint32_t)in.locus_entry_off[in.chr_locus_off[c]];
 }
 
-__global__ __launch_bounds__(TPB) void k_id_range(Raw in, uint32_t *id_max, uint32_t *id_negmin, int vec, Scalars *sc) {
+__device__ __forceinline__ void id_range_chunk(const Raw &in, uint32_t *id_max, uint32_t *id_negmin, int vec, Scalars *sc) {
     __shared__ uint32_t s_hi[TPB / 64], s_neg[TPB / 64];
     __shared__ uint32_t s_chr;
     for (uint32_t l = blockIdx.x * TPB + threadIdx.x; l + 1 < in.n_loci; l += gridDim.x * TPB) {
@@ -292,19 +347,21 @@
     }
 }
 
-__global__ void k_id_bases(Raw in, const uint32_t *id_max, const uint32_t *id_negmin, uint32_t *id_base,
-                           uint32_t *chr_entry, unsigned long long assumed_space, Scalars *sc) {
+__global__ __launch_bounds__(TPB) void k_id_range(Raw in, uint32_t *id_max, uint32_t *id_negmin, int vec,
+                                                 uint32_t *id_base, uint32_t *chr_entry,
+                                                 unsigned long long assumed_space, Scalars *sc) {
+    id_range_chunk(in, id_max, id_negmin, vec, sc);
+    if (!last_workgroup(&sc->ticket_ids)) return;
     const uint32_t n_chr = in.n_chr;
-    if (blockIdx.x != 0) return;
-    for (uint32_t c = threadIdx.x; c <= n_chr; c += blockDim.x) chr_entry[c] = chr_first_entry(in, c);
+    for (uint32_t c = threadIdx.x; c <= n_chr; c += TPB) chr_entry[c] = chr_first_entry(in, c);
     if (threadIdx.x != 0) return;
     unsigned long long sum = 0;
     uint32_t top = 0;
     for (uint32_t c = 0; c < n_chr; ++c) {
         id_base[c] = (uint32_t)min(sum, 0xFFFFFFFFull);
-        const uint32_t lo = ~id_negmin[c];
-        if ((id_max[c] | id_negmin[c]) != 0u) sum += (unsigned long long)(id_max[c] - lo) + 1ull;
-        top = max(top, id_max[c]);
+        const uint32_t hi = load_dev(id_max + c), neg = load_dev(id_negmin + c);
+        if ((hi | neg) != 0u) sum += (unsigned long long)(hi - ~neg) + 1ull;
+        top = max(top, hi);
     }
     id_base[n_chr] = (uint32_t)min(sum, 0xFFFFFFFFull);
     sc->id_space = sum;
@@ -471,6 +528,34 @@
         }
     }
 }
+constexpr int TPB_SCAN = 1024;
+template <int THREADS>
+__device__ __forceinline__ uint32_t scan_block_sums(const uint32_t *block_sum, uint32_t n_blocks, uint32_t *block_off) {
+    __shared__ uint32_t part[THREADS / 64];
+    const uint32_t lane = threadIdx.x & 63u, wv = threadIdx.x >> 6;
+    uint32_t carry = 0;
+    for (uint32_t base = 0; base < n_blocks; base += THREADS) {
+        const uint32_t i = base + threadIdx.x;
+        const uint32_t v = i < n_blocks ? load_dev(block_sum + i) : 0u;
+        uint32_t incl = v;
+        for (int off = 1; off < 64; off <<= 1) {
+            const uint32_t up = __shfl_up(incl, off);
+            if (lane >= (uint32_t)off) incl += up;
+        }
+        __syncthreads();
+        if (lane == 63u) part[wv] = incl;
+        __syncthreads();
+        uint32_t before = carry;
+#pragma unroll
+        for (int w2 = 0; w2 < THREADS / 64; ++w2) {
+            const uint32_t pw = part[w2];
+            if ((uint32_t)w2 < wv) before += pw;
+            carry += pw;
+        }
+        if (i < n_blocks) block_off[i] = before + incl - v;
+    }
+    return carry;
+}
 __global__ __launch_bounds__(TPB) void k_flag_count(const uint8_t *multi, uint32_t *block_sum) {
     __shared__ uint32_t part[TPB / 64];
     static_assert(kFlagBlock == TPB * 16, "a thread takes 16 consecutive flags");
@@ -485,35 +570,12 @@
         block_sum[blockIdx.x] = n;
     }
 }
-constexpr int TPB_SCAN = 1024;
 __global__ __launch_bounds__(TPB_SCAN) void k_flag_scan(const uint32_t *block_sum, uint32_t n_blocks, uint32_t *block_off,
                                                        uint32_t *total_out, Scalars *sc) {
-    constexpr int TPB = TPB_SCAN;
-    __shared__ uint32_t part[TPB / 64];
-    __shared__ uint32_t carry;
-    if (threadIdx.x == 0u) carry = 0;
-    __syncthreads();
-    const uint32_t lane = threadIdx.x & 63u, wv = threadIdx.x >> 6;
-    for (uint32_t base = 0; base < n_blocks; base += TPB) {
-        const uint32_t i = base + threadIdx.x;
-        const uint32_t v = i < n_blocks ? block_sum[i] : 0u;
-        uint32_t incl = v;
-        for (int off = 1; off < 64; off <<= 1) {
-            const uint32_t up = __shfl_up(incl, off);
-            if (lane >= (uint32_t)off) incl += up;
-        }
-        if (lane == 63u) part[wv] = incl;
-        __syncthreads();
-        uint32_t before = carry;
-        for (uint32_t w2 = 0; w2 < wv; ++w2) before += part[w2];
-        if (i < n_blocks) block_off[i] = before + incl - v;
-        __syncthreads();
-        if (threadIdx.x == TPB - 1) carry = before + incl;
-        __syncthreads();
-    }
+    const uint32_t total = scan_block_sums<TPB_SCAN>(block_sum, n_blocks, block_off);
     if (threadIdx.x == 0u) {
-        *total_out = carry;
-        if (sc) sc->n_multi_id = carry;
+        *total_out = total;
+        if (sc) sc->n_multi_id = total;
     }
 }
 struct MIndex {
@@ -526,7 +588,7 @@
 };
 __global__ __launch_bounds__(TPB) void k_compact_m(Raw in, const uint8_t *multi, const uint32_t *block_off,
                                                   uint32_t *chunk_pre, unsigned long long *chunk_mask,
-                                                  uint32_t *m_entry) {
+                                                  uint32_t *m_entry, uint32_t *count_m, Scalars *sc, Publish pub) {
     __shared__ uint32_t part[TPB / 64];
     const uint32_t lane = threadIdx.x & 63u, wv = threadIdx.x >> 6;
     const uint32_t e0 = blockIdx.x * kFlagBlock + threadIdx.x * 16u;
@@ -554,7 +616,12 @@
         chunk_mask[chunk] = m;
     }
     if (blockIdx.x == gridDim.x - 1u && threadIdx.x == 0u) chunk_mask[gridDim.x * (kFlagBlock / 64u)] = 0ull;
-    for (uint32_t b = bits; b; b &= b - 1u) m_entry[j++] = e0 + (uint32_t)__ffs((int)b) - 1u;
+    for (uint32_t b = bits; b; b &= b - 1u) {
+        count_m[j] = 0u;
+        m_entry[j++] = e0 + (uint32_t)__ffs((int)b) - 1u;
+    }
+    if (blockIdx.x == gridDim.x - 1u && threadIdx.x == TPB - 1) count_m[j] = 0u;
+    if (pub.box && blockIdx.x == 0u && threadIdx.x == 0u) publish_scalars(sc, pub);
 }
 __global__ __launch_bounds__(TPB) void k_pflag_count(const uint32_t *entry32, uint32_t n, uint32_t *block_sum) {
     __shared__ uint32_t part[TPB / 64];
@@ -665,8 +732,6 @@
 }
 void flag_lists_from_masks(const FlagScratch &fs, const uint4 *entry, const uint32_t *blk_off, size_t n_off,
                            uint32_t *grp, uint4 *rec, uint32_t *idx, hipStream_t stream) {
-    hipLaunchKernelGGL(k_flag_scan, dim3(1), dim3(TPB_SCAN), 0, stream, fs.block_sum, fs.nb, fs.block_off,
-                       fs.chunk_pre + 64 * (size_t)fs.nb, static_cast<Scalars *>(nullptr));
     hipLaunchKernelGGL(k_pflag_compact_masks, dim3(fs.nb), dim3(TPB), 0, stream, fs.chunk_mask, entry, fs.block_off, rec,
                        idx, fs.chunk_pre);
     flag_groups(fs, blk_off, n_off, grp, stream);
@@ -735,15 +800,6 @@
     uint32_t n_m;
     __device__ __forceinline__ uint32_t operator()(uint32_t j) const { return j < n_m ? 1u - mark_m[j] : 0u; }
 };
-__global__ void k_arank_m(const uint32_t *unm, const uint32_t *m_entry, uint32_t n_m, uint32_t n, uint32_t *arank_m,
-                          Scalars *sc) {
-    for (uint32_t j = blockIdx.x * TPB + threadIdx.x; j < n_m; j += gridDim.x * TPB) arank_m[j] = m_entry[j] - unm[j];
-    if (blockIdx.x == 0 && threadIdx.x == 0) sc->reads_total = n - unm[n_m];
-}
-__global__ void k_rbeg(Raw in, Ranks rank, uint32_t *rbeg) {
-    for (uint32_t c = blockIdx.x * TPB + threadIdx.x; c <= in.n_chr; c += gridDim.x * TPB)
-        rbeg[c] = rank((uint32_t)in.locus_entry_off[in.chr_locus_off[c]]);
-}
 struct HeadKeepOp {
     const unsigned long long *skey;
     const uint32_t *keep;
@@ -796,11 +852,30 @@
         }
     }
 }
+__global__ void k_ranks_runs(Raw in, Ranks rank, const uint32_t *m_entry, uint32_t n_m, uint32_t *arank_m,
+                             uint32_t *rbeg, const unsigned long long *incl, const uint32_t *sloc,
+                             uint32_t *run_start, uint32_t *read_locus, uint8_t *read_base, Scalars *sc) {
+    const uint32_t *unm = rank.unm;
+    for (uint32_t s = blockIdx.x * TPB + threadIdx.x; s < n_m; s += gridDim.x * TPB) {
+        arank_m[s] = m_entry[s] - unm[s];
+        const unsigned long long cur = incl[s], prev = s ? incl[s - 1] : 0ull;
+        if (incl_reads(cur) != incl_reads(prev)) run_start[incl_reads(cur) - 1] = s;
+        if (s == n_m - 1) run_start[incl_reads(cur)] = n_m;
+        if (incl_kept(cur) != incl_kept(prev)) {
+            const uint32_t k = incl_kept(prev), v = sloc[s];
+            read_locus[k] = sloc_locus(v);
+            read_base[k] = (uint8_t)sloc_base(v);
+        }
+    }
+    if (blockIdx.x == 0 && threadIdx.x == 0) sc->reads_total = in.n_entries - unm[n_m];
+    for (uint32_t c = blockIdx.x * TPB + threadIdx.x; c <= in.n_chr; c += gridDim.x * TPB)
+        rbeg[c] = rank((uint32_t)in.locus_entry_off[in.chr_locus_off[c]]);
+}
 
 __global__ __launch_bounds__(TPB) void k_read_info(Raw in, const unsigned long long *incl, const uint32_t *run_start,
                                                   const uint32_t *sval, const uint32_t *sloc,
                                                   const uint32_t *arank, uint32_t mfl, uint32_t *run_rank,
-                                                  uint32_t *rbeg, uint32_t *read_off, Scalars *sc) {
+                                                  uint32_t *rbeg, uint32_t *read_off, Scalars *sc, Publish pub) {
     __shared__ unsigned long long part[TPB / 64];
     __shared__ uint32_t part_len[TPB / 64];
     const uint32_t n = in.n_entries;
@@ -811,8 +886,8 @@
         const uint32_t s0 = run_start[r], s1 = run_start[r + 1];
         const uint32_t e0 = sval[s0];
         const uint32_t p0 = in.locus_pos[sloc_locus(sloc[s0])], p1 = in.locus_pos[sloc_locus(sloc[s1 - 1])];
-        if (p1 - p0 >= mfl) sc->long_reads = 1;
-        if ((unsigned long long)p1 + mfl > 0xFFFFFFFFull) sc->need_host = 1;
+        if (p1 - p0 >= mfl) store_dev(&sc->long_reads, 1u);
+        if ((unsigned long long)p1 + mfl > 0xFFFFFFFFull) store_dev(&sc->need_host, 1u);
         const uint32_t rk = arank[e0];
         run_rank[r] = rk;
         const uint32_t k0 = s0 ? incl_kept(incl[s0 - 1]) : 0u, k1 = incl_kept(incl[s1 - 1]);
@@ -844,6 +919,7 @@
         if (sum) atomicAdd(&sc->multi_entries, sum);
         if (len > 1) atomicMax(&sc->max_read_entries, len);
     }
+    if (pub.box && last_workgroup(&sc->ticket_reads) && threadIdx.x == 0) publish_scalars(sc, pub);
 }
 
 __global__ void k_completed(Raw in, Ranks rank, const uint32_t *rbeg, uint32_t mfl, uint32_t *cnt, Scalars *sc) {
@@ -1344,32 +1420,51 @@
     const uint32_t cap_loci = use_counts ? caps.loci_counts : caps.loci_plain;
     const uint32_t *seg_ends = seg_ends_both + (use_counts ? variant_stride : 0);
     const uint32_t *seg_count = seg_count_both + (use_counts ? variant_stride : 0);
-    __shared__ uint32_t s_base, s_span;
+    __shared__ uint32_t s_first[TPB];
+    __shared__ uint32_t s_part[TPB / 64];
+    __shared__ uint32_t s_span;
     if (threadIdx.x == 0) {
-        s_base = 0;
         s_span = 0;
         range_off[0] = 0;
     }
-    __syncthreads();
+    const uint32_t lane = threadIdx.x & 63u, wv = threadIdx.x >> 6;
     uint32_t span = 0;
-    for (uint32_t seg = 0; seg < n_seg; ++seg) {
-        const uint32_t base = s_base, cnt = seg_count[seg];
-        const uint32_t *ends = seg_ends + (size_t)seg * cap_loci;
-        for (uint32_t i = threadIdx.x; i < cnt; i += TPB) {
+    uint32_t done = 0;
+    for (uint32_t seg0 = 0; seg0 < n_seg; seg0 += TPB) {
+        const uint32_t n_here = min((uint32_t)TPB, n_seg - seg0);
+        const uint32_t cnt = threadIdx.x < n_here ? seg_count[seg0 + threadIdx.x] : 0u;
+        uint32_t incl = cnt;
+        for (int off = 1; off < 64; off <<= 1) {
+            const uint32_t up = __shfl_up(incl, off);
+            if (lane >= (uint32_t)off) incl += up;
+        }
+        __syncthreads();
+        if (lane == 63u) s_part[wv] = incl;
+        __syncthreads();
+        uint32_t before = 0, total = 0;
+#pragma unroll
+        for (int w2 = 0; w2 < TPB / 64; ++w2) {
+            if ((uint32_t)w2 < wv) before += s_part[w2];
+            total += s_part[w2];
+        }
+        s_first[threadIdx.x] = before + incl - cnt;
+        __syncthreads();
+        for (uint32_t r = threadIdx.x; r < total; r += TPB) {
+            const uint32_t sg = last_le<uint32_t>(s_first, n_here, r), i = r - s_first[sg];
+            const uint32_t seg = seg0 + sg;
+            const uint32_t *ends = seg_ends + (size_t)seg * cap_loci;
             const uint32_t e = ends[i];
             uint32_t begin = __shfl_up(e, 1);
-            if ((threadIdx.x & 63u) == 0) begin = i ? ends[i - 1] : seg * cap_loci;
-            range_off[1 + base + i] = e;
+            if (lane == 0u || i == 0u) begin = i ? ends[i - 1] : seg * cap_loci;
+            range_off[1 + done + r] = e;
             span = max(span, e - begin);
         }
-        __syncthreads();
-        if (threadIdx.x == 0) s_base = base + cnt;
-        __syncthreads();
+        done += total;
     }
     atomicMax(&s_span, span);
     __syncthreads();
     if (threadIdx.x == 0) {
-        sc->num_ranges = s_base;
+        sc->num_ranges = done;
         sc->max_range_span = s_span;
     }
 }
@@ -1630,18 +1725,28 @@
             if (sq[i]) atomicAdd(&per_cell_sq[first_cell + i], sq[i]);
 }
 
-__global__ __launch_bounds__(TPB) void k_pair_bound(const unsigned long long *per_cell_sq, uint32_t n_cells_padded,
-                                                   CapChoice caps, uint32_t assumed_counts, Scalars *sc) {
-    __shared__ unsigned long long s_best[TPB / 64];
+__global__ __launch_bounds__(TPB_SCAN) void k_records_tail(const unsigned long long *per_cell_sq, uint32_t n_cells_padded,
+                                                          CapChoice caps, uint32_t assumed_counts, Scalars *sc,
+                                                          Publish pub, const uint32_t *block_sum, uint32_t n_blocks,
+                                                          uint32_t *block_off, uint32_t *total_out) {
+    __shared__ unsigned long long s_best[TPB_SCAN / 64];
     unsigned long long best = 0;
-    for (uint32_t i = threadIdx.x; i < n_cells_padded; i += TPB) best = max(best, per_cell_sq[i]);
+    for (uint32_t i = threadIdx.x; i < n_cells_padded; i += TPB_SCAN) best = max(best, per_cell_sq[i]);
     for (int off = 32; off > 0; off >>= 1) best = max(best, (unsigned long long)__shfl_down(best, off));
     if ((threadIdx.x & 63) == 0) s_best[threadIdx.x >> 6] = best;
     __syncthreads();
     if (threadIdx.x == 0) {
-        for (int w = 1; w < TPB / 64; ++w) best = max(best, s_best[w]);
+        for (int w = 1; w < TPB_SCAN / 64; ++w) best = max(best, s_best[w]);
         sc->pair_bound = max(sc->pair_bound, best);
         sc->caps_wrong = (assumed_counts && !caps.counts(sc)) ? 1u : 0u;
+        if (pub.box) {
+            __threadfence();
+            publish_scalars(sc, pub);
+        }
+    }
+    if (block_sum) {
+        const uint32_t total = scan_block_sums<TPB_SCAN>(block_sum, n_blocks, block_off);
+        if (threadIdx.x == 0) *total_out = total;
     }
 }
 
@@ -1885,10 +1990,9 @@
     }
 
     Grouped group_by_read() {
+        const bool assume = !force_radix && !no_assumptions && pk.id_space_hint && pk.id_space_hint <= id_space_cap();
         hipLaunchKernelGGL(k_id_range, dim3(std::min<uint32_t>(256, (E + 4095) / 4096)), dim3(TPB), 0, stream, raw,
-                           m.id_max, m.id_negmin, ids_aligned, sc);
-        const bool assume = !force_radix && !no_assumptions && pk.id_space_hint && pk.id_space_hint <= id_space_cap();
-        hipLaunchKernelGGL(k_id_bases, dim3(1), dim3(64), 0, stream, raw, m.id_max, m.id_negmin, m.id_base, m.chr_entry,
+                           m.id_max, m.id_negmin, ids_aligned, m.id_base, m.chr_entry,
                            (unsigned long long)(assume ? pk.id_space_hint : 0), sc);
         Scalars hsc;
         std::memset(&hsc, 0, sizeof(hsc));
@@ -1937,10 +2041,11 @@
         hipLaunchKernelGGL(k_flag_count, dim3(n_flag_blocks), dim3(TPB), 0, stream, multi, sums.block_sum);
         hipLaunchKernelGGL(k_flag_scan, dim3(1), dim3(TPB_SCAN), 0, stream, sums.block_sum, n_flag_blocks, sums.block_off,
                            chunks.chunk_pre + (n_chunks - 1), sc);
+        const Publish pub = fold_publish(pk, nullptr);
         hipLaunchKernelGGL(k_compact_m, dim3(n_flag_blocks), dim3(TPB), 0, stream, raw, multi, sums.block_off,
-                           chunks.chunk_pre, chunks.chunk_mask, m_entry);
+                           chunks.chunk_pre, chunks.chunk_mask, m_entry, MReads(S[Arena::DENSE_M].p, 0).count_m, sc, pub);
         Scalars hsc;
-        HIP_OK(read_scalars(pk, stream, sc, nullptr, &hsc, nullptr));
+        HIP_OK(read_scalars(pk, stream, sc, nullptr, &hsc, nullptr, nullptr, &pub));
         STEP(scalar_verdict(hsc, false));
         Grouped g = whole_pileup(true);
         g.n_m = hsc.n_multi_id;
@@ -1958,7 +2063,6 @@
         if (g.n_m) {
             const uint32_t n_m = g.n_m;
             const MReads r(S[Arena::DENSE_M].p, n_m);
-            HIP_OK(hipMemsetAsync(r.count_m, 0, ((size_t)n_m + 1) * 4, stream));
             hipLaunchKernelGGL(k_m_fields, dim3(blocks_for(n_m)), dim3(TPB), 0, stream, raw, m.chr_entry, m.id_base,
                                m.id_negmin, last, g.m_index, m_entry, n_m, rid_m, idb_m, eloc_m, r.winner_m, r.count_m);
             HIP_OK(exclusive_sum(r.count_m, r.goff, (size_t)n_m + 1));
@@ -2028,7 +2132,7 @@
                          pk.read_locus.as<uint32_t>(),
                          pk.read_base.as<uint8_t>()};
     }
-    Attempt build_reads(const Grouped &g, const ReadViews &v, const uint32_t *split) {
+    Attempt build_reads(const Grouped &g, const ReadViews &v, const uint32_t *split, Publish *pub = nullptr) {
         const uint32_t n_m = g.n_m;
         uint32_t *mark_sub = g.single_entry ? v.mark_sub : v.marks.mark, *arank = v.marks.arank;
         if (n_m) {
@@ -2046,19 +2150,22 @@
             hipcub::TransformInputIterator<uint32_t, UnmarkedM, hipcub::CountingInputIterator<uint32_t>> unmarked(
                     entries, UnmarkedM{mark_sub, n_m});
             HIP_OK(exclusive_sum(unmarked, arank, (size_t)n_m + 1));
-            hipLaunchKernelGGL(k_arank_m, dim3(blocks_for(std::max(n_m, 1u))), dim3(TPB), 0, stream, arank, g.m_entry, n_m,
-                               E, v.arank_m, sc);
+            hipLaunchKernelGGL(k_ranks_runs, dim3(blocks_for(std::max(n_m, 1u))), dim3(TPB), 0, stream, raw, v.ranks,
+                               g.m_entry, n_m, v.arank_m, m.rbeg, v.incl, g.sloc, v.runs.run_start, v.read_locus,
+                               v.read_base, sc);
             arank_sub = v.arank_m;
-            hipLaunchKernelGGL(k_rbeg, dim3(1), dim3(TPB), 0, stream, raw, v.ranks, m.rbeg);
         } else {
             HIP_OK(exclusive_sum(v.marks.mark, arank, (size_t)E + 1));
+            if (n_m)
+                hipLaunchKernelGGL(k_runs_csr, dim3(blocks_for(n_m)), dim3(TPB), 0, stream, g.sub, v.incl, g.sval, g.sloc,
+                                   n_m, v.runs.run_start, v.read_locus, v.read_base);
         }
         if (n_m) {
-            hipLaunchKernelGGL(k_runs_csr, dim3(blocks_for(n_m)), dim3(TPB), 0, stream, g.sub, v.incl, g.sval, g.sloc, n_m,
-                               v.runs.run_start, v.read_locus, v.read_base);
-            hipLaunchKernelGGL(k_read_info, dim3(std::min<uint32_t>(blocks_for(n_m), 2048)), dim3(TPB), 0, stream, g.sub,
+            const bool fold = pub && g.single_entry;
+            const Publish folded = fold ? (*pub = fold_publish(pk, v.incl + (n_m - 1))) : Publish{nullptr, 0ull, nullptr};
+            hipLaunchKernelGGL(k_read_info, dim3(std::min<uint32_t>(blocks_for(n_m), fold ? 512 : 2048)), dim3(TPB), 0, stream, g.sub,
                                v.incl, v.runs.run_start, g.sval, g.sloc, arank_sub, mfl, v.runs.run_rank,
-                               g.single_entry ? nullptr : m.rbeg, v.read_off, sc);
+                               g.single_entry ? nullptr : m.rbeg, v.read_off, sc, folded);
         }
         HIP_OK(hipEventRecord(pk.ev_fork, stream));
         HIP_OK(hipStreamWaitEvent(pk.side, pk.ev_fork, 0));
@@ -2091,10 +2198,11 @@
         hipLaunchKernelGGL(k_ranges_segment, dim3(s.p.n_seg, s.p.caps.allow_counts ? 2u : 1u), dim3(TPB), 0, on, s.blk_off,
                            s.p.nb, L, s.p.caps, s.segs.seg_ends, s.segs.seg_count, s.p.variant_stride);
     }
-    Attempt cut_ranges_on_side(const Stage5 &s) {
+    Attempt cut_ranges_on_side(const Stage5 &s, bool pick) {
         HIP_OK(hipEventRecord(pk.ev_offsets, stream));
         HIP_OK(hipStreamWaitEvent(pk.side, pk.ev_offsets, 0));
         launch_ranges_segment(s, pk.side);
+        if (pick) compact_ranges(s, 0u, assumed_variant(s.p), pk.side);
         HIP_OK(hipEventRecord(pk.ev_join, pk.side));
         return Attempt();
     }
@@ -2105,14 +2213,21 @@
         HIP_OK(hipEventRecord(pk.ev_join, pk.side));
         return Attempt();
     }
-    void pick_ranges(const Stage5 &s, uint32_t sq_rows, int assumed, const uint8_t *dupflag) {
-        hipLaunchKernelGGL(k_ranges_compact, dim3(1), dim3(TPB), 0, stream, s.segs.seg_ends, s.segs.seg_count,
+    void compact_ranges(const Stage5 &s, uint32_t sq_rows, int assumed, hipStream_t on) {
+        hipLaunchKernelGGL(k_ranges_compact, dim3(1), dim3(TPB), 0, on, s.segs.seg_ends, s.segs.seg_count,
                            s.p.variant_stride, s.p.n_seg, s.p.caps, pk.range_off.as<uint32_t>(), s.per_cell_sq, sq_rows,
                            assumed, sc);
+    }
+    void locus_info(const Stage5 &s, const uint8_t *dupflag) {
         if (s.n_kept)
             hipLaunchKernelGGL(k_locus_info, dim3(blocks_for(L)), dim3(TPB), 0, stream, raw, pk.range_off.as<uint32_t>(),
                                sc, dupflag, m.locus_chr, m.locus_rel);
     }
+    void pick_ranges(const Stage5 &s, uint32_t sq_rows, int assumed, const uint8_t *dupflag) {
+        compact_ranges(s, sq_rows, assumed, stream);
+        locus_info(s, dupflag);
+    }
+    static int assumed_variant(const TilePlan &p) { return p.caps.allow_counts ? 1 : 0; }
 
     Attempt bin_radix(const Stage5 &s) {
         const BinRadix &b = s.bin;
@@ -2125,7 +2240,7 @@
                                stream, b.key2_b, s.n_kept, s.p.B, L, s.p.lbits, s.blk_cnt, s.per_cell_sq);
         }
         HIP_OK(exclusive_sum(s.blk_cnt, s.blk_off, s.n_off));
-        return cut_ranges_on_side(s);
+        return cut_ranges_on_side(s, false);
     }
     Attempt bin_counting(const Grouped &g, const ReadViews &v, const Stage5 &s, bool hist_first) {
         const TilePlan &p = s.p;
@@ -2143,8 +2258,9 @@
         trace.mark("offset scan launched");
         if (records_first) {
             launch_ranges_segment(s, stream);
+            compact_ranges(s, 0u, assumed_variant(p), stream);
         } else {
-            STEP(cut_ranges_on_side(s));
+            STEP(cut_ranges_on_side(s, true));
             if (s.kept_m) STEP(m_records_on_side(s, v));
         }
         if (s.n_kept) {
@@ -2166,11 +2282,11 @@
                                m.locus_chr, m.locus_rel, s.p.B, s.p.lbits, pk.entry.as<uint4>(), pk.entry32.as<uint32_t>(),
                                pk.stage_masks ? pk.mask32.as<uint32_t>() : nullptr, pk.entry_read.as<uint32_t>(), sc);
     }
-    bool records_counting(const Stage5 &s) {
+    bool records_counting(const Stage5 &s, Publish *pub) {
         const TilePlan &p = s.p;
-        const int assumed = p.caps.allow_counts ? 1 : 0;
+        const int assumed = assumed_variant(p);
         bool lists_here = false;
-        pick_ranges(s, 0u, assumed, s.dupflag);
+        locus_info(s, s.dupflag);
         if (s.n_kept) {
             const RecordTables tables{s.m_rec, m.locus_rel, pk.entry.as<uint4>(), pk.entry32.as<uint32_t>(),
                                       pk.stage_masks ? pk.mask32.as<uint32_t>() : nullptr, pk.entry_read.as<uint32_t>()};
@@ -2180,11 +2296,14 @@
                                GroupedKept(S[Arena::KEY_B].p, E).p, s.blk_off, s.n_kept, p.nb, L, p.B, p.lbits, tables,
                                s.per_cell_sq, sc, lists_here ? fs.chunk_mask : nullptr, lists_here ? fs.block_sum : nullptr);
         }
-        hipLaunchKernelGGL(k_pair_bound, dim3(1), dim3(TPB), 0, stream, s.per_cell_sq, s.n_kept ? p.nb * p.B : 0u, p.caps,
-                           (uint32_t)assumed, sc);
+        const FlagScratch fs(lists_here ? pk.flag_lists.scratch : nullptr, s.n_kept);
+        *pub = fold_publish(pk, nullptr);
+        hipLaunchKernelGGL(k_records_tail, dim3(1), dim3(TPB_SCAN), 0, stream, s.per_cell_sq, s.n_kept ? p.nb * p.B : 0u,
+                           p.caps, (uint32_t)assumed, sc, *pub, lists_here ? fs.block_sum : nullptr, fs.nb,
+                           lists_here ? fs.block_off : nullptr, lists_here ? fs.chunk_pre + 64 * (size_t)fs.nb : nullptr);
         return lists_here;
     }
-    Attempt close_attempt(const Stage5 &s, bool lists_launched) {
+    Attempt close_attempt(const Stage5 &s, bool lists_launched, const Publish *folded) {
         const TilePlan &p = s.p;
         Scalars hsc;
         trace.mark("records launched");
@@ -2192,7 +2311,7 @@
             if (lists_launched)
                 flag_lists_from_masks(FlagScratch(pk.flag_lists.scratch, s.n_kept), pk.entry.as<uint4>(), s.blk_off, s.n_off,
                                       pk.flag_lists.grp, pk.flag_lists.rec, pk.flag_lists.idx, stream);
-        }));
+        }, folded));
         trace.mark("read-back 3 arrived");
         if (!force_radix && hsc.caps_wrong && !hsc.regroup && hsc.error == 0) {
             pick_ranges(s, 0u, 0, nullptr);
@@ -2229,7 +2348,8 @@
 
         STEP(ensure_outputs());
         const ReadViews v = read_views(g);
-        STEP(build_reads(g, v, nullptr));
+        Publish pub2{nullptr, 0ull, nullptr};
+        STEP(build_reads(g, v, nullptr, &pub2));
         struct SideJoin {
             hipStream_t side;
             bool joined = false;
@@ -2239,7 +2359,8 @@
         Scalars hsc;
         unsigned long long totals = 0;
         trace.mark("reads built (launched)");
-        HIP_OK(read_scalars(pk, stream, sc, g.n_m ? v.incl + (g.n_m - 1) : nullptr, &hsc, &totals));
+        HIP_OK(read_scalars(pk, stream, sc, g.n_m ? v.incl + (g.n_m - 1) : nullptr, &hsc, &totals, nullptr,
+                            g.n_m && g.single_entry ? &pub2 : nullptr));
         trace.mark("read-back 2 arrived");
         const Attempt verdict = scalar_verdict(hsc, false);
         if (verdict.go() || verdict.kind == Attempt::RetryRadix || verdict.kind == Attempt::NeedHost)
@@ -2303,11 +2424,12 @@
         HIP_OK(hipStreamWaitEvent(stream, pk.ev_join, 0));
         side_join.joined = true;
         bool lists_launched = false;
+        Publish pub3{nullptr, 0ull, nullptr};
         if (force_radix)
             records_radix(v, s);
         else
-            lists_launched = records_counting(s);
-        return close_attempt(s, lists_launched);
+            lists_launched = records_counting(s, &pub3);
+        return close_attempt(s, lists_launched, force_radix ? nullptr : &pub3);
     }
 };
 
diff --git a/secedo_amd/csrc/simmat_api.cpp b/secedo_amd/csrc/simmat_api.cpp
--- a/secedo_amd/csrc/simmat_api.cpp
+++ b/secedo_amd/csrc/simmat_api.cpp
@@ -587,6 +587,20 @@
     return SECEDO_OK;
 }
 
+int secedo_simmat_debug_ranges(secedo_simmat_t *h, uint32_t *num_ranges, uint32_t *max_range_span, uint32_t *cap_loci,
+                               uint32_t *range_off) {
+    if (!h || !num_ranges || !max_range_span || !cap_loci) return fail(SECEDO_E_INVALID_ARG, "null argument");
+    if (!h->prepared) return fail(SECEDO_E_STATE, "no pileup has been prepared");
+    SECEDO_TRY(hipSetDevice(h->device));
+    SECEDO_TRY(hipDeviceSynchronize());
+    *num_ranges = h->pk.num_ranges;
+    *max_range_span = h->pk.max_range_span;
+    *cap_loci = h->pk.cap_loci;
+    if (range_off)
+        SECEDO_TRY(hipMemcpy(range_off, h->pk.range_off.p, ((size_t)h->pk.num_ranges + 1) * 4, hipMemcpyDeviceToHost));
+    return SECEDO_OK;
+}
+
 int secedo_simmat_last_pair_kernel_ms(secedo_simmat_t *h, float *ms) {
     if (!h || !ms) return fail(SECEDO_E_INVALID_ARG, "null argument");
     if (!h->timed || !h->timed_mid) return fail(SECEDO_E_STATE, "the last accumulate did not run the sparse-loci kernels");
```

After: 828.9 billion updates/s, median of 6. 1.6% higher.
